# ParCoreLab/aCG

Hardware: AMD Instinct MI355X
Metric: CG iter/s (whole node), Queen_4147-shaped fp64 (higher is better)
Workload: dtype fp64; 1 GPU; model=queen4147-like-27pt-dof3-G111, rows=4102893, solver=cg-pipelined, parallelism=slab1-rccl

## Files before the change

acg_amd/gen/device_slab.py:

```python

from __future__ import annotations

import numpy as np
import torch

from ..part.subdomain import HaloPattern
from .stencil import _blocks, _slab_bounds


class DeviceSlabSystem:

    def __init__(self, **kw):
        self.__dict__.update(kw)

    @property
    def nlocal(self):
        return self.nowned + self.nghost

    @property
    def nnzA(self):
        return self._nnzA

    @property
    def nnzO(self):
        return self._nnzO


def estimate_slab_gib(gx: int, gy: int, gz: int, spec: dict, rank: int,
                      nranks: int, matfree: bool = False) -> float:
    dof = spec["dof"]
    pts = len(spec["offsets"]) + 1
    z0, z1 = _slab_bounds(gz, rank, nranks)
    nghost_planes = (1 if rank > 0 else 0) + (1 if rank < nranks - 1 else 0)
    nlocal = (z1 - z0 + nghost_planes) * gx * gy * dof
    bytes_per_row = 81.0 if matfree else 12.0 * pts * dof + 73.0
    return nlocal * bytes_per_row / 2**30


def preflight_slab(gx: int, gy: int, gz: int, spec: dict, rank: int,
                   nranks: int, matfree: bool, total_bytes: int,
                   headroom: float = 0.94) -> float:
    est = estimate_slab_gib(gx, gy, gz, spec, rank, nranks, matfree)
    budget = headroom * total_bytes / 2**30
    if est > budget:
        raise MemoryError(
            f"rank {rank}/{nranks} of {gx}x{gy}x{gz} needs ~{est:.0f} GiB "
            f"({'matfree' if matfree else 'assembled'}) but this GPU has "
            f"{total_bytes / 2**30:.0f} GiB ({budget:.0f} usable); use more "
            f"ranks, --matfree, or a smaller --grid")
    return est


def device_stencil_slab(gx: int, gy: int, gz: int, spec: dict,
                        rank: int, nranks: int, device,
                        operator: bool = True) -> DeviceSlabSystem:
    from ..ops import gpu_ops

    K = gpu_ops.K
    device = torch.device(device)
    dof = spec["dof"]
    M, D = _blocks(spec)
    z0, z1 = _slab_bounds(gz, rank, nranks)
    nz_own = z1 - z0
    if nz_own <= 0:
        raise ValueError(f"rank {rank} owns no z-planes")
    plane_nodes = gx * gy
    has_lo, has_hi = rank > 0, rank < nranks - 1
    border_planes = sorted(set(([z0] if has_lo else []) +
                               ([z1 - 1] if has_hi else [])))
    interior_planes = [z for z in range(z0, z1) if z not in border_planes]
    ghost_planes = ([z0 - 1] if has_lo else []) + ([z1] if has_hi else [])
    plane_seq = interior_planes + border_planes + ghost_planes

    nown_nodes = nz_own * plane_nodes
    ninterior_nodes = len(interior_planes) * plane_nodes
    nborder_nodes = len(border_planes) * plane_nodes
    nghost_nodes = len(ghost_planes) * plane_nodes
    nowned = nown_nodes * dof
    nghost = nghost_nodes * dof
    assert (nowned + nghost) * 1 < 2**31, "device generator needs int32 local cols"

    pb = torch.full((gz + 2,), -1, dtype=torch.int64)
    for k, z in enumerate(plane_seq):
        pb[z + 1] = k * plane_nodes
    zs_own = torch.tensor([z for z in interior_planes + border_planes],
                          dtype=torch.int32)
    pb = pb.to(device)
    zs_own = zs_own.to(device)
    offs_np = np.asarray([[dx, dy, dz, w] for (dx, dy, dz, w) in spec["offsets"]],
                         dtype=np.float64)
    offs = torch.from_numpy(offs_np).reshape(-1).to(device)
    ksten = len(spec["offsets"])
    blocks = torch.from_numpy(
        np.concatenate([M.reshape(-1), D.reshape(-1)])).to(device)
    stream = torch.cuda.current_stream(device).cuda_stream

    def build(filter_ghost: int, nodes: int, row0_node: int):
        if nodes == 0:
            empty = torch.zeros(1, dtype=torch.int64, device=device)
            return (torch.zeros(1, dtype=torch.int64, device=device),
                    torch.zeros(0, dtype=torch.int32, device=device),
                    torch.zeros(0, dtype=torch.float64, device=device), 0)
        rowlen_nodes = torch.empty(nodes, dtype=torch.int64, device=device)
        K.stencil_rowlen(nodes, row0_node, gx, gy, gz, dof, nown_nodes,
                         zs_own.data_ptr(), pb.data_ptr(), offs.data_ptr(),
                         ksten, filter_ghost, rowlen_nodes.data_ptr(), stream)
        rowlen = rowlen_nodes if dof == 1 else rowlen_nodes.repeat_interleave(dof)
        nnz = int(rowlen.sum())
        if not operator:
            return None, None, None, nnz
        nrows = nodes * dof
        nslices = (nrows + 63) // 64
        padded = torch.zeros(nslices * 64, dtype=torch.int64, device=device)
        padded[:nrows] = rowlen
        slice_len = padded.view(nslices, 64).max(dim=1).values
        sellptr = torch.zeros(nslices + 1, dtype=torch.int64, device=device)
        torch.cumsum(slice_len * 64, dim=0, out=sellptr[1:])
        total = int(sellptr[-1])
        cols = torch.zeros(total, dtype=torch.int32, device=device)
        vals = torch.zeros(total, dtype=torch.float64, device=device)
        K.stencil_fill(nodes, row0_node, gx, gy, gz, dof, nown_nodes,
                       zs_own.data_ptr(), pb.data_ptr(), offs.data_ptr(),
                       ksten, blocks.data_ptr(), filter_ghost,
                       sellptr.data_ptr(), cols.data_ptr(), vals.data_ptr(),
                       stream)
        return sellptr, cols, vals, nnz

    A_sellptr, A_cols, A_vals, nnzA = build(0, nown_nodes, 0)
    O_sellptr, O_cols, O_vals, nnzO = build(1, nborder_nodes, ninterior_nodes)

    mf_tables = None
    if dof == 1:
        w7 = None
        if ksten == 6:
            wmap = {(int(dx), int(dy), int(dz)): float(w)
                    for (dx, dy, dz, w) in spec["offsets"]}
            keys = [(-1, 0, 0), (1, 0, 0), (0, -1, 0),
                    (0, 1, 0), (0, 0, -1), (0, 0, 1)]
            if set(wmap) == set(keys):
                w7 = tuple(wmap[k] for k in keys)
        mf_tables = dict(zs=zs_own, pb=pb, offs=offs, ksten=ksten,
                         diag=float(D[0, 0]), gx=gx, gy=gy, gz=gz,
                         nown_nodes=nown_nodes, z0=z0, z1=z1, w7=w7)

    A_bsell = None
    if operator and 2 <= dof <= 4 and nown_nodes > 0:
        blocklen = torch.empty(nown_nodes, dtype=torch.int64, device=device)
        K.stencil_blocklen(nown_nodes, gx, gy, gz, nown_nodes,
                           zs_own.data_ptr(), pb.data_ptr(), offs.data_ptr(),
                           ksten, blocklen.data_ptr(), stream)
        nbslices = (nown_nodes + 63) // 64
        bp = torch.zeros(nbslices * 64, dtype=torch.int64, device=device)
        bp[:nown_nodes] = blocklen
        blk_slice = bp.view(nbslices, 64).max(dim=1).values
        bptr = torch.zeros(nbslices + 1, dtype=torch.int64, device=device)
        torch.cumsum(blk_slice * 64, dim=0, out=bptr[1:])
        btotal = int(bptr[-1])
        bcol = torch.zeros(btotal, dtype=torch.int32, device=device)
        bvals = torch.zeros(btotal * dof * dof, dtype=torch.float64, device=device)
        K.stencil_bfill(nown_nodes, gx, gy, gz, dof, nown_nodes,
                        zs_own.data_ptr(), pb.data_ptr(), offs.data_ptr(),
                        ksten, blocks.data_ptr(), bptr.data_ptr(),
                        bcol.data_ptr(), bvals.data_ptr(), stream)
        A_bsell = (bptr, bcol, bvals, dof)

    senders, recvcounts, rdispls = [], [], []
    recipients, sendidx_parts = [], []
    off = 0
    if has_lo:
        senders.append(rank - 1)
        recvcounts.append(plane_nodes * dof)
        rdispls.append(off)
        off += plane_nodes * dof
    if has_hi:
        senders.append(rank + 1)
        recvcounts.append(plane_nodes * dof)
        rdispls.append(off)
        off += plane_nodes * dof

    plane_local = {z: k for k, z in enumerate(plane_seq)}

    def plane_rows(z):
        b = plane_local[z] * plane_nodes
        node_loc = b + np.arange(plane_nodes, dtype=np.int64)
        return (node_loc[:, None] * dof + np.arange(dof)[None, :]).ravel()

    if has_lo:
        recipients.append(rank - 1)
        sendidx_parts.append(plane_rows(z0))
    if has_hi:
        recipients.append(rank + 1)
        sendidx_parts.append(plane_rows(z1 - 1))
    sendcounts = [len(s) for s in sendidx_parts]
    sdispls = list(np.concatenate([[0], np.cumsum(sendcounts)[:-1]])) if sendcounts else []
    sendidx = (np.concatenate(sendidx_parts) if sendidx_parts
               else np.zeros(0, np.int64))
    halo = HaloPattern(
        senders=np.asarray(senders, dtype=np.int32),
        recvcounts=np.asarray(recvcounts, dtype=np.int64),
        rdispls=np.asarray(rdispls, dtype=np.int64),
        recipients=np.asarray(recipients, dtype=np.int32),
        sendcounts=np.asarray(sendcounts, dtype=np.int64),
        sdispls=np.asarray(sdispls, dtype=np.int64),
        sendidx=sendidx.astype(np.int32),
    )
    return DeviceSlabSystem(
        rank=rank, nparts=nranks, n_global=gx * gy * gz * dof,
        nowned=nowned, ninterior=ninterior_nodes * dof,
        nborder=nborder_nodes * dof, nghost=nghost,
        A_sell=(A_sellptr, A_cols, A_vals) if operator else None,
        A_bsell=A_bsell,
        O_sell=(O_sellptr, O_cols, O_vals) if operator else None,
        mf_tables=mf_tables,
        _nnzA=nnzA, _nnzO=nnzO, halo=halo, device=device,
    )
```

acg_amd/ops/gpu_ops.py:

```python

from __future__ import annotations

import torch

try:
    from . import _acg_kernels as K
except ImportError as e:
    raise ImportError(
        "acg_amd HIP kernel extension (_acg_kernels) is not built. "
        "Run `python -m acg_amd.ops.build` (hipcc --offload-arch=gfx950). "
        f"Original error: {e}"
    ) from e

S_RR = K.S_RR
S_PT = K.S_PT
S_RR_PREV = K.S_RR_PREV
S_BNRM2 = K.S_BNRM2
S_GAMMA = K.S_GAMMA
S_DELTA = K.S_DELTA
S_GAMMA_PREV = K.S_GAMMA_PREV
S_ALPHA_PREV = K.S_ALPHA_PREV
S_NSLOTS = K.S_NSLOTS
MAXG = K.MAXG


def _stream() -> int:
    return torch.cuda.current_stream().cuda_stream


def alloc_scalars(device) -> torch.Tensor:
    return torch.zeros(S_NSLOTS, dtype=torch.float64, device=device)


def alloc_partials(device) -> torch.Tensor:
    return torch.zeros(2 * MAXG, dtype=torch.float64, device=device)


def pick_lanes(mean_nnz_per_row: float) -> int:
    if mean_nnz_per_row <= 4.0:
        return 4
    if mean_nnz_per_row <= 8.0:
        return 8
    if mean_nnz_per_row <= 16.0:
        return 16
    if mean_nnz_per_row <= 96.0:
        return 32
    return 64


def spmv(rowptr: torch.Tensor, colidx: torch.Tensor, vals: torch.Tensor,
         x: torch.Tensor, y: torch.Tensor, *, rowbase: int = 0,
         lanes: int = 16, accum: bool = False,
         partials: torch.Tensor | None = None,
         scal: torch.Tensor | None = None, dotslot: int = -1,
         dot_accum: bool = True) -> None:
    nrows = rowptr.numel() - 1
    if nrows <= 0:
        return
    fuse = scal is not None and dotslot >= 0
    K.spmv(nrows, rowbase, rowptr.data_ptr(), colidx.data_ptr(),
           1 if colidx.dtype == torch.int64 else 0,
           vals.data_ptr(), x.data_ptr(), y.data_ptr(), lanes, accum,
           partials.data_ptr() if fuse else 0,
           scal.data_ptr() if fuse else 0, dotslot, dot_accum, _stream())


def build_row_bins(rowptr, max_lanes: int = 64):
    import numpy as np

    rowptr = np.asarray(rowptr)
    lens = np.diff(rowptr)
    order = np.argsort(-lens, kind="stable").astype(np.int32)
    slens = lens[order.astype(np.int64)]
    bins = []
    lo = 0
    for lanes, thresh in ((64, 96), (32, 16), (16, 8), (8, 4), (4, None)):
        if lanes > max_lanes:
            continue
        if thresh is None:
            hi = len(slens)
        else:
            hi = int(np.searchsorted(-slens, -thresh - 1, side="right"))
        if hi > lo:
            bins.append((lo, hi - lo, lanes))
            lo = hi
    return order, bins


def build_sellcsr_hybrid(rowptr, colidx, vals, cut: int = 192,
                         window: int = 0, bucket: int = 8):
    import numpy as np

    from .torch_ref import sellcsr_split

    sellptr, cols, svals, perm, long_rows, nshort = sellcsr_split(
        rowptr, colidx, vals, cut=cut, window=window, bucket=bucket)
    lens = np.diff(np.asarray(rowptr))
    longlens = lens[long_rows.astype(np.int64)]
    bins = []
    lo = 0
    for lanes, thresh in ((64, 96), (32, 16), (16, 8), (8, 4), (4, None)):
        if thresh is None:
            hi = len(longlens)
        else:
            hi = int(np.searchsorted(-longlens, -thresh - 1, side="right"))
        if hi > lo:
            bins.append((lo, hi - lo, lanes))
            lo = hi
        if lo >= len(longlens):
            break
    if nshort == 0:
        sellptr = None
    return sellptr, cols, svals, perm, long_rows, bins


def spmv_binned(rowptr: torch.Tensor, colidx: torch.Tensor, vals: torch.Tensor,
                rowlist: torch.Tensor, bins, x: torch.Tensor, y: torch.Tensor,
                *, rowbase: int = 0, accum: bool = False,
                partials: torch.Tensor | None = None,
                scal: torch.Tensor | None = None, dotslot: int = -1,
                dot_accum: bool = True) -> None:
    if rowlist.numel() == 0:
        return
    assert rowlist.dtype == torch.int32
    fuse = scal is not None and dotslot >= 0
    K.spmv_binned(rowbase, rowptr.data_ptr(), colidx.data_ptr(),
                  1 if colidx.dtype == torch.int64 else 0,
                  vals.data_ptr(), x.data_ptr(), y.data_ptr(),
                  rowlist.data_ptr(), [list(b) for b in bins], accum,
                  partials.data_ptr() if fuse else 0,
                  scal.data_ptr() if fuse else 0, dotslot, dot_accum,
                  _stream())


SELL_NT, SELL_SWZ, SELL_U8 = 1, 2, 4
DEFAULT_SELL_VARIANT = SELL_NT | SELL_U8


def spmv_sell(sellptr: torch.Tensor, cols: torch.Tensor, vals: torch.Tensor,
              nrows: int, x: torch.Tensor, y: torch.Tensor, *,
              rowbase: int = 0, accum: bool = False,
              partials: torch.Tensor | None = None,
              scal: torch.Tensor | None = None, dotslot: int = -1,
              dot_accum: bool = True, variant: int | None = None,
              perm: torch.Tensor | None = None) -> None:
    nslices = sellptr.numel() - 1
    if nslices <= 0:
        return
    if variant is None:
        variant = DEFAULT_SELL_VARIANT
    fuse = scal is not None and dotslot >= 0
    K.spmv_sell(nslices, nrows, rowbase, sellptr.data_ptr(), cols.data_ptr(),
                1 if cols.dtype == torch.int64 else 0,
                vals.data_ptr(), x.data_ptr(), y.data_ptr(), accum,
                partials.data_ptr() if fuse else 0,
                scal.data_ptr() if fuse else 0, dotslot, dot_accum,
                variant, perm.data_ptr() if perm is not None else 0, _stream())


def spmv_bsell(bptr: torch.Tensor, bcol: torch.Tensor, bvals: torch.Tensor,
               nnodes: int, dof: int, x: torch.Tensor, y: torch.Tensor, *,
               partials: torch.Tensor | None = None,
               scal: torch.Tensor | None = None, dotslot: int = -1,
               dot_accum: bool = True) -> None:
    nslices = bptr.numel() - 1
    if nslices <= 0:
        return
    fuse = scal is not None and dotslot >= 0
    K.spmv_bsell(nslices, nnodes, dof, bptr.data_ptr(), bcol.data_ptr(),
                 bvals.data_ptr(), x.data_ptr(), y.data_ptr(),
                 partials.data_ptr() if fuse else 0,
                 scal.data_ptr() if fuse else 0, dotslot, dot_accum, _stream())


def stencil_spmv(mf, nrows_nodes: int, row0_node: int, x: torch.Tensor,
                 y: torch.Tensor, *, mato: bool = False,
                 partials: torch.Tensor | None = None,
                 scal: torch.Tensor | None = None, dotslot: int = -1,
                 dot_accum: bool = True) -> None:
    if nrows_nodes <= 0:
        return
    fuse = scal is not None and dotslot >= 0
    pp = partials.data_ptr() if fuse else 0
    sp = scal.data_ptr() if fuse else 0
    if not mato and mf["w7"] is not None:
        K.stencil_spmv7(mf["gx"] * mf["gy"], mf["gx"], mf["z0"], mf["z1"],
                        mf["gz"], mf["nown_nodes"], mf["pb"].data_ptr(),
                        mf["diag"], *mf["w7"], x.data_ptr(), y.data_ptr(),
                        pp, sp, dotslot, dot_accum, _stream())
        return
    K.stencil_spmv(nrows_nodes, row0_node, mf["gx"], mf["gy"], mf["gz"],
                   mf["nown_nodes"], mf["zs"].data_ptr(),
                   mf["pb"].data_ptr(), mf["offs"].data_ptr(), mf["ksten"],
                   mf["diag"], x.data_ptr(), y.data_ptr(), mato,
                   pp, sp, dotslot, dot_accum, _stream())


def stencil_pipe(mf, nrows_nodes: int, row0_node: int, border_base: int,
                 w_old, qpart, z, t, p, x, r, w_new, scal, first: bool,
                 partials, partials_off: int, mato: bool) -> int:
    if nrows_nodes <= 0:
        return 0
    qp = qpart.data_ptr() if qpart is not None else 0
    if not mato and mf["w7"] is not None:
        return K.stencil_pipe7(mf["gx"] * mf["gy"], mf["gx"], mf["z0"],
                               mf["z1"], mf["gz"], border_base,
                               mf["nown_nodes"], mf["pb"].data_ptr(),
                               mf["diag"], *mf["w7"], w_old.data_ptr(), qp,
                               z.data_ptr(), t.data_ptr(), p.data_ptr(),
                               x.data_ptr(), r.data_ptr(), w_new.data_ptr(),
                               scal.data_ptr(), 1 if first else 0,
                               partials.data_ptr(), partials_off, _stream())
    return K.stencil_pipe(nrows_nodes, row0_node, border_base, mf["gx"],
                          mf["gy"], mf["gz"], mf["nown_nodes"],
                          mf["zs"].data_ptr(), mf["pb"].data_ptr(),
                          mf["offs"].data_ptr(), mf["ksten"], mf["diag"],
                          w_old.data_ptr(), qp,
                          z.data_ptr(), t.data_ptr(), p.data_ptr(),
                          x.data_ptr(), r.data_ptr(), w_new.data_ptr(),
                          scal.data_ptr(), 1 if first else 0,
                          partials.data_ptr(), partials_off, mato, _stream())


def spmv_bsell_daypx(bptr, bcol, bvals, nnodes: int, dof: int,
                     pold: torch.Tensor, rvec: torch.Tensor,
                     pnew: torch.Tensor, y: torch.Tensor,
                     scal: torch.Tensor, partials: torch.Tensor,
                     dotslot: int) -> None:
    nslices = bptr.numel() - 1
    if nslices <= 0:
        return
    K.spmv_bsell_daypx(nslices, nnodes, dof, bptr.data_ptr(), bcol.data_ptr(),
                       bvals.data_ptr(), pold.data_ptr(), rvec.data_ptr(),
                       pnew.data_ptr(), y.data_ptr(), scal.data_ptr(),
                       partials.data_ptr(), dotslot, _stream())


def zero_scalars(scal: torch.Tensor, i0: int = 0, count: int | None = None) -> None:
    K.zero_scalars(scal.data_ptr(), i0, count if count is not None else scal.numel() - i0,
                   _stream())


def cg_prep_pt(scal: torch.Tensor) -> None:
    K.cg_prep_pt(scal.data_ptr(), _stream())


def cg_prep_rr(scal: torch.Tensor) -> None:
    K.cg_prep_rr(scal.data_ptr(), _stream())


def dot(x: torch.Tensor, y: torch.Tensor, partials: torch.Tensor,
        scal: torch.Tensor, slot: int, n: int | None = None,
        accumulate: bool = False) -> None:
    n = x.numel() if n is None else n
    K.dot(x.data_ptr(), y.data_ptr(), n, partials.data_ptr(), scal.data_ptr(),
          slot, accumulate, _stream())


def dot2(r: torch.Tensor, w: torch.Tensor, partials: torch.Tensor,
         scal: torch.Tensor, n: int, accumulate: bool = False) -> None:
    K.dot2(r.data_ptr(), w.data_ptr(), n, partials.data_ptr(), scal.data_ptr(),
           accumulate, _stream())


def axpy_ratio(y: torch.Tensor, x: torch.Tensor, scal: torch.Tensor,
               num: int, den: int, sign: float = 1.0, n: int | None = None) -> None:
    K.axpy_ratio(y.data_ptr(), x.data_ptr(), y.numel() if n is None else n,
                 scal.data_ptr(), num, den, sign, _stream())


def daypx_ratio(y: torch.Tensor, x: torch.Tensor, scal: torch.Tensor,
                num: int, den: int, n: int | None = None) -> None:
    K.daypx_ratio(y.data_ptr(), x.data_ptr(), y.numel() if n is None else n,
                  scal.data_ptr(), num, den, _stream())


def cg_fused_update(r: torch.Tensor, x: torch.Tensor, p: torch.Tensor,
                    t: torch.Tensor, scal: torch.Tensor,
                    partials: torch.Tensor, n: int) -> None:
    K.cg_fused_update(r.data_ptr(), x.data_ptr(), p.data_ptr(), t.data_ptr(),
                      n, scal.data_ptr(), partials.data_ptr(), _stream())


def pcg_fused_update(r, x, p, t, z, dinv, scal, partials, n: int) -> None:
    K.pcg_fused_update(r.data_ptr(), x.data_ptr(), p.data_ptr(), t.data_ptr(),
                       z.data_ptr(), dinv.data_ptr(), n, scal.data_ptr(),
                       partials.data_ptr(), _stream())


def sell_pipe(sellptr, cols, vals, nrows_pass: int, rowbase: int,
              border_base: int, w_old, qpart, z, t, p, x, r, w_new,
              scal, first: bool, partials, partials_off: int,
              mato: bool) -> int:
    nslices = sellptr.numel() - 1
    assert cols.dtype == torch.int32
    return K.sell_pipe(nslices, nrows_pass, rowbase, border_base,
                       sellptr.data_ptr(), cols.data_ptr(), vals.data_ptr(),
                       w_old.data_ptr(),
                       qpart.data_ptr() if qpart is not None else 0,
                       z.data_ptr(), t.data_ptr(), p.data_ptr(), x.data_ptr(),
                       r.data_ptr(), w_new.data_ptr(), scal.data_ptr(),
                       1 if first else 0, partials.data_ptr(), partials_off,
                       mato, _stream())


def pipelined_finalize(partials, nblocks: int, scal, first: bool) -> None:
    K.pipelined_finalize(partials.data_ptr(), nblocks, scal.data_ptr(),
                         1 if first else 0, _stream())


def pipelined_fused(z, t, p, x, r, w, q, scal: torch.Tensor,
                    partials: torch.Tensor, n: int, first: bool,
                    nt_update: bool = True) -> None:
    K.pipelined_fused(z.data_ptr(), t.data_ptr(), p.data_ptr(), x.data_ptr(),
                      r.data_ptr(), w.data_ptr(), q.data_ptr(), n,
                      scal.data_ptr(), 1 if first else 0, partials.data_ptr(),
                      nt_update, _stream())


BAR_STATE_WORDS = 400


def cg_device(sellptr: torch.Tensor, cols: torch.Tensor, vals: torch.Tensor,
              nrows: int, b: torch.Tensor, x: torch.Tensor, r: torch.Tensor,
              p: torch.Tensor, t: torch.Tensor, scal: torch.Tensor,
              partials: torch.Tensor, out2: torch.Tensor,
              barrier_state: torch.Tensor, maxits: int,
              res_atol: float, res_rtol: float,
              hier: bool | None = None) -> int:
    nslices = sellptr.numel() - 1
    assert barrier_state.numel() >= BAR_STATE_WORDS
    if hier is None:
        import os

        v = os.environ.get("ACG_DEVCG_HIER", "auto")
        ih = -1 if v == "auto" else (0 if v == "0" else 1)
    else:
        ih = 1 if hier else 0
    return K.cg_device(nslices, nrows, sellptr.data_ptr(), cols.data_ptr(),
                       1 if cols.dtype == torch.int64 else 0, vals.data_ptr(),
                       b.data_ptr(), x.data_ptr(), r.data_ptr(), p.data_ptr(),
                       t.data_ptr(), scal.data_ptr(), partials.data_ptr(),
                       out2.data_ptr(), barrier_state.data_ptr(),
                       maxits, res_atol, res_rtol, _stream(), ih)


def pack_gather(sendbuf: torch.Tensor, x: torch.Tensor, idx: torch.Tensor) -> None:
    K.pack_gather(sendbuf.data_ptr(), x.data_ptr(), idx.data_ptr(),
                  1 if idx.dtype == torch.int64 else 0,
                  sendbuf.numel(), _stream())
```

acg_amd/ops/kernels.hip:

```cpp
#define S_RR 0
#define S_PT 1
#define S_RR_PREV 2
#define S_BNRM2 3
#define S_GAMMA 4
#define S_DELTA 5
#define S_GAMMA_PREV 6
#define S_ALPHA_PREV 7
#define S_NSLOTS 8

#define MAXG 16384

#include <hip/hip_runtime.h>
#include <pybind11/pybind11.h>
#include <pybind11/stl.h>
#include <array>
#include <cstdint>
#include <vector>
#include <stdexcept>
#include <string>

namespace py = pybind11;

#define WAVE 64
#define BLOCK 256

static inline void check_hip(const char* what) {
    hipError_t e = hipGetLastError();
    if (e != hipSuccess)
        throw std::runtime_error(std::string("HIP error in ") + what + ": " + hipGetErrorString(e));
}

static inline long elem_grid(long n, long per_thread = 4) {
    long blocks = (n + (long)BLOCK * per_thread - 1) / ((long)BLOCK * per_thread);
    if (blocks > 4096) blocks = 4096;
    if (blocks < 1) blocks = 1;
    return blocks;
}

__device__ __forceinline__ double block_reduce(double v) {
    #pragma unroll
    for (int off = WAVE / 2; off > 0; off >>= 1)
        v += __shfl_down(v, off, WAVE);
    __shared__ double w[BLOCK / WAVE];
    const int lane = threadIdx.x & (WAVE - 1);
    const int wid = threadIdx.x >> 6;
    if (lane == 0) w[wid] = v;
    __syncthreads();
    if (wid == 0) {
        v = (lane < BLOCK / WAVE) ? w[lane] : 0.0;
        #pragma unroll
        for (int off = (BLOCK / WAVE) / 2; off > 0; off >>= 1)
            v += __shfl_down(v, off, WAVE);
    }
    return v;
}

__device__ __forceinline__ double safe_div(double a, double b) {
    return b != 0.0 ? a / b : 0.0;
}

__global__ void __launch_bounds__(BLOCK)
k_reduce_partials(const double* __restrict__ partials, int nblocks,
                  double* scal, int slot, int accumulate) {
    double v = 0.0;
    for (int i = threadIdx.x; i < nblocks; i += BLOCK) v += partials[i];
    v = block_reduce(v);
    if (threadIdx.x == 0) scal[slot] = accumulate ? scal[slot] + v : v;
}

template <typename ColT, int LANES, bool ACCUM, bool FUSE_DOT, bool ROWLIST = false>
__global__ void __launch_bounds__(BLOCK)
spmv_csr_vector(long nrows, long rowbase,
                const long* __restrict__ rowptr,
                const ColT* __restrict__ colidx,
                const double* __restrict__ vals,
                const double* __restrict__ x,
                double* __restrict__ y,
                double* __restrict__ partials,
                const int* __restrict__ rowlist = nullptr) {
    const int lane = threadIdx.x & (LANES - 1);
    const long group = ((long)blockIdx.x * BLOCK + threadIdx.x) / LANES;
    const long ngroups = (long)gridDim.x * BLOCK / LANES;
    double dacc = 0.0;
    for (long i = group; i < nrows; i += ngroups) {
        const long r = ROWLIST ? (long)rowlist[i] : i;
        const long k0 = rowptr[r], k1 = rowptr[r + 1];
        double sum = 0.0;
        for (long k = k0 + lane; k < k1; k += LANES)
            sum += vals[k] * x[colidx[k]];
        #pragma unroll
        for (int off = LANES / 2; off > 0; off >>= 1)
            sum += __shfl_down(sum, off, LANES);
        if (lane == 0) {
            const long row = rowbase + r;
            if (ACCUM) y[row] += sum; else y[row] = sum;
            if (FUSE_DOT) dacc += x[row] * sum;
        }
    }
    if (FUSE_DOT) {
        dacc = block_reduce(dacc);
        if (threadIdx.x == 0) partials[blockIdx.x] = dacc;
    }
}

#define SELL_NT 1
#define SELL_SWZ 2
#define SELL_U8 4

template <typename T>
__device__ __forceinline__ T ld_nt(const T* p) { return __builtin_nontemporal_load(p); }

template <typename ColT, bool ACCUM, bool FUSE_DOT, bool NT, bool SWZ, int UNROLL,
          bool PERM = false>
__global__ void __launch_bounds__(BLOCK)
k_spmv_sell(long nslices, long nrows, long rowbase,
          const long* __restrict__ sellptr,
          const ColT* __restrict__ cols,
          const double* __restrict__ vals,
          const double* __restrict__ x,
          double* __restrict__ y,
          double* __restrict__ partials,
          const int* __restrict__ perm = nullptr) {
    const int lane = threadIdx.x & (WAVE - 1);
    long blk = blockIdx.x;
    if (SWZ) {
        const long nb = gridDim.x, q = nb / 8, rr = nb % 8, xcd = blk % 8;
        blk = (xcd < rr ? xcd * (q + 1) : rr * (q + 1) + (xcd - rr) * q) + blk / 8;
    }
    const long wslice = (blk * BLOCK + threadIdx.x) >> 6;
    const long nw = ((long)gridDim.x * BLOCK) >> 6;
    double dacc = 0.0;
    for (long s = wslice; s < nslices; s += nw) {
        const long base = sellptr[s];
        const long len = (sellptr[s + 1] - base) >> 6;
        const double* __restrict__ v = vals + base + lane;
        const ColT* __restrict__ c = cols + base + lane;
        double sum = 0.0;
        long j = 0;
        for (; j + UNROLL <= len; j += UNROLL) {
            double a[UNROLL], xx[UNROLL];
            #pragma unroll
            for (int u = 0; u < UNROLL; ++u) {
                a[u] = NT ? ld_nt(v + (j + u) * WAVE) : v[(j + u) * WAVE];
                const ColT ci = NT ? ld_nt(c + (j + u) * WAVE) : c[(j + u) * WAVE];
                xx[u] = x[ci];
            }
            #pragma unroll
            for (int u = 0; u < UNROLL; ++u) sum += a[u] * xx[u];
        }
        for (; j < len; ++j) {
            const double a = NT ? ld_nt(v + j * WAVE) : v[j * WAVE];
            const ColT ci = NT ? ld_nt(c + j * WAVE) : c[j * WAVE];
            sum += a * x[ci];
        }
        const long row = PERM ? (long)perm[s * WAVE + lane] : s * WAVE + lane;
        if (row < nrows) {
            if (ACCUM) y[rowbase + row] += sum; else y[rowbase + row] = sum;
            if (FUSE_DOT) dacc += x[rowbase + row] * sum;
        }
    }
    if (FUSE_DOT) {
        dacc = block_reduce(dacc);
        if (threadIdx.x == 0) partials[blockIdx.x] = dacc;
    }
}

__device__ __forceinline__ long stencil_col_node(
    int xi, int yi, int zi, int dx, int dy, int dz, int gx, int gy, int gz,
    const long* __restrict__ pb);

template <int D2>
__device__ __forceinline__ long bval_off(int k, int lane) {
    constexpr int EVEN = D2 & ~1;
    return (k < EVEN) ? (long)(k >> 1) * (2 * WAVE) + lane * 2 + (k & 1)
                      : (long)EVEN * WAVE + lane;
}

template <int DOF, bool FUSE_DOT>
__global__ void __launch_bounds__(BLOCK)
k_spmv_bsell(long nslices, long nnodes,
             const long* __restrict__ bptr,
             const int* __restrict__ bcol,
             const double* __restrict__ bvals,
             const double* __restrict__ x,
             double* __restrict__ y,
             double* __restrict__ partials) {
    const int lane = threadIdx.x & (WAVE - 1);
    const long wslice = ((long)blockIdx.x * BLOCK + threadIdx.x) >> 6;
    const long nw = ((long)gridDim.x * BLOCK) >> 6;
    double dacc = 0.0;
    for (long s = wslice; s < nslices; s += nw) {
        const long b0 = bptr[s];
        const long blen = (bptr[s + 1] - b0) >> 6;
        const int* __restrict__ c = bcol + b0 + lane;
        const double* __restrict__ v = bvals + b0 * (DOF * DOF);
        double acc[DOF];
        #pragma unroll
        for (int r = 0; r < DOF; ++r) acc[r] = 0.0;
        for (long j = 0; j < blen; ++j) {
            const int cb = ld_nt(c + j * WAVE);
            double xv[DOF];
            #pragma unroll
            for (int cc = 0; cc < DOF; ++cc) xv[cc] = x[(long)cb * DOF + cc];
            const double* __restrict__ vj = v + j * (DOF * DOF) * WAVE;
            #pragma unroll
            for (int k = 0; k < DOF * DOF; ++k) {
                const double a = ld_nt(vj + bval_off<DOF * DOF>(k, lane));
                acc[k / DOF] += a * xv[k % DOF];
            }
        }
        const long node = s * WAVE + lane;
        if (node < nnodes) {
            #pragma unroll
            for (int r = 0; r < DOF; ++r) {
                y[node * DOF + r] = acc[r];
                if (FUSE_DOT) dacc += x[node * DOF + r] * acc[r];
            }
        }
    }
    if (FUSE_DOT) {
        dacc = block_reduce(dacc);
        if (threadIdx.x == 0) partials[blockIdx.x] = dacc;
    }
}

template <int DOF>
__global__ void __launch_bounds__(BLOCK)
k_spmv_bsell_daypx(long nslices, long nnodes,
                   const long* __restrict__ bptr,
                   const int* __restrict__ bcol,
                   const double* __restrict__ bvals,
                   const double* __restrict__ pold,
                   const double* __restrict__ rvec,
                   double* __restrict__ pnew,
                   double* __restrict__ y,
                   const double* __restrict__ scal,
                   double* __restrict__ partials) {
    const int lane = threadIdx.x & (WAVE - 1);
    const long wslice = ((long)blockIdx.x * BLOCK + threadIdx.x) >> 6;
    const long nw = ((long)gridDim.x * BLOCK) >> 6;
    const double beta = safe_div(scal[S_RR], scal[S_RR_PREV]);
    double dacc = 0.0;
    for (long s = wslice; s < nslices; s += nw) {
        const long b0 = bptr[s];
        const long blen = (bptr[s + 1] - b0) >> 6;
        const int* __restrict__ c = bcol + b0 + lane;
        const double* __restrict__ v = bvals + b0 * (DOF * DOF);
        double acc[DOF];
        #pragma unroll
        for (int r = 0; r < DOF; ++r) acc[r] = 0.0;
        for (long j = 0; j < blen; ++j) {
            const int cb = ld_nt(c + j * WAVE);
            double xv[DOF];
            #pragma unroll
            for (int cc = 0; cc < DOF; ++cc)
                xv[cc] = beta * pold[(long)cb * DOF + cc]
                         + rvec[(long)cb * DOF + cc];
            const double* __restrict__ vj = v + j * (DOF * DOF) * WAVE;
            #pragma unroll
            for (int k = 0; k < DOF * DOF; ++k) {
                const double a = ld_nt(vj + bval_off<DOF * DOF>(k, lane));
                acc[k / DOF] += a * xv[k % DOF];
            }
        }
        const long node = s * WAVE + lane;
        if (node < nnodes) {
            #pragma unroll
            for (int r = 0; r < DOF; ++r) {
                const double pn = beta * pold[node * DOF + r]
                                  + rvec[node * DOF + r];
                pnew[node * DOF + r] = pn;
                y[node * DOF + r] = acc[r];
                dacc += pn * acc[r];
            }
        }
    }
    dacc = block_reduce(dacc);
    if (threadIdx.x == 0) partials[blockIdx.x] = dacc;
}

__global__ void __launch_bounds__(BLOCK)
k_stencil_blocklen(long nnodes, int gx, int gy, int gz, long nown_nodes,
                   const int* __restrict__ zs_of_plane,
                   const long* __restrict__ pb,
                   const double* __restrict__ offs, int ksten,
                   long* __restrict__ blocklen) {
    const long stride = (long)gridDim.x * BLOCK;
    const long plane_nodes = (long)gx * gy;
    for (long i = (long)blockIdx.x * BLOCK + threadIdx.x; i < nnodes; i += stride) {
        const int pl = (int)(i / plane_nodes);
        const long rem = i - (long)pl * plane_nodes;
        const int xi = (int)(rem % gx), yi = (int)(rem / gx);
        const int zi = zs_of_plane[pl];
        long cnt = 1;
        for (int o = 0; o < ksten; ++o) {
            const long cn = stencil_col_node(xi, yi, zi, (int)offs[o * 4],
                                             (int)offs[o * 4 + 1],
                                             (int)offs[o * 4 + 2], gx, gy, gz, pb);
            if (cn >= 0 && cn < nown_nodes) ++cnt;
        }
        blocklen[i] = cnt;
    }
}

template <int DOF>
__global__ void __launch_bounds__(BLOCK)
k_stencil_bfill(long nnodes, int gx, int gy, int gz, long nown_nodes,
                const int* __restrict__ zs_of_plane,
                const long* __restrict__ pb,
                const double* __restrict__ offs, int ksten,
                const double* __restrict__ blocks,
                const long* __restrict__ bptr,
                int* __restrict__ bcol, double* __restrict__ bvals) {
    const long stride = (long)gridDim.x * BLOCK;
    const long plane_nodes = (long)gx * gy;
    const double* M = blocks;
    const double* D = blocks + DOF * DOF;
    for (long i = (long)blockIdx.x * BLOCK + threadIdx.x; i < nnodes; i += stride) {
        const int pl = (int)(i / plane_nodes);
        const long rem = i - (long)pl * plane_nodes;
        const int xi = (int)(rem % gx), yi = (int)(rem / gx);
        const int zi = zs_of_plane[pl];
        const long s = i >> 6;
        const int lane = (int)(i & 63);
        const long b0 = bptr[s];
        const long blen = (bptr[s + 1] - b0) >> 6;
        long j = 0;
        double* __restrict__ bv = bvals + b0 * DOF * DOF;
        bcol[b0 + j * WAVE + lane] = (int)i;
        for (int k = 0; k < DOF * DOF; ++k)
            bv[j * DOF * DOF * WAVE + bval_off<DOF * DOF>(k, lane)] = D[k];
        ++j;
        for (int o = 0; o < ksten; ++o) {
            const long cn = stencil_col_node(xi, yi, zi, (int)offs[o * 4],
                                             (int)offs[o * 4 + 1],
                                             (int)offs[o * 4 + 2], gx, gy, gz, pb);
            if (cn < 0 || cn >= nown_nodes) continue;
            const double w = offs[o * 4 + 3];
            bcol[b0 + j * WAVE + lane] = (int)cn;
            for (int k = 0; k < DOF * DOF; ++k)
                bv[j * DOF * DOF * WAVE + bval_off<DOF * DOF>(k, lane)] = w * M[k];
            ++j;
        }
        for (; j < blen; ++j) {
            bcol[b0 + j * WAVE + lane] = (int)i;
            for (int k = 0; k < DOF * DOF; ++k)
                bv[j * DOF * DOF * WAVE + bval_off<DOF * DOF>(k, lane)] = 0.0;
        }
    }
}


__global__ void __launch_bounds__(BLOCK)
k_zero_scalars(double* scal, int i0, int count) {
    for (int i = threadIdx.x; i < count; i += BLOCK) scal[i0 + i] = 0.0;
}

__global__ void k_cg_prep_pt(double* scal) { if (threadIdx.x == 0) scal[S_PT] = 0.0; }

__global__ void k_cg_prep_rr(double* scal) {
    if (threadIdx.x == 0) scal[S_RR_PREV] = scal[S_RR];
}

__global__ void __launch_bounds__(BLOCK)
k_cg_finalize(const double* __restrict__ partials, int nblocks, double* scal) {
    double v = 0.0;
    for (int i = threadIdx.x; i < nblocks; i += BLOCK) v += partials[i];
    v = block_reduce(v);
    if (threadIdx.x == 0) {
        scal[S_RR_PREV] = scal[S_RR];
        scal[S_RR] = v;
    }
}

__global__ void __launch_bounds__(BLOCK)
k_pcg_fused_update(double* __restrict__ r, double* __restrict__ x,
                   const double* __restrict__ p, const double* __restrict__ t,
                   double* __restrict__ z, const double* __restrict__ dinv,
                   long n, const double* __restrict__ scal,
                   double* __restrict__ partials) {
    const double alpha = safe_div(scal[S_RR], scal[S_PT]);
    double arz = 0.0, arr = 0.0;
    const long stride = (long)gridDim.x * BLOCK;
    for (long i = (long)blockIdx.x * BLOCK + threadIdx.x; i < n; i += stride) {
        const double rn = r[i] - alpha * ld_nt(t + i);
        r[i] = rn;
        __builtin_nontemporal_store(ld_nt(x + i) + alpha * p[i], x + i);
        const double zi = dinv[i] * rn;
        z[i] = zi;
        arz += rn * zi;
        arr += rn * rn;
    }
    arz = block_reduce(arz);
    __syncthreads();
    arr = block_reduce(arr);
    if (threadIdx.x == 0) {
        partials[blockIdx.x] = arz;
        partials[MAXG + blockIdx.x] = arr;
    }
}

__global__ void __launch_bounds__(BLOCK)
k_pcg_finalize(const double* __restrict__ partials, int nblocks,
               double* scal) {
    double vz = 0.0, vr = 0.0;
    for (int i = threadIdx.x; i < nblocks; i += BLOCK) {
        vz += partials[i];
        vr += partials[MAXG + i];
    }
    vz = block_reduce(vz);
    __syncthreads();
    vr = block_reduce(vr);
    if (threadIdx.x == 0) {
        scal[S_RR_PREV] = scal[S_RR];
        scal[S_RR] = vz;
        scal[S_GAMMA] = vr;
    }
}

__global__ void __launch_bounds__(BLOCK)
k_dot(const double* __restrict__ x, const double* __restrict__ y, long n,
      double* __restrict__ partials) {
    double acc = 0.0;
    const long stride = (long)gridDim.x * BLOCK;
    for (long i = (long)blockIdx.x * BLOCK + threadIdx.x; i < n; i += stride)
        acc += x[i] * y[i];
    acc = block_reduce(acc);
    if (threadIdx.x == 0) partials[blockIdx.x] = acc;
}

__global__ void __launch_bounds__(BLOCK)
k_dot2(const double* __restrict__ r, const double* __restrict__ w, long n,
       double* __restrict__ partials) {
    double g = 0.0, d = 0.0;
    const long stride = (long)gridDim.x * BLOCK;
    for (long i = (long)blockIdx.x * BLOCK + threadIdx.x; i < n; i += stride) {
        const double ri = r[i];
        g += ri * ri;
        d += w[i] * ri;
    }
    g = block_reduce(g);
    __syncthreads();
    d = block_reduce(d);
    if (threadIdx.x == 0) {
        partials[blockIdx.x] = g;
        partials[MAXG + blockIdx.x] = d;
    }
}

__global__ void __launch_bounds__(BLOCK)
k_reduce_partials2(const double* __restrict__ partials, int nblocks,
                   double* scal, int accumulate) {
    double g = 0.0, d = 0.0;
    for (int i = threadIdx.x; i < nblocks; i += BLOCK) {
        g += partials[i];
        d += partials[MAXG + i];
    }
    g = block_reduce(g);
    __syncthreads();
    d = block_reduce(d);
    if (threadIdx.x == 0) {
        scal[S_GAMMA] = accumulate ? scal[S_GAMMA] + g : g;
        scal[S_DELTA] = accumulate ? scal[S_DELTA] + d : d;
    }
}

__global__ void __launch_bounds__(BLOCK)
k_axpy_ratio(double* __restrict__ y, const double* __restrict__ x, long n,
             const double* __restrict__ scal, int num, int den, double sign) {
    const double a = sign * safe_div(scal[num], scal[den]);
    const long stride = (long)gridDim.x * BLOCK;
    for (long i = (long)blockIdx.x * BLOCK + threadIdx.x; i < n; i += stride)
        y[i] += a * x[i];
}

__global__ void __launch_bounds__(BLOCK)
k_daypx_ratio(double* __restrict__ y, const double* __restrict__ x, long n,
              const double* __restrict__ scal, int num, int den) {
    const double b = safe_div(scal[num], scal[den]);
    const long stride = (long)gridDim.x * BLOCK;
    for (long i = (long)blockIdx.x * BLOCK + threadIdx.x; i < n; i += stride)
        y[i] = b * y[i] + x[i];
}

__global__ void __launch_bounds__(BLOCK)
k_cg_fused_update(double* __restrict__ r, double* __restrict__ x,
                  const double* __restrict__ p, const double* __restrict__ t,
                  long n, const double* __restrict__ scal,
                  double* __restrict__ partials) {
    const double alpha = safe_div(scal[S_RR], scal[S_PT]);
    double acc = 0.0;
    const long stride = (long)gridDim.x * BLOCK;
    for (long i = (long)blockIdx.x * BLOCK + threadIdx.x; i < n; i += stride) {
        const double rn = r[i] - alpha * ld_nt(t + i);
        r[i] = rn;
        __builtin_nontemporal_store(ld_nt(x + i) + alpha * p[i], x + i);
        acc += rn * rn;
    }
    acc = block_reduce(acc);
    if (threadIdx.x == 0) partials[blockIdx.x] = acc;
}

__device__ __forceinline__ void pipelined_coeffs(const double* scal, int first,
                                                 double* beta, double* alpha) {
    const double gamma = scal[S_GAMMA], delta = scal[S_DELTA];
    if (first) { *beta = 0.0; *alpha = safe_div(gamma, delta); }
    else {
        const double b = safe_div(gamma, scal[S_GAMMA_PREV]);
        *beta = b;
        *alpha = safe_div(gamma,
                          delta - b * safe_div(gamma, scal[S_ALPHA_PREV]));
    }
}

template <bool NTU>
__global__ void __launch_bounds__(BLOCK)
k_pipelined_fused(double* __restrict__ z, double* __restrict__ t,
                  double* __restrict__ p, double* __restrict__ x,
                  double* __restrict__ r, double* __restrict__ w,
                  const double* __restrict__ q, long n,
                  const double* __restrict__ scal, int first,
                  double* __restrict__ partials) {
    double beta, alpha;
    pipelined_coeffs(scal, first, &beta, &alpha);
    double g = 0.0, d = 0.0;
    const long stride = (long)gridDim.x * BLOCK;
    for (long i = (long)blockIdx.x * BLOCK + threadIdx.x; i < n; i += stride) {
        const double zi = (NTU ? ld_nt(q + i) : q[i]) + beta * (NTU ? ld_nt(z + i) : z[i]);
        const double ti = w[i] + beta * (NTU ? ld_nt(t + i) : t[i]);
        const double pi = r[i] + beta * (NTU ? ld_nt(p + i) : p[i]);
        const double xn = (NTU ? ld_nt(x + i) : x[i]) + alpha * pi;
        if (NTU) {
            __builtin_nontemporal_store(zi, z + i);
            __builtin_nontemporal_store(ti, t + i);
            __builtin_nontemporal_store(pi, p + i);
            __builtin_nontemporal_store(xn, x + i);
        } else {
            z[i] = zi; t[i] = ti; p[i] = pi; x[i] = xn;
        }
        const double rn = r[i] - alpha * ti;
        const double wn = w[i] - alpha * zi;
        r[i] = rn; w[i] = wn;
        g += rn * rn;
        d += wn * rn;
    }
    g = block_reduce(g);
    __syncthreads();
    d = block_reduce(d);
    if (threadIdx.x == 0) {
        partials[blockIdx.x] = g;
        partials[MAXG + blockIdx.x] = d;
    }
}

template <typename ColT, bool NT, int UNROLL, bool MATO>
__global__ void __launch_bounds__(BLOCK)
k_sell_pipe(long nslices, long nrows_pass, long rowbase, long border_base,
            const long* __restrict__ sellptr, const ColT* __restrict__ cols,
            const double* __restrict__ vals,
            const double* __restrict__ w_old,
            double* __restrict__ qpart,
            double* __restrict__ z, double* __restrict__ t,
            double* __restrict__ p, double* __restrict__ x,
            double* __restrict__ r, double* __restrict__ w_new,
            const double* __restrict__ scal, int first,
            double* __restrict__ partials, long partials_off) {
    const int lane = threadIdx.x & (WAVE - 1);
    const long wslice = ((long)blockIdx.x * BLOCK + threadIdx.x) >> 6;
    const long nw = ((long)gridDim.x * BLOCK) >> 6;
    double beta, alpha;
    pipelined_coeffs(scal, first, &beta, &alpha);
    double g = 0.0, d = 0.0;
    for (long s = wslice; s < nslices; s += nw) {
        const long base = sellptr[s];
        const long len = (sellptr[s + 1] - base) >> 6;
        const double* __restrict__ v = vals + base + lane;
        const ColT* __restrict__ c = cols + base + lane;
        double sum = 0.0;
        long j = 0;
        for (; j + UNROLL <= len; j += UNROLL) {
            double a[UNROLL], xx[UNROLL];
            #pragma unroll
            for (int u = 0; u < UNROLL; ++u) {
                a[u] = NT ? ld_nt(v + (j + u) * WAVE) : v[(j + u) * WAVE];
                xx[u] = w_old[c[(j + u) * WAVE]];
            }
            #pragma unroll
            for (int u = 0; u < UNROLL; ++u) sum += a[u] * xx[u];
        }
        for (; j < len; ++j)
            sum += (NT ? ld_nt(v + j * WAVE) : v[j * WAVE]) * w_old[c[j * WAVE]];
        const long rr = s * WAVE + lane;
        if (rr < nrows_pass) {
            const long row = rowbase + rr;
            if (!MATO && row >= border_base) {
                qpart[row - border_base] = sum;
            } else {
                const double q = MATO ? sum + qpart[row - border_base] : sum;
                const double zi = q + beta * ld_nt(z + row);
                const double ti = w_old[row] + beta * ld_nt(t + row);
                const double pi = r[row] + beta * ld_nt(p + row);
                __builtin_nontemporal_store(zi, z + row);
                __builtin_nontemporal_store(ti, t + row);
                __builtin_nontemporal_store(pi, p + row);
                __builtin_nontemporal_store(ld_nt(x + row) + alpha * pi, x + row);
                const double rn = r[row] - alpha * ti;
                const double wn = w_old[row] - alpha * zi;
                r[row] = rn; w_new[row] = wn;
                g += rn * rn;
                d += wn * rn;
            }
        }
    }
    g = block_reduce(g);
    __syncthreads();
    d = block_reduce(d);
    if (threadIdx.x == 0) {
        partials[partials_off + blockIdx.x] = g;
        partials[MAXG + partials_off + blockIdx.x] = d;
    }
}

__global__ void __launch_bounds__(BLOCK)
k_pipelined_finalize(const double* __restrict__ partials, int nblocks,
                     double* scal, int first) {
    double g = 0.0, d = 0.0;
    for (int i = threadIdx.x; i < nblocks; i += BLOCK) {
        g += partials[i];
        d += partials[MAXG + i];
    }
    g = block_reduce(g);
    __syncthreads();
    d = block_reduce(d);
    if (threadIdx.x == 0) {
        double beta, alpha;
        pipelined_coeffs(scal, first, &beta, &alpha);
        scal[S_GAMMA_PREV] = scal[S_GAMMA];
        scal[S_ALPHA_PREV] = alpha;
        scal[S_GAMMA] = g;
        scal[S_DELTA] = d;
    }
}


__device__ __forceinline__ long stencil_col_node(
    int xi, int yi, int zi, int dx, int dy, int dz, int gx, int gy, int gz,
    const long* __restrict__ pb) {
    const int nx = xi + dx, ny = yi + dy, nz = zi + dz;
    if (nx < 0 || nx >= gx || ny < 0 || ny >= gy || nz < 0 || nz >= gz)
        return -1;
    const long base = pb[nz + 1];
    if (base < 0) return -1;
    return base + nx + (long)gx * ny;
}

__global__ void __launch_bounds__(BLOCK)
k_stencil_rowlen(long nrows_nodes, long row0_node, int gx, int gy, int gz,
                 int dof, long nown_nodes,
                 const int* __restrict__ zs_of_plane,
                 const long* __restrict__ pb,
                 const double* __restrict__ offs, int ksten,
                 int filter_ghost, long* __restrict__ rowlen) {
    const long stride = (long)gridDim.x * BLOCK;
    const long plane_nodes = (long)gx * gy;
    for (long i = (long)blockIdx.x * BLOCK + threadIdx.x; i < nrows_nodes;
         i += stride) {
        const long node = row0_node + i;
        const int pl = (int)(node / plane_nodes);
        const long rem = node - (long)pl * plane_nodes;
        const int xi = (int)(rem % gx), yi = (int)(rem / gx);
        const int zi = zs_of_plane[pl];
        long cnt = filter_ghost ? 0 : 1;
        for (int o = 0; o < ksten; ++o) {
            const int dx = (int)offs[o * 4 + 0], dy = (int)offs[o * 4 + 1],
                      dz = (int)offs[o * 4 + 2];
            const long cn = stencil_col_node(xi, yi, zi, dx, dy, dz, gx, gy, gz, pb);
            if (cn < 0) continue;
            const bool ghost = cn >= nown_nodes;
            if (ghost == (bool)filter_ghost) ++cnt;
        }
        rowlen[i] = cnt * dof;
    }
}

__global__ void __launch_bounds__(BLOCK)
k_stencil_fill(long nrows_nodes, long row0_node, int gx, int gy, int gz,
               int dof, long nown_nodes,
               const int* __restrict__ zs_of_plane,
               const long* __restrict__ pb,
               const double* __restrict__ offs, int ksten,
               const double* __restrict__ blocks,
               int filter_ghost,
               const long* __restrict__ sellptr,
               int* __restrict__ cols, double* __restrict__ vals) {
    const long stride = (long)gridDim.x * BLOCK;
    const long plane_nodes = (long)gx * gy;
    const double* M = blocks;
    const double* D = blocks + dof * dof;
    const long nrows = nrows_nodes * dof;
    for (long row = (long)blockIdx.x * BLOCK + threadIdx.x; row < nrows;
         row += stride) {
        const long nodei = row / dof;
        const int a = (int)(row - nodei * dof);
        const long node = row0_node + nodei;
        const int pl = (int)(node / plane_nodes);
        const long rem = node - (long)pl * plane_nodes;
        const int xi = (int)(rem % gx), yi = (int)(rem / gx);
        const int zi = zs_of_plane[pl];
        const long s = row >> 6;
        const int lane = (int)(row & 63);
        const long base = sellptr[s];
        const long len = (sellptr[s + 1] - base) >> 6;
        long j = 0;
        if (!filter_ghost) {
            for (int bb = 0; bb < dof; ++bb, ++j) {
                cols[base + j * WAVE + lane] = (int)(node * dof + bb);
                vals[base + j * WAVE + lane] = D[a * dof + bb];
            }
        }
        for (int o = 0; o < ksten; ++o) {
            const int dx = (int)offs[o * 4 + 0], dy = (int)offs[o * 4 + 1],
                      dz = (int)offs[o * 4 + 2];
            const double w = offs[o * 4 + 3];
            const long cn = stencil_col_node(xi, yi, zi, dx, dy, dz, gx, gy, gz, pb);
            if (cn < 0) continue;
            const bool ghost = cn >= nown_nodes;
            if (ghost != (bool)filter_ghost) continue;
            for (int bb = 0; bb < dof; ++bb, ++j) {
                cols[base + j * WAVE + lane] = (int)(cn * dof + bb);
                vals[base + j * WAVE + lane] = w * M[a * dof + bb];
            }
        }
        const int selfcol = (int)(filter_ghost ? 0 : node * dof + a);
        for (; j < len; ++j) {
            cols[base + j * WAVE + lane] = selfcol;
            vals[base + j * WAVE + lane] = 0.0;
        }
    }
}

void spmv_bsell(long nslices, long nnodes, int dof, uintptr_t bptr,
                uintptr_t bcol, uintptr_t bvals, uintptr_t x, uintptr_t y,
                uintptr_t partials, uintptr_t scal, int dotslot,
                bool dot_accum, uintptr_t stream) {
    if (nnodes == 0) return;
    long blocks = (nslices * WAVE + BLOCK - 1) / BLOCK;
    if (blocks > MAXG) blocks = MAXG;
    const bool fuse = partials != 0 && dotslot >= 0;
    dim3 g((unsigned)blocks), b(BLOCK);
    #define LBS(D, FD) \
        hipLaunchKernelGGL((k_spmv_bsell<D, FD>), g, b, 0, (hipStream_t)stream, \
            nslices, nnodes, (const long*)bptr, (const int*)bcol, \
            (const double*)bvals, (const double*)x, (double*)y, (double*)partials)
    switch (dof) {
        case 2: if (fuse) { LBS(2, true); } else { LBS(2, false); } break;
        case 3: if (fuse) { LBS(3, true); } else { LBS(3, false); } break;
        case 4: if (fuse) { LBS(4, true); } else { LBS(4, false); } break;
        default: throw std::runtime_error("spmv_bsell: dof must be 2/3/4");
    }
    #undef LBS
    check_hip("spmv_bsell");
    if (fuse) {
        hipLaunchKernelGGL(k_reduce_partials, dim3(1), dim3(BLOCK), 0,
                           (hipStream_t)stream, (const double*)partials,
                           (int)blocks, (double*)scal, dotslot, dot_accum ? 1 : 0);
        check_hip("spmv_bsell_reduce");
    }
}

void spmv_bsell_daypx(long nslices, long nnodes, int dof, uintptr_t bptr,
                      uintptr_t bcol, uintptr_t bvals, uintptr_t pold,
                      uintptr_t rvec, uintptr_t pnew, uintptr_t y,
                      uintptr_t scal, uintptr_t partials, int dotslot,
                      uintptr_t stream) {
    if (nnodes == 0) return;
    long blocks = (nslices * WAVE + BLOCK - 1) / BLOCK;
    if (blocks > MAXG) blocks = MAXG;
    dim3 g((unsigned)blocks), b(BLOCK);
    #define LBD(D) \
        hipLaunchKernelGGL((k_spmv_bsell_daypx<D>), g, b, 0, (hipStream_t)stream, \
            nslices, nnodes, (const long*)bptr, (const int*)bcol, \
            (const double*)bvals, (const double*)pold, (const double*)rvec, \
            (double*)pnew, (double*)y, (const double*)scal, (double*)partials)
    switch (dof) {
        case 2: LBD(2); break;
        case 3: LBD(3); break;
        case 4: LBD(4); break;
        default: throw std::runtime_error("spmv_bsell_daypx: dof must be 2/3/4");
    }
    #undef LBD
    check_hip("spmv_bsell_daypx");
    hipLaunchKernelGGL(k_reduce_partials, dim3(1), dim3(BLOCK), 0,
                       (hipStream_t)stream, (const double*)partials,
                       (int)blocks, (double*)scal, dotslot, 0);
    check_hip("spmv_bsell_daypx_reduce");
}

void stencil_blocklen(long nnodes, int gx, int gy, int gz, long nown_nodes,
                      uintptr_t zs_of_plane, uintptr_t pb, uintptr_t offs,
                      int ksten, uintptr_t blocklen, uintptr_t stream) {
    hipLaunchKernelGGL(k_stencil_blocklen, dim3((unsigned)elem_grid(nnodes)),
                       dim3(BLOCK), 0, (hipStream_t)stream,
                       nnodes, gx, gy, gz, nown_nodes, (const int*)zs_of_plane,
                       (const long*)pb, (const double*)offs, ksten,
                       (long*)blocklen);
    check_hip("stencil_blocklen");
}

void stencil_bfill(long nnodes, int gx, int gy, int gz, int dof,
                   long nown_nodes, uintptr_t zs_of_plane, uintptr_t pb,
                   uintptr_t offs, int ksten, uintptr_t blocks_md,
                   uintptr_t bptr, uintptr_t bcol, uintptr_t bvals,
                   uintptr_t stream) {
    dim3 g((unsigned)elem_grid(nnodes)), b(BLOCK);
    #define LBF(D) \
        hipLaunchKernelGGL((k_stencil_bfill<D>), g, b, 0, (hipStream_t)stream, \
            nnodes, gx, gy, gz, nown_nodes, (const int*)zs_of_plane, \
            (const long*)pb, (const double*)offs, ksten, \
            (const double*)blocks_md, (const long*)bptr, (int*)bcol, \
            (double*)bvals)
    switch (dof) {
        case 2: LBF(2); break;
        case 3: LBF(3); break;
        case 4: LBF(4); break;
        default: throw std::runtime_error("stencil_bfill: dof must be 2/3/4");
    }
    #undef LBF
    check_hip("stencil_bfill");
}

void stencil_rowlen(long nrows_nodes, long row0_node, int gx, int gy, int gz,
                    int dof, long nown_nodes, uintptr_t zs_of_plane,
                    uintptr_t pb, uintptr_t offs, int ksten, int filter_ghost,
                    uintptr_t rowlen, uintptr_t stream) {
    hipLaunchKernelGGL(k_stencil_rowlen, dim3((unsigned)elem_grid(nrows_nodes)),
                       dim3(BLOCK), 0, (hipStream_t)stream,
                       nrows_nodes, row0_node, gx, gy, gz, dof, nown_nodes,
                       (const int*)zs_of_plane, (const long*)pb,
                       (const double*)offs, ksten, filter_ghost, (long*)rowlen);
    check_hip("stencil_rowlen");
}

void stencil_fill(long nrows_nodes, long row0_node, int gx, int gy, int gz,
                  int dof, long nown_nodes, uintptr_t zs_of_plane,
                  uintptr_t pb, uintptr_t offs, int ksten, uintptr_t blocks,
                  int filter_ghost, uintptr_t sellptr, uintptr_t cols,
                  uintptr_t vals, uintptr_t stream) {
    const long nrows = nrows_nodes * dof;
    hipLaunchKernelGGL(k_stencil_fill, dim3((unsigned)elem_grid(nrows)),
                       dim3(BLOCK), 0, (hipStream_t)stream,
                       nrows_nodes, row0_node, gx, gy, gz, dof, nown_nodes,
                       (const int*)zs_of_plane, (const long*)pb,
                       (const double*)offs, ksten, (const double*)blocks,
                       filter_ghost, (const long*)sellptr, (int*)cols,
                       (double*)vals);
    check_hip("stencil_fill");
}

template <bool MATO, bool FUSE_DOT>
__global__ void __launch_bounds__(BLOCK)
k_stencil_spmv(long nrows_nodes, long row0_node, int gx, int gy, int gz,
               long nown_nodes,
               const int* __restrict__ zs_of_plane,
               const long* __restrict__ pb,
               const double* __restrict__ offs, int ksten, double diag,
               const double* __restrict__ x, double* __restrict__ y,
               double* __restrict__ partials) {
    const long stride = (long)gridDim.x * BLOCK;
    const long plane_nodes = (long)gx * gy;
    double dacc = 0.0;
    for (long i = (long)blockIdx.x * BLOCK + threadIdx.x; i < nrows_nodes;
         i += stride) {
        const long node = row0_node + i;
        const int pl = (int)(node / plane_nodes);
        const long rem = node - (long)pl * plane_nodes;
        const int xi = (int)(rem % gx), yi = (int)(rem / gx);
        const int zi = zs_of_plane[pl];
        double sum = MATO ? 0.0 : diag * x[node];
        for (int o = 0; o < ksten; ++o) {
            const int dx = (int)offs[o * 4 + 0], dy = (int)offs[o * 4 + 1],
                      dz = (int)offs[o * 4 + 2];
            const long cn = stencil_col_node(xi, yi, zi, dx, dy, dz,
                                             gx, gy, gz, pb);
            if (cn < 0) continue;
            if ((cn >= nown_nodes) == MATO) sum += offs[o * 4 + 3] * x[cn];
        }
        if (MATO) y[node] += sum; else y[node] = sum;
        if (FUSE_DOT) dacc += x[node] * sum;
    }
    if (FUSE_DOT) {
        dacc = block_reduce(dacc);
        if (threadIdx.x == 0) partials[blockIdx.x] = dacc;
    }
}

template <bool MATO>
__global__ void __launch_bounds__(BLOCK)
k_stencil_pipe(long nrows_nodes, long row0_node, long border_base,
               int gx, int gy, int gz, long nown_nodes,
               const int* __restrict__ zs_of_plane,
               const long* __restrict__ pb,
               const double* __restrict__ offs, int ksten, double diag,
               const double* __restrict__ w_old, double* __restrict__ qpart,
               double* __restrict__ z, double* __restrict__ t,
               double* __restrict__ p, double* __restrict__ xv,
               double* __restrict__ r, double* __restrict__ w_new,
               const double* __restrict__ scal, int first,
               double* __restrict__ partials, long partials_off) {
    const long stride = (long)gridDim.x * BLOCK;
    const long plane_nodes = (long)gx * gy;
    double beta, alpha;
    pipelined_coeffs(scal, first, &beta, &alpha);
    double g = 0.0, d = 0.0;
    for (long i = (long)blockIdx.x * BLOCK + threadIdx.x; i < nrows_nodes;
         i += stride) {
        const long node = row0_node + i;
        const int pl = (int)(node / plane_nodes);
        const long rem = node - (long)pl * plane_nodes;
        const int xi = (int)(rem % gx), yi = (int)(rem / gx);
        const int zi = zs_of_plane[pl];
        double sum = MATO ? 0.0 : diag * w_old[node];
        for (int o = 0; o < ksten; ++o) {
            const int dx = (int)offs[o * 4 + 0], dy = (int)offs[o * 4 + 1],
                      dz = (int)offs[o * 4 + 2];
            const long cn = stencil_col_node(xi, yi, zi, dx, dy, dz,
                                             gx, gy, gz, pb);
            if (cn < 0) continue;
            if ((cn >= nown_nodes) == MATO) sum += offs[o * 4 + 3] * w_old[cn];
        }
        const long row = node;
        if (!MATO && row >= border_base) {
            qpart[row - border_base] = sum;
        } else {
            const double q = MATO ? sum + qpart[row - border_base] : sum;
            const double zi_ = q + beta * ld_nt(z + row);
            const double ti = w_old[row] + beta * ld_nt(t + row);
            const double pi = r[row] + beta * ld_nt(p + row);
            __builtin_nontemporal_store(zi_, z + row);
            __builtin_nontemporal_store(ti, t + row);
            __builtin_nontemporal_store(pi, p + row);
            __builtin_nontemporal_store(ld_nt(xv + row) + alpha * pi, xv + row);
            const double rn = r[row] - alpha * ti;
            const double wn = w_old[row] - alpha * zi_;
            r[row] = rn; w_new[row] = wn;
            g += rn * rn;
            d += wn * rn;
        }
    }
    g = block_reduce(g);
    __syncthreads();
    d = block_reduce(d);
    if (threadIdx.x == 0) {
        partials[partials_off + blockIdx.x] = g;
        partials[MAXG + partials_off + blockIdx.x] = d;
    }
}

template <bool FUSE_DOT>
__global__ void __launch_bounds__(BLOCK)
k_stencil_spmv7(long plane_nodes, int gx, int z0, int z1, int gz,
                long nown_nodes, const long* __restrict__ pb,
                double diag, double wxm, double wxp, double wym, double wyp,
                double wzm, double wzp,
                const double* __restrict__ x, double* __restrict__ y,
                double* __restrict__ partials) {
    const long stride = (long)gridDim.x * BLOCK;
    double dacc = 0.0;
    for (long xy = (long)blockIdx.x * BLOCK + threadIdx.x; xy < plane_nodes;
         xy += stride) {
        const int xi = (int)(xy % gx);
        const long yi = xy / gx;
        const bool hxm = xi > 0, hxp = xi < gx - 1;
        const bool hym = yi > 0, hyp = yi < plane_nodes / gx - 1;
        long base_c = pb[z0 + 1];
        double xc = x[base_c + xy];
        const long base_m = (z0 > 0) ? pb[z0] : -1;
        bool hm = base_m >= 0 && base_m < nown_nodes;
        double xm = hm ? x[base_m + xy] : 0.0;
        for (int zz = z0; zz < z1; ++zz) {
            const long node = base_c + xy;
            const long base_p = (zz + 1 < gz) ? pb[zz + 2] : -1;
            const bool hp = base_p >= 0 && base_p < nown_nodes;
            const double xp = hp ? x[base_p + xy] : 0.0;
            double sum = diag * xc;
            if (hxm) sum += wxm * x[node - 1];
            if (hxp) sum += wxp * x[node + 1];
            if (hym) sum += wym * x[node - gx];
            if (hyp) sum += wyp * x[node + gx];
            if (hm) sum += wzm * xm;
            if (hp) sum += wzp * xp;
            y[node] = sum;
            if (FUSE_DOT) dacc += xc * sum;
            xm = xc; hm = true;
            xc = xp; base_c = base_p;
        }
    }
    if (FUSE_DOT) {
        dacc = block_reduce(dacc);
        if (threadIdx.x == 0) partials[blockIdx.x] = dacc;
    }
}

__global__ void __launch_bounds__(BLOCK)
k_stencil_pipe7(long plane_nodes, int gx, int z0, int z1, int gz,
                long border_base, long nown_nodes,
                const long* __restrict__ pb,
                double diag, double wxm, double wxp, double wym, double wyp,
                double wzm, double wzp,
                const double* __restrict__ w_old, double* __restrict__ qpart,
                double* __restrict__ z, double* __restrict__ t,
                double* __restrict__ p, double* __restrict__ xv,
                double* __restrict__ r, double* __restrict__ w_new,
                const double* __restrict__ scal, int first,
                double* __restrict__ partials, long partials_off) {
    const long stride = (long)gridDim.x * BLOCK;
    double beta, alpha;
    pipelined_coeffs(scal, first, &beta, &alpha);
    double g = 0.0, d = 0.0;
    for (long xy = (long)blockIdx.x * BLOCK + threadIdx.x; xy < plane_nodes;
         xy += stride) {
        const int xi = (int)(xy % gx);
        const long yi = xy / gx;
        const bool hxm = xi > 0, hxp = xi < gx - 1;
        const bool hym = yi > 0, hyp = yi < plane_nodes / gx - 1;
        long base_c = pb[z0 + 1];
        double xc = w_old[base_c + xy];
        const long base_m = (z0 > 0) ? pb[z0] : -1;
        bool hm = base_m >= 0 && base_m < nown_nodes;
        double xm = hm ? w_old[base_m + xy] : 0.0;
        for (int zz = z0; zz < z1; ++zz) {
            const long node = base_c + xy;
            const long base_p = (zz + 1 < gz) ? pb[zz + 2] : -1;
            const bool hp = base_p >= 0 && base_p < nown_nodes;
            const double xp = hp ? w_old[base_p + xy] : 0.0;
            double sum = diag * xc;
            if (hxm) sum += wxm * w_old[node - 1];
            if (hxp) sum += wxp * w_old[node + 1];
            if (hym) sum += wym * w_old[node - gx];
            if (hyp) sum += wyp * w_old[node + gx];
            if (hm) sum += wzm * xm;
            if (hp) sum += wzp * xp;
            if (node >= border_base) {
                qpart[node - border_base] = sum;
            } else {
                const double zi_ = sum + beta * ld_nt(z + node);
                const double ti = xc + beta * ld_nt(t + node);
                const double pi = r[node] + beta * ld_nt(p + node);
                __builtin_nontemporal_store(zi_, z + node);
                __builtin_nontemporal_store(ti, t + node);
                __builtin_nontemporal_store(pi, p + node);
                __builtin_nontemporal_store(ld_nt(xv + node) + alpha * pi,
                                            xv + node);
                const double rn = r[node] - alpha * ti;
                const double wn = xc - alpha * zi_;
                r[node] = rn; w_new[node] = wn;
                g += rn * rn;
                d += wn * rn;
            }
            xm = xc; hm = true;
            xc = xp; base_c = base_p;
        }
    }
    g = block_reduce(g);
    __syncthreads();
    d = block_reduce(d);
    if (threadIdx.x == 0) {
        partials[partials_off + blockIdx.x] = g;
        partials[MAXG + partials_off + blockIdx.x] = d;
    }
}

void stencil_spmv7(long plane_nodes, int gx, int z0, int z1, int gz,
                   long nown_nodes, uintptr_t pb, double diag,
                   double wxm, double wxp, double wym, double wyp,
                   double wzm, double wzp, uintptr_t x, uintptr_t y,
                   uintptr_t partials, uintptr_t scal, int dotslot,
                   bool dot_accum, uintptr_t stream) {
    if (plane_nodes == 0 || z1 <= z0) return;
    long blocks = (plane_nodes + BLOCK - 1) / BLOCK;
    if (blocks > MAXG) blocks = MAXG;
    const bool fuse = partials != 0 && dotslot >= 0;
    dim3 g((unsigned)blocks), b(BLOCK);
    #define LS7(FD) \
        hipLaunchKernelGGL((k_stencil_spmv7<FD>), g, b, 0, (hipStream_t)stream, \
            plane_nodes, gx, z0, z1, gz, nown_nodes, (const long*)pb, diag, \
            wxm, wxp, wym, wyp, wzm, wzp, (const double*)x, (double*)y, \
            (double*)partials)
    if (fuse) { LS7(true); } else { LS7(false); }
    #undef LS7
    check_hip("stencil_spmv7");
    if (fuse) {
        hipLaunchKernelGGL(k_reduce_partials, dim3(1), dim3(BLOCK), 0,
                           (hipStream_t)stream, (const double*)partials,
                           (int)blocks, (double*)scal, dotslot, dot_accum ? 1 : 0);
        check_hip("stencil_spmv7_reduce");
    }
}

long stencil_pipe7(long plane_nodes, int gx, int z0, int z1, int gz,
                   long border_base, long nown_nodes, uintptr_t pb,
                   double diag, double wxm, double wxp, double wym,
                   double wyp, double wzm, double wzp, uintptr_t w_old,
                   uintptr_t qpart, uintptr_t z, uintptr_t t, uintptr_t p,
                   uintptr_t xv, uintptr_t r, uintptr_t w_new, uintptr_t scal,
                   int first, uintptr_t partials, long partials_off,
                   uintptr_t stream) {
    if (plane_nodes == 0 || z1 <= z0) return 0;
    long blocks = (plane_nodes + BLOCK - 1) / BLOCK;
    const long cap = (partials_off == 0) ? (MAXG - 1024) : (MAXG - partials_off);
    if (blocks > cap) blocks = cap;
    dim3 g((unsigned)blocks), b(BLOCK);
    hipLaunchKernelGGL(k_stencil_pipe7, g, b, 0, (hipStream_t)stream,
                       plane_nodes, gx, z0, z1, gz, border_base, nown_nodes,
                       (const long*)pb, diag, wxm, wxp, wym, wyp, wzm, wzp,
                       (const double*)w_old, (double*)qpart, (double*)z,
                       (double*)t, (double*)p, (double*)xv, (double*)r,
                       (double*)w_new, (const double*)scal, first,
                       (double*)partials, partials_off);
    check_hip("stencil_pipe7");
    return blocks;
}

void stencil_spmv(long nrows_nodes, long row0_node, int gx, int gy, int gz,
                  long nown_nodes, uintptr_t zs_of_plane, uintptr_t pb,
                  uintptr_t offs, int ksten, double diag, uintptr_t x,
                  uintptr_t y, bool mato, uintptr_t partials, uintptr_t scal,
                  int dotslot, bool dot_accum, uintptr_t stream) {
    if (nrows_nodes == 0) return;
    const long blocks = elem_grid(nrows_nodes);
    const bool fuse = partials != 0 && dotslot >= 0;
    dim3 g((unsigned)blocks), b(BLOCK);
    #define LMS(MATO, FD) \
        hipLaunchKernelGGL((k_stencil_spmv<MATO, FD>), g, b, 0, \
            (hipStream_t)stream, nrows_nodes, row0_node, gx, gy, gz, \
            nown_nodes, (const int*)zs_of_plane, (const long*)pb, \
            (const double*)offs, ksten, diag, (const double*)x, (double*)y, \
            (double*)partials)
    if (mato) { if (fuse) { LMS(true, true); } else { LMS(true, false); } }
    else      { if (fuse) { LMS(false, true); } else { LMS(false, false); } }
    #undef LMS
    check_hip("stencil_spmv");
    if (fuse) {
        hipLaunchKernelGGL(k_reduce_partials, dim3(1), dim3(BLOCK), 0,
                           (hipStream_t)stream, (const double*)partials,
                           (int)blocks, (double*)scal, dotslot, dot_accum ? 1 : 0);
        check_hip("stencil_spmv_reduce");
    }
}

long stencil_pipe(long nrows_nodes, long row0_node, long border_base,
                  int gx, int gy, int gz, long nown_nodes,
                  uintptr_t zs_of_plane, uintptr_t pb, uintptr_t offs,
                  int ksten, double diag, uintptr_t w_old, uintptr_t qpart,
                  uintptr_t z, uintptr_t t, uintptr_t p, uintptr_t xv,
                  uintptr_t r, uintptr_t w_new, uintptr_t scal, int first,
                  uintptr_t partials, long partials_off, bool mato,
                  uintptr_t stream) {
    if (nrows_nodes == 0) return 0;
    long blocks = elem_grid(nrows_nodes);
    const long cap = (partials_off == 0) ? (MAXG - 1024) : (MAXG - partials_off);
    if (blocks > cap) blocks = cap;
    dim3 g((unsigned)blocks), b(BLOCK);
    #define LMP(MATO) \
        hipLaunchKernelGGL((k_stencil_pipe<MATO>), g, b, 0, (hipStream_t)stream, \
            nrows_nodes, row0_node, border_base, gx, gy, gz, nown_nodes, \
            (const int*)zs_of_plane, (const long*)pb, (const double*)offs, \
            ksten, diag, (const double*)w_old, (double*)qpart, (double*)z, \
            (double*)t, (double*)p, (double*)xv, (double*)r, (double*)w_new, \
            (const double*)scal, first, (double*)partials, partials_off)
    if (mato) { LMP(true); } else { LMP(false); }
    #undef LMP
    check_hip("stencil_pipe");
    return blocks;
}

#include <hip/hip_cooperative_groups.h>

#define RLX_AGENT __ATOMIC_RELAXED, __HIP_MEMORY_SCOPE_AGENT
typedef __attribute__((address_space(1))) unsigned int gu32;

#define BAR_GEN0 16
#define BAR_GENSTRIDE 16
#define BAR_XCNT0 144
#define BAR_XCNT_PAR 128
#define BAR_STATE_WORDS 400

__device__ __forceinline__ void st_sc1_f64(double* p, double v) {
    __hip_atomic_store(reinterpret_cast<unsigned long long*>(p),
                       (unsigned long long)__double_as_longlong(v), RLX_AGENT);
}

__device__ __forceinline__ bool grid_barrier_hier(unsigned* state) {
    gu32* fail = (gu32*)(state + 1);
    asm volatile("s_waitcnt vmcnt(0)" ::: "memory");
    __syncthreads();
    bool ok = true;
    if (threadIdx.x == 0) {
        const int myxcd = (int)(blockIdx.x & 7);
        const unsigned nb = gridDim.x;
        const unsigned q = nb >> 3, rmd = nb & 7u;
        const unsigned blocks_on_mine = q + ((unsigned)myxcd < rmd ? 1u : 0u);
        const unsigned nxcd = nb < 8u ? nb : 8u;
        gu32* mygen = (gu32*)(state + BAR_GEN0 + BAR_GENSTRIDE * myxcd);
        const unsigned g = __hip_atomic_load(mygen, RLX_AGENT);
        const unsigned par = g & 1u;
        gu32* xcnt = (gu32*)(state + BAR_XCNT0 + BAR_XCNT_PAR * par
                             + BAR_GENSTRIDE * myxcd);
        const unsigned ax = __hip_atomic_fetch_add(xcnt, 1u, RLX_AGENT) + 1u;
        bool releaser = false;
        if (ax == blocks_on_mine) {
            gu32* gcnt = (gu32*)(state + (par ? 8 : 0));
            const unsigned ag = __hip_atomic_fetch_add(gcnt, 1u, RLX_AGENT) + 1u;
            if (ag == nxcd) {
                __hip_atomic_store(gcnt, 0u, RLX_AGENT);
                #pragma unroll
                for (int xx = 0; xx < 8; ++xx)
                    __hip_atomic_store(
                        (gu32*)(state + BAR_XCNT0 + BAR_XCNT_PAR * par
                                + BAR_GENSTRIDE * xx), 0u, RLX_AGENT);
                #pragma unroll
                for (int xx = 0; xx < 8; ++xx)
                    __hip_atomic_store(
                        (gu32*)(state + BAR_GEN0 + BAR_GENSTRIDE * xx),
                        g + 1u, RLX_AGENT);
                releaser = true;
            }
        }
        if (!releaser) {
            unsigned spins = 0;
            while (__hip_atomic_load(mygen, RLX_AGENT) == g) {
                if (spins < 32) __builtin_amdgcn_s_sleep(2);
                else __builtin_amdgcn_s_sleep(64);
                if (++spins > 4000000u) {
                    __hip_atomic_store(fail, 1u, RLX_AGENT);
                    ok = false;
                    break;
                }
                if (__hip_atomic_load(fail, RLX_AGENT)) { ok = false; break; }
            }
        }
        __builtin_amdgcn_fence(__ATOMIC_ACQUIRE, "agent");
    }
    __syncthreads();
    return ok;
}

__device__ __forceinline__ bool grid_barrier(unsigned* state) {
    gu32* fail = (gu32*)(state + 1);
    asm volatile("s_waitcnt vmcnt(0)" ::: "memory");
    __syncthreads();
    bool ok = true;
    if (threadIdx.x == 0) {
        const int myxcd = (int)(blockIdx.x & 7);
        gu32* mygen = (gu32*)(state + BAR_GEN0 + BAR_GENSTRIDE * myxcd);
        const unsigned g = __hip_atomic_load(mygen, RLX_AGENT);
        gu32* cnt = (gu32*)(state + ((g & 1u) ? 8 : 0));
        const unsigned arrived = __hip_atomic_fetch_add(cnt, 1u, RLX_AGENT) + 1u;
        if (arrived == gridDim.x) {
            __hip_atomic_store(cnt, 0u, RLX_AGENT);
            #pragma unroll
            for (int xx = 0; xx < 8; ++xx)
                __hip_atomic_store((gu32*)(state + BAR_GEN0 + BAR_GENSTRIDE * xx),
                                   g + 1u, RLX_AGENT);
        } else {
            unsigned spins = 0;
            while (__hip_atomic_load(mygen, RLX_AGENT) == g) {
                if (spins < 32) __builtin_amdgcn_s_sleep(2);
                else __builtin_amdgcn_s_sleep(64);
                if (++spins > 4000000u) {
                    __hip_atomic_store(fail, 1u, RLX_AGENT);
                    ok = false;
                    break;
                }
                if (__hip_atomic_load(fail, RLX_AGENT)) { ok = false; break; }
            }
        }
        __builtin_amdgcn_fence(__ATOMIC_ACQUIRE, "agent");
    }
    __syncthreads();
    return ok;
}

template <typename ColT>
__global__ void __launch_bounds__(BLOCK)
k_cg_device(long nslices, long nrows,
            const long* __restrict__ sellptr, const ColT* __restrict__ cols,
            const double* __restrict__ vals,
            const double* __restrict__ b, double* __restrict__ x,
            double* __restrict__ r, double* __restrict__ p,
            double* __restrict__ t,
            double* __restrict__ scal, double* __restrict__ partials,
            int* __restrict__ out2, unsigned* __restrict__ barrier_state,
            int maxits, double res_atol, double res_rtol, int hier) {
    const long tid = (long)blockIdx.x * BLOCK + threadIdx.x;
    const long nth = (long)gridDim.x * BLOCK;
    const int lane = threadIdx.x & (WAVE - 1);
    const long wslice0 = tid >> 6;
    const long nw = nth >> 6;
    bool alive = true;
    auto gsync = [&]() {
        if (alive && !(hier ? grid_barrier_hier(barrier_state)
                            : grid_barrier(barrier_state))) alive = false;
        return alive;
    };

    auto grid_sum = [&](double v, int slot) {
        v = block_reduce(v);
        if (threadIdx.x == 0) st_sc1_f64(partials + blockIdx.x, v);
        if (!gsync()) return;
        if (blockIdx.x == 0) {
            double s = 0.0;
            for (int i = threadIdx.x; i < (int)gridDim.x; i += BLOCK)
                s += partials[i];
            s = block_reduce(s);
            if (threadIdx.x == 0) st_sc1_f64(scal + slot, s);
        }
        gsync();
    };
    auto spmv = [&](const double* __restrict__ xin, double* __restrict__ yout,
                    bool fuse) -> double {
        double dacc = 0.0;
        for (long s = wslice0; s < nslices; s += nw) {
            const long base = sellptr[s];
            const long len = (sellptr[s + 1] - base) >> 6;
            const double* __restrict__ v = vals + base + lane;
            const ColT* __restrict__ c = cols + base + lane;
            double sum = 0.0;
            long j = 0;
            for (; j + 4 <= len; j += 4) {
                double a0 = ld_nt(v + (j + 0) * WAVE), x0 = xin[c[(j + 0) * WAVE]];
                double a1 = ld_nt(v + (j + 1) * WAVE), x1 = xin[c[(j + 1) * WAVE]];
                double a2 = ld_nt(v + (j + 2) * WAVE), x2 = xin[c[(j + 2) * WAVE]];
                double a3 = ld_nt(v + (j + 3) * WAVE), x3 = xin[c[(j + 3) * WAVE]];
                sum += a0 * x0; sum += a1 * x1; sum += a2 * x2; sum += a3 * x3;
            }
            for (; j < len; ++j) sum += ld_nt(v + j * WAVE) * xin[c[j * WAVE]];
            const long row = s * WAVE + lane;
            if (row < nrows) {
                st_sc1_f64(yout + row, sum);
                if (fuse) dacc += xin[row] * sum;
            }
        }
        return dacc;
    };

    double acc = 0.0;
    for (long i = tid; i < nrows; i += nth) acc += b[i] * b[i];
    grid_sum(acc, S_BNRM2);
    spmv(x, t, false);
    gsync();
    acc = 0.0;
    for (long i = tid; i < nrows; i += nth) {
        const double ri = b[i] - t[i];
        st_sc1_f64(r + i, ri);
        st_sc1_f64(p + i, ri);
        acc += ri * ri;
    }
    grid_sum(acc, S_RR);
    const double bnrm2sqr = alive ? scal[S_BNRM2] : 1.0;
    double rr = alive ? scal[S_RR] : 0.0;
    if (tid == 0) st_sc1_f64(scal + S_RR_PREV, rr);
    const double rt = res_rtol * sqrt(bnrm2sqr) > res_atol
        ? res_rtol * sqrt(bnrm2sqr) : res_atol;
    const double rtol2 = rt * rt;
    int k = 0, converged = (rtol2 > 0.0 && rr <= rtol2) ? 1 : 0;
    while (alive && !converged && k < maxits) {
        gsync();
        const double pt_part = spmv(p, t, true);
        grid_sum(pt_part, S_PT);
        if (!alive) break;
        const double alpha = safe_div(rr, scal[S_PT]);
        acc = 0.0;
        for (long i = tid; i < nrows; i += nth) {
            const double rn = r[i] - alpha * t[i];
            st_sc1_f64(r + i, rn);
            st_sc1_f64(x + i, x[i] + alpha * p[i]);
            acc += rn * rn;
        }
        grid_sum(acc, S_RR);
        if (!alive) break;
        const double rr_new = scal[S_RR];
        const double beta = rr_new / rr;
        for (long i = tid; i < nrows; i += nth)
            st_sc1_f64(p + i, beta * p[i] + r[i]);
        rr = rr_new;
        ++k;
        if (rtol2 > 0.0 && rr <= rtol2) converged = 1;
    }
    if (tid == 0) {
        st_sc1_f64(scal + S_RR, rr);
        out2[0] = k;
        out2[1] = alive ? converged : -1;
    }
    (void)bnrm2sqr;
}

__global__ void __launch_bounds__(BLOCK)
k_atomic_probe(double* __restrict__ y, const int* __restrict__ idx,
               const double* __restrict__ v, long nnz, int mode) {
    const long stride = (long)gridDim.x * BLOCK;
    double acc = 0.0;
    for (long i = (long)blockIdx.x * BLOCK + threadIdx.x; i < nnz; i += stride) {
        if (mode == 0) unsafeAtomicAdd(&y[idx[i]], v[i]);
        else if (mode == 1) y[idx[i]] = v[i];
        else acc += y[idx[i]] * v[i];
    }
    if (mode == 2 && acc == -1.0) y[0] = acc;
}

template <typename IdxT>
__global__ void __launch_bounds__(BLOCK)
k_pack_gather(double* __restrict__ sendbuf, const double* __restrict__ x,
              const IdxT* __restrict__ idx, long n) {
    const long stride = (long)gridDim.x * BLOCK;
    for (long i = (long)blockIdx.x * BLOCK + threadIdx.x; i < n; i += stride)
        sendbuf[i] = x[idx[i]];
}


using std::uintptr_t;

static inline hipStream_t S(uintptr_t s) { return (hipStream_t)s; }

static void reduce_partials(uintptr_t partials, int nblocks, uintptr_t scal,
                            int slot, bool accumulate, uintptr_t stream) {
    hipLaunchKernelGGL(k_reduce_partials, dim3(1), dim3(BLOCK), 0, S(stream),
                       (const double*)partials, nblocks, (double*)scal, slot,
                       accumulate ? 1 : 0);
    check_hip("reduce_partials");
}

void spmv(long nrows, long rowbase, uintptr_t rowptr, uintptr_t colidx,
          int col64, uintptr_t vals, uintptr_t x, uintptr_t y,
          int lanes, bool accum, uintptr_t partials, uintptr_t scal,
          int dotslot, bool dot_accum, uintptr_t stream) {
    if (nrows == 0) return;
    const int rows_per_block = BLOCK / lanes;
    long blocks = (nrows + rows_per_block - 1) / rows_per_block;
    if (blocks > MAXG) blocks = MAXG;
    const bool fuse = partials != 0 && dotslot >= 0;
    dim3 g((unsigned)blocks), b(BLOCK);
    #define LAUNCH_SPMV(CT, L, AC, FD) \
        hipLaunchKernelGGL((spmv_csr_vector<CT, L, AC, FD>), g, b, 0, S(stream), \
            nrows, rowbase, (const long*)rowptr, (const CT*)colidx, \
            (const double*)vals, (const double*)x, (double*)y, (double*)partials)
    #define DISPATCH_L(CT, AC, FD) \
        switch (lanes) { \
            case 4:  LAUNCH_SPMV(CT, 4,  AC, FD); break; \
            case 8:  LAUNCH_SPMV(CT, 8,  AC, FD); break; \
            case 16: LAUNCH_SPMV(CT, 16, AC, FD); break; \
            case 32: LAUNCH_SPMV(CT, 32, AC, FD); break; \
            case 64: LAUNCH_SPMV(CT, 64, AC, FD); break; \
            default: throw std::runtime_error("spmv: lanes must be 4/8/16/32/64"); }
    #define DISPATCH_AC(CT) \
        if (accum) { if (fuse) { DISPATCH_L(CT, true, true) } else { DISPATCH_L(CT, true, false) } } \
        else       { if (fuse) { DISPATCH_L(CT, false, true) } else { DISPATCH_L(CT, false, false) } }
    if (col64) { DISPATCH_AC(long) } else { DISPATCH_AC(int) }
    #undef DISPATCH_AC
    #undef DISPATCH_L
    #undef LAUNCH_SPMV
    check_hip("spmv");
    if (fuse)
        reduce_partials(partials, (int)blocks, scal, dotslot, dot_accum, stream);
}

void spmv_binned(long rowbase, uintptr_t rowptr, uintptr_t colidx, int col64,
                 uintptr_t vals, uintptr_t x, uintptr_t y, uintptr_t rowlist,
                 const std::vector<std::array<long, 3>>& bins,
                 bool accum, uintptr_t partials, uintptr_t scal,
                 int dotslot, bool dot_accum, uintptr_t stream) {
    const bool fuse = partials != 0 && dotslot >= 0;
    long poff = 0;
    for (const auto& bin : bins) {
        const long start = bin[0], count = bin[1];
        const int lanes = (int)bin[2];
        if (count == 0) continue;
        const int rows_per_block = BLOCK / lanes;
        long blocks = (count + rows_per_block - 1) / rows_per_block;
        if (blocks > 3072) blocks = 3072;
        if (poff + blocks > MAXG)
            throw std::runtime_error("spmv_binned: partials overflow");
        dim3 g((unsigned)blocks), b(BLOCK);
        const int* rl = (const int*)rowlist + start;
        double* pp = (double*)partials + poff;
        #define LAUNCH_BIN(CT, L, AC, FD) \
            hipLaunchKernelGGL((spmv_csr_vector<CT, L, AC, FD, true>), g, b, 0, \
                S(stream), count, rowbase, (const long*)rowptr, \
                (const CT*)colidx, (const double*)vals, (const double*)x, \
                (double*)y, pp, rl)
        #define DISPATCH_BL(CT, AC, FD) \
            switch (lanes) { \
                case 4:  LAUNCH_BIN(CT, 4,  AC, FD); break; \
                case 8:  LAUNCH_BIN(CT, 8,  AC, FD); break; \
                case 16: LAUNCH_BIN(CT, 16, AC, FD); break; \
                case 32: LAUNCH_BIN(CT, 32, AC, FD); break; \
                case 64: LAUNCH_BIN(CT, 64, AC, FD); break; \
                default: throw std::runtime_error("spmv_binned: lanes 4/8/16/32/64"); }
        #define DISPATCH_BA(CT) \
            if (accum) { if (fuse) { DISPATCH_BL(CT, true, true) } else { DISPATCH_BL(CT, true, false) } } \
            else       { if (fuse) { DISPATCH_BL(CT, false, true) } else { DISPATCH_BL(CT, false, false) } }
        if (col64) { DISPATCH_BA(long) } else { DISPATCH_BA(int) }
        #undef DISPATCH_BA
        #undef DISPATCH_BL
        #undef LAUNCH_BIN
        if (fuse) poff += blocks;
    }
    check_hip("spmv_binned");
    if (fuse && poff > 0)
        reduce_partials(partials, (int)poff, scal, dotslot, dot_accum, stream);
}

void spmv_sell(long nslices, long nrows, long rowbase, uintptr_t sellptr,
               uintptr_t cols, int col64, uintptr_t vals, uintptr_t x,
               uintptr_t y, bool accum, uintptr_t partials, uintptr_t scal,
               int dotslot, bool dot_accum, int variant, uintptr_t perm,
               uintptr_t stream) {
    if (nrows == 0) return;
    long blocks = (nslices * WAVE + BLOCK - 1) / BLOCK;
    if (blocks > MAXG) blocks = MAXG;
    const bool fuse = partials != 0 && dotslot >= 0;
    dim3 g((unsigned)blocks), b(BLOCK);
    if (perm != 0) {
        #define LAUNCH_PERM_U(CT, AC, FD, U) \
            hipLaunchKernelGGL((k_spmv_sell<CT, AC, FD, true, false, U, true>), \
                g, b, 0, S(stream), nslices, nrows, rowbase, \
                (const long*)sellptr, (const CT*)cols, (const double*)vals, \
                (const double*)x, (double*)y, (double*)partials, (const int*)perm)
        #define LAUNCH_PERM(CT, AC, FD) \
            if (variant & SELL_U8) { LAUNCH_PERM_U(CT, AC, FD, 8); } \
            else { LAUNCH_PERM_U(CT, AC, FD, 4); }
        #define DISPP(CT) \
            if (accum) { if (fuse) { LAUNCH_PERM(CT, true, true); } else { LAUNCH_PERM(CT, true, false); } } \
            else       { if (fuse) { LAUNCH_PERM(CT, false, true); } else { LAUNCH_PERM(CT, false, false); } }
        if (col64) { DISPP(long) } else { DISPP(int) }
        #undef DISPP
        #undef LAUNCH_PERM
        #undef LAUNCH_PERM_U
        check_hip("spmv_sell_perm");
        if (fuse)
            reduce_partials(partials, (int)blocks, scal, dotslot, dot_accum, stream);
        return;
    }
    #define LAUNCH_SELL(CT, AC, FD, NT, SWZ, U) \
        hipLaunchKernelGGL((k_spmv_sell<CT, AC, FD, NT, SWZ, U>), g, b, 0, S(stream), \
            nslices, nrows, rowbase, (const long*)sellptr, (const CT*)cols, \
            (const double*)vals, (const double*)x, (double*)y, (double*)partials)
    #define DISP_V(CT, AC, FD) \
        switch (variant & (SELL_NT | SELL_SWZ | SELL_U8)) { \
            case 0:                               LAUNCH_SELL(CT, AC, FD, false, false, 4); break; \
            case SELL_NT:                         LAUNCH_SELL(CT, AC, FD, true,  false, 4); break; \
            case SELL_SWZ:                        LAUNCH_SELL(CT, AC, FD, false, true,  4); break; \
            case SELL_NT | SELL_SWZ:              LAUNCH_SELL(CT, AC, FD, true,  true,  4); break; \
            case SELL_U8:                         LAUNCH_SELL(CT, AC, FD, false, false, 8); break; \
            case SELL_U8 | SELL_NT:               LAUNCH_SELL(CT, AC, FD, true,  false, 8); break; \
            case SELL_U8 | SELL_SWZ:              LAUNCH_SELL(CT, AC, FD, false, true,  8); break; \
            default:                              LAUNCH_SELL(CT, AC, FD, true,  true,  8); break; }
    #define DISP2(CT) \
        if (accum) { if (fuse) { DISP_V(CT, true, true) } else { DISP_V(CT, true, false) } } \
        else       { if (fuse) { DISP_V(CT, false, true) } else { DISP_V(CT, false, false) } }
    if (col64) { DISP2(long) } else { DISP2(int) }
    #undef DISP2
    #undef DISP_V
    #undef LAUNCH_SELL
    check_hip("spmv_sell");
    if (fuse)
        reduce_partials(partials, (int)blocks, scal, dotslot, dot_accum, stream);
}

void zero_scalars(uintptr_t scal, int i0, int count, uintptr_t stream) {
    hipLaunchKernelGGL(k_zero_scalars, dim3(1), dim3(BLOCK), 0, S(stream),
                       (double*)scal, i0, count);
    check_hip("zero_scalars");
}

void cg_prep_pt(uintptr_t scal, uintptr_t stream) {
    hipLaunchKernelGGL(k_cg_prep_pt, dim3(1), dim3(64), 0, S(stream), (double*)scal);
    check_hip("cg_prep_pt");
}

void cg_prep_rr(uintptr_t scal, uintptr_t stream) {
    hipLaunchKernelGGL(k_cg_prep_rr, dim3(1), dim3(64), 0, S(stream), (double*)scal);
    check_hip("cg_prep_rr");
}

void dot(uintptr_t x, uintptr_t y, long n, uintptr_t partials, uintptr_t scal,
         int slot, bool accumulate, uintptr_t stream) {
    long blocks = elem_grid(n);
    hipLaunchKernelGGL(k_dot, dim3((unsigned)blocks), dim3(BLOCK), 0, S(stream),
                       (const double*)x, (const double*)y, n, (double*)partials);
    check_hip("dot");
    reduce_partials(partials, (int)blocks, scal, slot, accumulate, stream);
}

void dot2(uintptr_t r, uintptr_t w, long n, uintptr_t partials, uintptr_t scal,
          bool accumulate, uintptr_t stream) {
    long blocks = elem_grid(n);
    hipLaunchKernelGGL(k_dot2, dim3((unsigned)blocks), dim3(BLOCK), 0, S(stream),
                       (const double*)r, (const double*)w, n, (double*)partials);
    check_hip("dot2");
    hipLaunchKernelGGL(k_reduce_partials2, dim3(1), dim3(BLOCK), 0, S(stream),
                       (const double*)partials, (int)blocks, (double*)scal,
                       accumulate ? 1 : 0);
    check_hip("dot2_reduce");
}

void axpy_ratio(uintptr_t y, uintptr_t x, long n, uintptr_t scal, int num, int den,
                double sign, uintptr_t stream) {
    hipLaunchKernelGGL(k_axpy_ratio, dim3((unsigned)elem_grid(n)), dim3(BLOCK), 0, S(stream),
                       (double*)y, (const double*)x, n, (const double*)scal, num, den, sign);
    check_hip("axpy_ratio");
}

void daypx_ratio(uintptr_t y, uintptr_t x, long n, uintptr_t scal, int num, int den,
                 uintptr_t stream) {
    hipLaunchKernelGGL(k_daypx_ratio, dim3((unsigned)elem_grid(n)), dim3(BLOCK), 0, S(stream),
                       (double*)y, (const double*)x, n, (const double*)scal, num, den);
    check_hip("daypx_ratio");
}

void pcg_fused_update(uintptr_t r, uintptr_t x, uintptr_t p, uintptr_t t,
                      uintptr_t z, uintptr_t dinv, long n, uintptr_t scal,
                      uintptr_t partials, uintptr_t stream) {
    long blocks = elem_grid(n);
    hipLaunchKernelGGL(k_pcg_fused_update, dim3((unsigned)blocks), dim3(BLOCK),
                       0, S(stream), (double*)r, (double*)x, (const double*)p,
                       (const double*)t, (double*)z, (const double*)dinv,
                       n, (const double*)scal, (double*)partials);
    check_hip("pcg_fused_update");
    hipLaunchKernelGGL(k_pcg_finalize, dim3(1), dim3(BLOCK), 0, S(stream),
                       (const double*)partials, (int)blocks, (double*)scal);
    check_hip("pcg_finalize");
}

void cg_fused_update(uintptr_t r, uintptr_t x, uintptr_t p, uintptr_t t, long n,
                     uintptr_t scal, uintptr_t partials, uintptr_t stream) {
    long blocks = elem_grid(n);
    hipLaunchKernelGGL(k_cg_fused_update, dim3((unsigned)blocks), dim3(BLOCK), 0, S(stream),
                       (double*)r, (double*)x, (const double*)p, (const double*)t,
                       n, (const double*)scal, (double*)partials);
    check_hip("cg_fused_update");
    hipLaunchKernelGGL(k_cg_finalize, dim3(1), dim3(BLOCK), 0, S(stream),
                       (const double*)partials, (int)blocks, (double*)scal);
    check_hip("cg_finalize");
}

long sell_pipe(long nslices, long nrows_pass, long rowbase, long border_base,
               uintptr_t sellptr, uintptr_t cols, uintptr_t vals,
               uintptr_t w_old, uintptr_t qpart, uintptr_t z, uintptr_t t,
               uintptr_t p, uintptr_t x, uintptr_t r, uintptr_t w_new,
               uintptr_t scal, int first, uintptr_t partials,
               long partials_off, bool mato, uintptr_t stream) {
    if (nrows_pass == 0) return 0;
    long blocks = (nslices * WAVE + BLOCK - 1) / BLOCK;
    const long cap = (partials_off == 0) ? (MAXG - 1024) : (MAXG - partials_off);
    if (blocks > cap) blocks = cap;
    dim3 g((unsigned)blocks), b(BLOCK);
    #define LP(MATO) \
        hipLaunchKernelGGL((k_sell_pipe<int, true, 8, MATO>), g, b, 0, S(stream), \
            nslices, nrows_pass, rowbase, border_base, (const long*)sellptr, \
            (const int*)cols, (const double*)vals, (const double*)w_old, \
            (double*)qpart, (double*)z, (double*)t, (double*)p, (double*)x, \
            (double*)r, (double*)w_new, (const double*)scal, first, \
            (double*)partials, partials_off)
    if (mato) { LP(true); } else { LP(false); }
    #undef LP
    check_hip("sell_pipe");
    return blocks;
}

void pipelined_finalize(uintptr_t partials, int nblocks, uintptr_t scal, int first,
                        uintptr_t stream) {
    hipLaunchKernelGGL(k_pipelined_finalize, dim3(1), dim3(BLOCK), 0, S(stream),
                       (const double*)partials, nblocks, (double*)scal, first);
    check_hip("pipelined_finalize");
}

void pipelined_fused(uintptr_t z, uintptr_t t, uintptr_t p, uintptr_t x, uintptr_t r,
                     uintptr_t w, uintptr_t q, long n, uintptr_t scal, int first,
                     uintptr_t partials, bool nt_update, uintptr_t stream) {
    long blocks = elem_grid(n);
    if (nt_update)
        hipLaunchKernelGGL(k_pipelined_fused<true>, dim3((unsigned)blocks), dim3(BLOCK), 0, S(stream),
                           (double*)z, (double*)t, (double*)p, (double*)x, (double*)r,
                           (double*)w, (const double*)q, n, (const double*)scal, first,
                           (double*)partials);
    else
        hipLaunchKernelGGL(k_pipelined_fused<false>, dim3((unsigned)blocks), dim3(BLOCK), 0, S(stream),
                           (double*)z, (double*)t, (double*)p, (double*)x, (double*)r,
                           (double*)w, (const double*)q, n, (const double*)scal, first,
                           (double*)partials);
    check_hip("pipelined_fused");
    hipLaunchKernelGGL(k_pipelined_finalize, dim3(1), dim3(BLOCK), 0, S(stream),
                       (const double*)partials, (int)blocks, (double*)scal, first);
    check_hip("pipelined_finalize");
}

int cg_device(long nslices, long nrows, uintptr_t sellptr, uintptr_t cols,
              int col64, uintptr_t vals, uintptr_t b, uintptr_t x, uintptr_t r,
              uintptr_t p, uintptr_t t, uintptr_t scal, uintptr_t partials,
              uintptr_t out2, uintptr_t barrier_state,
              int maxits, double res_atol, double res_rtol,
              uintptr_t stream, int hier) {
    int dev = 0;
    hipGetDevice(&dev);
    hipDeviceProp_t props;
    hipGetDeviceProperties(&props, dev);
    const void* kern = col64 ? (const void*)&k_cg_device<long>
                             : (const void*)&k_cg_device<int>;
    int blocks_per_cu = 0;
    hipError_t oe = hipOccupancyMaxActiveBlocksPerMultiprocessor(
        &blocks_per_cu, kern, BLOCK, 0);
    if (oe != hipSuccess || blocks_per_cu < 1) blocks_per_cu = 1;
    if (blocks_per_cu > 4) blocks_per_cu = 4;
    long grid = (long)props.multiProcessorCount * blocks_per_cu;
    long need = (nslices * WAVE + BLOCK - 1) / BLOCK;
    if (grid > need) grid = need;
    if (grid > MAXG) grid = MAXG;
    if (hier < 0) hier = grid >= 64 ? 1 : 0;
    for (;;) {
        void* args[] = {&nslices, &nrows, (void*)&sellptr, (void*)&cols,
                        (void*)&vals, (void*)&b, (void*)&x, (void*)&r,
                        (void*)&p, (void*)&t, (void*)&scal, (void*)&partials,
                        (void*)&out2, (void*)&barrier_state,
                        &maxits, &res_atol, &res_rtol, &hier};
        hipError_t e = hipLaunchCooperativeKernel(
            kern, dim3((unsigned)grid), dim3(BLOCK), args, 0, S(stream));
        if (e == hipSuccess) break;
        if (e == hipErrorCooperativeLaunchTooLarge && grid > props.multiProcessorCount) {
            (void)hipGetLastError();
            grid -= props.multiProcessorCount;
            continue;
        }
        throw std::runtime_error(std::string("cg_device launch: ") + hipGetErrorString(e));
    }
    check_hip("cg_device");
    return (int)grid;
}

void atomic_probe(uintptr_t y, uintptr_t idx, uintptr_t v, long nnz,
                  int mode, uintptr_t stream) {
    const long blocks = elem_grid(nnz, 8);
    hipLaunchKernelGGL(k_atomic_probe, dim3((unsigned)blocks), dim3(BLOCK), 0,
                       S(stream), (double*)y, (const int*)idx,
                       (const double*)v, nnz, mode);
    check_hip("atomic_probe");
}

void pack_gather(uintptr_t sendbuf, uintptr_t x, uintptr_t idx, int idx64, long n,
                 uintptr_t stream) {
    if (n == 0) return;
    dim3 g((unsigned)elem_grid(n, 1)), b(BLOCK);
    if (idx64)
        hipLaunchKernelGGL(k_pack_gather<long>, g, b, 0, S(stream),
                           (double*)sendbuf, (const double*)x, (const long*)idx, n);
    else
        hipLaunchKernelGGL(k_pack_gather<int>, g, b, 0, S(stream),
                           (double*)sendbuf, (const double*)x, (const int*)idx, n);
    check_hip("pack_gather");
}

PYBIND11_MODULE(_acg_kernels, m) {
    m.doc() = "acg_amd gfx950 HIP kernels";
    m.def("spmv", &spmv);
    m.def("spmv_binned", &spmv_binned);
    m.def("spmv_sell", &spmv_sell);
    m.def("zero_scalars", &zero_scalars);
    m.def("cg_prep_pt", &cg_prep_pt);
    m.def("cg_prep_rr", &cg_prep_rr);
    m.def("dot", &dot);
    m.def("dot2", &dot2);
    m.def("axpy_ratio", &axpy_ratio);
    m.def("daypx_ratio", &daypx_ratio);
    m.def("cg_fused_update", &cg_fused_update);
    m.def("pcg_fused_update", &pcg_fused_update);
    m.def("pipelined_fused", &pipelined_fused);
    m.def("sell_pipe", &sell_pipe);
    m.def("pipelined_finalize", &pipelined_finalize);
    m.def("pack_gather", &pack_gather);
    m.def("atomic_probe", &atomic_probe);
    m.def("cg_device", &cg_device);
    m.def("stencil_rowlen", &stencil_rowlen);
    m.def("stencil_fill", &stencil_fill);
    m.def("spmv_bsell", &spmv_bsell);
    m.def("spmv_bsell_daypx", &spmv_bsell_daypx);
    m.def("stencil_blocklen", &stencil_blocklen);
    m.def("stencil_bfill", &stencil_bfill);
    m.def("stencil_spmv", &stencil_spmv);
    m.def("stencil_pipe", &stencil_pipe);
    m.def("stencil_spmv7", &stencil_spmv7);
    m.def("stencil_pipe7", &stencil_pipe7);
    m.attr("S_RR") = S_RR;
    m.attr("S_PT") = S_PT;
    m.attr("S_RR_PREV") = S_RR_PREV;
    m.attr("S_BNRM2") = S_BNRM2;
    m.attr("S_GAMMA") = S_GAMMA;
    m.attr("S_DELTA") = S_DELTA;
    m.attr("S_GAMMA_PREV") = S_GAMMA_PREV;
    m.attr("S_ALPHA_PREV") = S_ALPHA_PREV;
    m.attr("S_NSLOTS") = S_NSLOTS;
    m.attr("MAXG") = MAXG;
}
```

acg_amd/ops/torch_ref.py:

```python

from __future__ import annotations

import torch

S_RR, S_PT, S_RR_PREV, S_BNRM2 = 0, 1, 2, 3
S_GAMMA, S_DELTA, S_GAMMA_PREV, S_ALPHA_PREV = 4, 5, 6, 7
S_NSLOTS = 8
MAXG = 16384


def alloc_scalars(device="cpu") -> torch.Tensor:
    return torch.zeros(S_NSLOTS, dtype=torch.float64, device=device)


def alloc_partials(device="cpu") -> torch.Tensor:
    return torch.zeros(1, dtype=torch.float64, device=device)


def spmv(rowptr, colidx, vals, x, y, *, rowbase: int = 0, accum: bool = False,
         partials=None, scal=None, dotslot: int = -1, dot_accum: bool = True) -> None:
    nrows = rowptr.numel() - 1
    if nrows <= 0:
        return
    counts = rowptr[1:] - rowptr[:-1]
    rows = torch.repeat_interleave(torch.arange(nrows, dtype=torch.int64,
                                                device=rowptr.device), counts)
    prod = vals * x[colidx.long()]
    contrib = torch.zeros(nrows, dtype=torch.float64, device=x.device)
    contrib.index_add_(0, rows, prod)
    sl = slice(rowbase, rowbase + nrows)
    if accum:
        y[sl] += contrib
    else:
        y[sl] = contrib
    if scal is not None and dotslot >= 0:
        d = torch.dot(x[sl], contrib)
        scal[dotslot] = scal[dotslot] + d if dot_accum else d


def spmv_binned(rowptr, colidx, vals, rowlist, bins, x, y, *, rowbase: int = 0,
                accum: bool = False, partials=None, scal=None,
                dotslot: int = -1, dot_accum: bool = True) -> None:
    if rowlist.numel() == 0:
        return
    spmv(rowptr, colidx, vals, x, y, rowbase=rowbase, accum=accum,
         partials=partials, scal=scal, dotslot=dotslot, dot_accum=dot_accum)


def zero_scalars(scal, i0: int = 0, count=None) -> None:
    scal[i0:i0 + (count if count is not None else scal.numel() - i0)] = 0.0


def sell_from_csr(rowptr, colidx, vals, C: int = 64, sigma: int = 1):
    import numpy as np

    rowptr = np.asarray(rowptr)
    colidx = np.asarray(colidx)
    vals = np.asarray(vals)
    nrows = len(rowptr) - 1
    nslices = (nrows + C - 1) // C
    counts = np.diff(rowptr)
    perm = None
    rowof = np.arange(nslices * C, dtype=np.int64)
    if sigma > 1 and nrows:
        win = sigma * C
        order = np.empty(nrows, dtype=np.int64)
        for w0 in range(0, nrows, win):
            w1 = min(w0 + win, nrows)
            sub = np.argsort(-counts[w0:w1], kind="stable")
            order[w0:w1] = w0 + sub
        rowof = np.full(nslices * C, nrows, dtype=np.int64)
        rowof[:nrows] = order
        perm = rowof.astype(np.int32)
    cpad = np.zeros(nslices * C, dtype=np.int64)
    valid = rowof < nrows
    cpad[valid] = counts[rowof[valid]]
    slice_len = cpad.reshape(nslices, C).max(axis=1)
    sellptr = np.zeros(nslices + 1, dtype=np.int64)
    np.cumsum(slice_len * C, out=sellptr[1:])
    total = int(sellptr[-1])
    slice_of_p = np.repeat(np.arange(nslices, dtype=np.int64), slice_len * C)
    lane = (np.arange(total, dtype=np.int64) - sellptr[slice_of_p]) % C
    defrow = np.minimum(rowof[np.minimum(slice_of_p * C + lane,
                                         nslices * C - 1)], nrows - 1)
    cols = defrow.astype(colidx.dtype)
    svals = np.zeros(total, dtype=np.float64)
    nnz = len(colidx)
    if perm is not None:
        invperm = np.empty(nslices * C, dtype=np.int64)
        invperm[rowof] = np.arange(nslices * C, dtype=np.int64)
        sellrow = invperm[:nrows]
    else:
        sellrow = np.arange(nrows, dtype=np.int64)
    rows = np.repeat(sellrow, counts)
    within = np.arange(nnz, dtype=np.int64) - rowptr[np.repeat(
        np.arange(nrows, dtype=np.int64), counts)]
    dst = sellptr[rows // C] + within * C + rows % C
    cols[dst] = colidx
    svals[dst] = vals
    if perm is not None:
        return sellptr, cols, svals, perm
    return sellptr, cols, svals


def sellcsr_split(rowptr, colidx, vals, cut: int = 192, C: int = 64,
                  window: int = 0, bucket: int = 8):
    import numpy as np

    rowptr = np.asarray(rowptr)
    colidx = np.asarray(colidx)
    vals = np.asarray(vals)
    n = len(rowptr) - 1
    lens = np.diff(rowptr)
    order = np.argsort(-lens, kind="stable")
    slens = lens[order]
    nlong = int(np.searchsorted(-slens, -int(cut) - 1, side="right"))
    long_rows = order[:nlong].astype(np.int32)
    short_rows = order[nlong:].astype(np.int64)
    if bucket and nlong and cut >= 96:
        ll = lens[long_rows.astype(np.int64)]
        fc = colidx[rowptr[long_rows.astype(np.int64)]]
        bw = max(bucket * 8, 64)
        long_rows = long_rows[np.lexsort((fc, -((ll + bw - 1) // bw)))]
    if window and len(short_rows):
        sr = np.sort(short_rows)
        out = np.empty_like(sr)
        for w0 in range(0, len(sr), window):
            w1 = min(w0 + window, len(sr))
            sub = np.argsort(-lens[sr[w0:w1]], kind="stable")
            out[w0:w1] = sr[w0:w1][sub]
        short_rows = out
    elif bucket and len(short_rows):
        sl = lens[short_rows]
        firstcol = np.where(sl > 0, colidx[rowptr[short_rows]], 0)
        bkt = (sl + bucket - 1) // bucket
        order2 = np.lexsort((firstcol, -bkt))
        short_rows = short_rows[order2]
    nshort = len(short_rows)
    nslices = (nshort + C - 1) // C
    padlens = np.zeros(nslices * C, dtype=np.int64)
    padlens[:nshort] = lens[short_rows]
    slice_len = padlens.reshape(nslices, C).max(axis=1) if nslices else \
        np.zeros(0, np.int64)
    sellptr = np.zeros(nslices + 1, dtype=np.int64)
    np.cumsum(slice_len * C, out=sellptr[1:])
    total = int(sellptr[-1])
    perm = np.full(nslices * C, n, dtype=np.int32)
    perm[:nshort] = short_rows
    slice_of_p = np.repeat(np.arange(nslices, dtype=np.int64), slice_len * C)
    lane = (np.arange(total, dtype=np.int64) - sellptr[slice_of_p]) % C
    defrow = np.minimum(perm[np.minimum(slice_of_p * C + lane,
                                        max(nslices * C - 1, 0))], n - 1)
    cols = defrow.astype(colidx.dtype)
    svals = np.zeros(total, dtype=np.float64)
    counts = lens[short_rows]
    rows_rep = np.repeat(np.arange(nshort, dtype=np.int64), counts)
    excl = np.zeros(nshort, dtype=np.int64)
    if nshort:
        np.cumsum(counts[:-1], out=excl[1:])
    within = np.arange(int(counts.sum()), dtype=np.int64) - excl[rows_rep]
    src = np.repeat(rowptr[short_rows], counts) + within
    dst = sellptr[rows_rep // C] + within * C + rows_rep % C
    cols[dst] = colidx[src]
    svals[dst] = vals[src]
    return sellptr, cols, svals, perm, long_rows, nshort


def bsell_from_csr(rowptr, colidx, vals, dof: int, C: int = 64):
    import numpy as np

    rowptr = np.asarray(rowptr)
    colidx = np.asarray(colidx, dtype=np.int64)
    vals = np.asarray(vals)
    nrows = len(rowptr) - 1
    if dof < 2 or nrows % dof:
        return None
    nnodes = nrows // dof
    nnz = len(colidx)
    rows = np.repeat(np.arange(nrows, dtype=np.int64), np.diff(rowptr))
    try:
        from ..host import _acg_host as H

        blocks_per_node, bcols, inv = (np.asarray(a) for a in
                                       H.bsell_blocks(rowptr, colidx, dof))
        nblocks = len(bcols)
        bnode = np.repeat(np.arange(nnodes, dtype=np.int64), blocks_per_node)
    except ImportError:
        node = rows // dof
        bcol_of_entry = colidx // dof
        key = node * (np.int64(1) << 32) | bcol_of_entry.astype(np.int64)
        uk, inv = np.unique(key, return_inverse=True)
        nblocks = len(uk)
        bnode = (uk >> 32).astype(np.int64)
        bcols = (uk & 0xFFFFFFFF).astype(np.int64)
        blocks_per_node = np.bincount(bnode, minlength=nnodes)
    density = nnz / (nblocks * dof * dof)
    nslices = (nnodes + C - 1) // C
    padlen = np.zeros(nslices * C, dtype=np.int64)
    padlen[:nnodes] = blocks_per_node
    slice_len = padlen.reshape(nslices, C).max(axis=1)
    bptr = np.zeros(nslices + 1, dtype=np.int64)
    np.cumsum(slice_len * C, out=bptr[1:])
    btotal = int(bptr[-1])
    slice_of_p = np.repeat(np.arange(nslices, dtype=np.int64), slice_len * C)
    lane = (np.arange(btotal, dtype=np.int64) - bptr[slice_of_p]) % C
    bcol = np.minimum(slice_of_p * C + lane, nnodes - 1).astype(np.int32)
    bvals = np.zeros(btotal * dof * dof, dtype=np.float64)
    starts = np.zeros(nnodes + 1, dtype=np.int64)
    np.cumsum(blocks_per_node, out=starts[1:])
    within = np.arange(nblocks, dtype=np.int64) - starts[bnode]
    bdst = bptr[bnode // C] + within * C + bnode % C
    bcol[bdst] = bcols.astype(np.int32)
    entry_block_dst = bdst[inv]
    k = (rows % dof) * dof + colidx % dof
    lane_p = entry_block_dst % C
    base_p = entry_block_dst - lane_p
    D2 = dof * dof
    even = D2 & ~1
    off = np.where(k < even, (k >> 1) * (2 * C) + lane_p * 2 + (k & 1),
                   even * C + lane_p)
    vdst = base_p * D2 + off
    bvals[vdst] = vals
    return bptr, bcol, bvals, density


def spmv_sell(sellptr, cols, vals, nrows, x, y, *, rowbase: int = 0,
              accum: bool = False, partials=None, scal=None,
              dotslot: int = -1, dot_accum: bool = True, C: int = 64,
              variant=None, perm=None) -> None:
    nslices = sellptr.numel() - 1
    assert (nrows + C - 1) // C == nslices, \
        f"SELL structure was built with a different chunk size than C={C}"
    contrib = torch.zeros(nrows, dtype=torch.float64, device=x.device)
    for s in range(nslices):
        base = int(sellptr[s])
        L = (int(sellptr[s + 1]) - base) // C
        block = (vals[base:base + L * C].view(L, C)
                 * x[cols[base:base + L * C].long()].view(L, C)).sum(dim=0)
        if perm is not None:
            rowof = perm[s * C:(s + 1) * C].long()
            ok = rowof < nrows
            contrib[rowof[ok]] = block[ok]
            continue
        hi = min(C, nrows - s * C)
        contrib[s * C:s * C + hi] = block[:hi]
    sl = slice(rowbase, rowbase + nrows)
    if accum:
        y[sl] += contrib
    else:
        y[sl] = contrib
    if scal is not None and dotslot >= 0:
        d = torch.dot(x[sl], contrib)
        scal[dotslot] = scal[dotslot] + d if dot_accum else d


def _bsell_contrib(bptr, bcol, bvals, nnodes: int, dof: int, xg, C: int = 64):
    D2 = dof * dof
    even = D2 & ~1
    nslices = bptr.numel() - 1
    assert (nnodes + C - 1) // C == nslices, \
        f"BSELL structure was built with a different chunk size than C={C}"
    contrib = torch.zeros(nnodes * dof, dtype=torch.float64, device=xg.device)
    for s in range(nslices):
        b0 = int(bptr[s])
        L = (int(bptr[s + 1]) - b0) // C
        acc = torch.zeros(C, dof, dtype=torch.float64, device=xg.device)
        if L:
            cb = bcol[b0:b0 + L * C].view(L, C).long()
            v = bvals[b0 * D2:(b0 + L * C) * D2].view(L, D2 * C)
            for k in range(D2):
                if k < even:
                    lo = (k >> 1) * 2 * C + (k & 1)
                    a = v[:, lo:(k >> 1) * 2 * C + 2 * C:2]
                else:
                    a = v[:, even * C:even * C + C]
                acc[:, k // dof] += (a * xg[cb * dof + k % dof]).sum(dim=0)
        hi = min(C, nnodes - s * C)
        contrib[s * C * dof:(s * C + hi) * dof] = acc[:hi].reshape(-1)
    return contrib


def spmv_bsell(bptr, bcol, bvals, nnodes: int, dof: int, x, y, *,
               partials=None, scal=None, dotslot: int = -1,
               dot_accum: bool = True) -> None:
    if bptr.numel() - 1 <= 0:
        return
    n = nnodes * dof
    contrib = _bsell_contrib(bptr, bcol, bvals, nnodes, dof, x)
    y[:n] = contrib
    if scal is not None and dotslot >= 0:
        d = torch.dot(x[:n], contrib)
        scal[dotslot] = scal[dotslot] + d if dot_accum else d


def spmv_bsell_daypx(bptr, bcol, bvals, nnodes: int, dof: int, pold, rvec,
                     pnew, y, scal, partials, dotslot: int) -> None:
    if bptr.numel() - 1 <= 0:
        return
    n = nnodes * dof
    beta = _sdiv(float(scal[S_RR]), float(scal[S_RR_PREV]))
    pn = beta * pold[:n] + rvec[:n]
    contrib = _bsell_contrib(bptr, bcol, bvals, nnodes, dof, pn)
    pnew[:n] = pn
    y[:n] = contrib
    scal[dotslot] = torch.dot(pn, contrib)


def cg_prep_pt(scal) -> None:
    scal[S_PT] = 0.0


def cg_prep_rr(scal) -> None:
    scal[S_RR_PREV] = scal[S_RR].clone()


def dot(x, y, partials, scal, slot, n=None, accumulate=False) -> None:
    n = x.numel() if n is None else n
    d = torch.dot(x[:n], y[:n])
    scal[slot] = scal[slot] + d if accumulate else d


def dot2(r, w, partials, scal, n, accumulate=False) -> None:
    g = torch.dot(r[:n], r[:n])
    d = torch.dot(w[:n], r[:n])
    if accumulate:
        scal[S_GAMMA] += g
        scal[S_DELTA] += d
    else:
        scal[S_GAMMA] = g
        scal[S_DELTA] = d


def _sdiv(a, b):
    return a / b if float(b) != 0.0 else torch.zeros_like(a) if torch.is_tensor(a) else 0.0


def axpy_ratio(y, x, scal, num, den, sign=1.0, n=None) -> None:
    n = y.numel() if n is None else n
    a = sign * _sdiv(float(scal[num]), float(scal[den]))
    y[:n] += a * x[:n]


def daypx_ratio(y, x, scal, num, den, n=None) -> None:
    n = y.numel() if n is None else n
    b = _sdiv(float(scal[num]), float(scal[den]))
    y[:n] = b * y[:n] + x[:n]


def cg_fused_update(r, x, p, t, scal, partials, n) -> None:
    alpha = _sdiv(float(scal[S_RR]), float(scal[S_PT]))
    r[:n] -= alpha * t[:n]
    x[:n] += alpha * p[:n]
    scal[S_RR_PREV] = scal[S_RR].clone()
    scal[S_RR] = torch.dot(r[:n], r[:n])


def pcg_fused_update(r, x, p, t, z, dinv, scal, partials, n) -> None:
    alpha = _sdiv(float(scal[S_RR]), float(scal[S_PT]))
    r[:n] -= alpha * t[:n]
    x[:n] += alpha * p[:n]
    z[:n] = dinv[:n] * r[:n]
    scal[S_RR_PREV] = scal[S_RR].clone()
    scal[S_RR] = torch.dot(r[:n], z[:n])
    scal[S_GAMMA] = torch.dot(r[:n], r[:n])


def _pipelined_coeffs(scal, first: bool):
    gamma = float(scal[S_GAMMA])
    delta = float(scal[S_DELTA])
    if first:
        return 0.0, _sdiv(gamma, delta)
    beta = _sdiv(gamma, float(scal[S_GAMMA_PREV]))
    alpha = _sdiv(gamma, delta - beta * _sdiv(gamma, float(scal[S_ALPHA_PREV])))
    return beta, alpha


def pipelined_fused(z, t, p, x, r, w, q, scal, partials, n, first: bool,
                    nt_update: bool = True) -> None:
    beta, alpha = _pipelined_coeffs(scal, first)
    z[:n] = q[:n] + beta * z[:n]
    t[:n] = w[:n] + beta * t[:n]
    p[:n] = r[:n] + beta * p[:n]
    x[:n] += alpha * p[:n]
    r[:n] -= alpha * t[:n]
    w[:n] -= alpha * z[:n]
    scal[S_GAMMA_PREV] = scal[S_GAMMA].clone()
    scal[S_ALPHA_PREV] = alpha
    scal[S_GAMMA] = torch.dot(r[:n], r[:n])
    scal[S_DELTA] = torch.dot(w[:n], r[:n])


def sell_pipe(sellptr, cols, vals, nrows_pass: int, rowbase: int,
              border_base: int, w_old, qpart, z, t, p, x, r, w_new, scal,
              first: bool, partials, partials_off: int, mato: bool,
              C: int = 64) -> int:
    if nrows_pass == 0:
        return 0
    q = torch.zeros(rowbase + nrows_pass, dtype=torch.float64,
                    device=w_old.device)
    spmv_sell(sellptr, cols, vals, nrows_pass, w_old, q, rowbase=rowbase, C=C)
    beta, alpha = _pipelined_coeffs(scal, first)
    rows = torch.arange(rowbase, rowbase + nrows_pass, device=w_old.device)
    if mato:
        upd = rows
        qu = q[upd] + qpart[upd - border_base]
    else:
        defer = rows[rows >= border_base]
        qpart[defer - border_base] = q[defer]
        upd = rows[rows < border_base]
        qu = q[upd]
    zi = qu + beta * z[upd]
    ti = w_old[upd] + beta * t[upd]
    pi = r[upd] + beta * p[upd]
    z[upd] = zi
    t[upd] = ti
    p[upd] = pi
    x[upd] += alpha * pi
    rn = r[upd] - alpha * ti
    wn = w_old[upd] - alpha * zi
    r[upd] = rn
    w_new[upd] = wn
    partials[partials_off] = torch.dot(rn, rn)
    partials[MAXG + partials_off] = torch.dot(wn, rn)
    return 1


def pipelined_finalize(partials, nblocks: int, scal, first: bool) -> None:
    _, alpha = _pipelined_coeffs(scal, first)
    g = partials[:nblocks].sum()
    d = partials[MAXG:MAXG + nblocks].sum()
    scal[S_GAMMA_PREV] = scal[S_GAMMA].clone()
    scal[S_ALPHA_PREV] = alpha
    scal[S_GAMMA] = g
    scal[S_DELTA] = d


def pack_gather(sendbuf, x, idx) -> None:
    torch.index_select(x, 0, idx.long(), out=sendbuf)
```

acg_amd/solvers/hip.py:

```python

from __future__ import annotations

import math
import os
import time

import numpy as np
import torch

from ..dist.halo import HaloExchange
from ..ops import gpu_ops as ops
from ..part.subdomain import LocalSystem
from .base import SolveResult, cg_flops_per_iter


class CGSolverHIP:

    def __init__(self, local: LocalSystem, comm=None, device=None,
                 lanes: int | None = None, use_sell: bool = True,
                 profile: bool = False, matfree: bool = False,
                 force_format: str | None = None):
        self.local = local
        self.comm = comm
        if device is None:
            device = comm.device if comm is not None and comm.device is not None \
                else torch.device("cuda", 0)
        self.device = torch.device(device)
        L = local

        def up(a, dtype=None):
            t = torch.from_numpy(np.ascontiguousarray(a))
            return t.to(self.device, non_blocking=True)

        self.n = L.nowned
        self.nlocal = L.nowned + L.nghost
        self.sell = None
        self.sellO = None
        self.sell_perm = None
        self.A_rowptr = self.A_colidx = self.A_vals = None
        self.O_rowptr = self.O_colidx = self.O_vals = None
        self.lanesA = self.lanesO = lanes or 16
        self.bsell = None
        self.hybrid = None
        self.matfree = None
        if matfree:
            mf = getattr(L, "mf_tables", None)
            if mf is None:
                raise ValueError(
                    "matfree=True needs a device-generated dof=1 stencil "
                    "system (gen.device_slab with spec dof==1)")
            self.matfree = mf
        if hasattr(L, "A_sell"):
            self.sell = L.A_sell
            self.sellO = L.O_sell
            self.bsell = getattr(L, "A_bsell", None)
            if self.sell is None and self.matfree is None:
                raise ValueError("system generated with operator=False "
                                 "requires matfree=True")
        else:
            self.A_rowptr = up(L.A_rowptr)
            self.A_colidx = up(L.A_colidx)
            self.A_vals = up(L.A_vals)
            self.O_rowptr = up(L.O_rowptr)
            self.O_colidx = up(L.O_colidx)
            self.O_vals = up(L.O_vals)
            mean_nnz = L.nnzA / max(L.nowned, 1)
            self.lanesA = lanes or ops.pick_lanes(mean_nnz)
            mean_nnzO = L.nnzO / max(L.nborder, 1)
            self.lanesO = lanes or ops.pick_lanes(mean_nnzO)
            self._pick_format(L, up, use_sell, force_format)
        self.can_megafuse = (
            self.matfree is not None
            or (self.sell is not None and self.sell_perm is None
                and self.sell[1].dtype == torch.int32
                and (L.nnzO == 0 or (self.sellO is not None
                                     and self.sellO[1].dtype == torch.int32))))
        self.megafuse_auto = (self.can_megafuse
                              and (self.matfree is not None
                                   or L.nnzA / max(L.nowned, 1) <= 16.0))
        self.halo = HaloExchange(L.halo, L.nowned, self.device, comm)
        self.scal = ops.alloc_scalars(self.device)
        self.partials = ops.alloc_partials(self.device)
        from .profiling import EventProfiler

        self.prof = EventProfiler(profile)
        self.comm_stream = torch.cuda.Stream(self.device)
        self.allred_stream = torch.cuda.Stream(self.device)
        self.copy_stream = torch.cuda.Stream(self.device)
        self._rr_host = torch.zeros(1, dtype=torch.float64, pin_memory=True)
        self._ev_p = torch.cuda.Event()
        self._ev_recv = torch.cuda.Event()
        self._ev_rr = torch.cuda.Event()
        self.niterations_total = 0
        self._ws: dict = {}
        self._graphs: dict = {}
        self._nstag = 0

    def _pick_format(self, L, up, use_sell: bool, force: str | None) -> None:
        from ..ops.torch_ref import bsell_from_csr, sell_from_csr

        if L.nowned == 0:
            return

        def mk_hybrid(cut: int | None = None):
            if cut is None:
                cut = int(os.environ.get("ACG_HYBRID_CUT", "192"))
            window = int(os.environ.get("ACG_HYBRID_WINDOW", "0"))
            bucket = int(os.environ.get("ACG_HYBRID_BUCKET", "8"))
            sp_, cols, svals, perm, rowlist, bins = ops.build_sellcsr_hybrid(
                L.A_rowptr, L.A_colidx, L.A_vals, cut=cut, window=window,
                bucket=bucket)
            self.hybrid = {
                "sellptr": up(sp_) if sp_ is not None else None,
                "cols": up(cols) if sp_ is not None else None,
                "svals": up(svals) if sp_ is not None else None,
                "perm": up(perm) if sp_ is not None else None,
                "rowlist": up(rowlist) if len(rowlist) else None,
                "bins": bins,
            }
            if L.nnzO > 0:
                rlO, binsO = ops.build_row_bins(L.O_rowptr)
                self.hybrid["rowlistO"] = up(rlO)
                self.hybrid["binsO"] = binsO

        def mk_binned():
            rowlist, bins = ops.build_row_bins(L.A_rowptr)
            self.hybrid = {"sellptr": None, "cols": None, "svals": None,
                           "perm": None, "rowlist": up(rowlist),
                           "bins": bins}

        def mk_sell(sigma):
            out = sell_from_csr(L.A_rowptr, L.A_colidx, L.A_vals, sigma=sigma)
            if sigma > 1:
                sellptr, scols, svals, perm = out
                self.sell_perm = up(perm)
            else:
                sellptr, scols, svals = out
                self.sell_perm = None
            self.sell = (up(sellptr), up(scols), up(svals))
            if L.nnzO > 0:
                optr, ocols, ovals = sell_from_csr(L.O_rowptr, L.O_colidx,
                                                   L.O_vals)
                self.sellO = (up(optr), up(ocols), up(ovals))
            return (int(sellptr[-1]) - L.nnzA) / max(L.nnzA, 1)

        def mk_bsell():
            for dof_try in (4, 3, 2):
                out = bsell_from_csr(L.A_rowptr, L.A_colidx, L.A_vals, dof_try)
                if out is None:
                    continue
                bptr_h, bcol_h, bvals_h, density = out
                if density >= 0.75:
                    self.bsell = (up(bptr_h), up(bcol_h), up(bvals_h), dof_try)
                    return True
            return False

        if force == "csr":
            return
        if force == "hybrid":
            mk_hybrid()
            return
        if force == "binned":
            mk_binned()
            return
        if force == "sell":
            mk_sell(1)
        elif force == "sigma":
            mk_sell(4096)
        elif force == "bsell":
            if not mk_bsell():
                raise ValueError("force_format=bsell: no dense dof x dof "
                                 "block structure (density < 0.75)")
        elif use_sell:
            waste = mk_sell(1)
            if waste > 0.3:
                self.sell = self.sellO = self.sell_perm = None
                waste = mk_sell(16)
                if waste > 0.5:
                    self.sell = self.sellO = self.sell_perm = None
                    mk_hybrid()
            mk_bsell()
        if self.sell is not None or self.bsell is not None:
            self.A_rowptr = self.A_colidx = self.A_vals = None

    def _workspace(self, key: str, names) -> dict:
        ws = self._ws.setdefault(key, {})
        for nm, nghost in names:
            if nm not in ws:
                n = self.nlocal if nghost else self.n
                off = 520 * self._nstag
                self._nstag += 1
                buf = torch.zeros(n + off, dtype=torch.float64,
                                  device=self.device)
                ws[nm] = buf[off:] if off else buf
        return ws


    def _allreduce_slot(self, slot: int, count: int = 1):
        if self.comm is not None and self.comm.size > 1:
            self.comm.allreduce_(self.scal[slot:slot + count])

    def _spmv_overlapped(self, xfull: torch.Tensor, y: torch.Tensor,
                         fuse_dotslot: int = -1):
        L = self.local
        have_halo = self.comm is not None and self.comm.size > 1
        cur = torch.cuda.current_stream(self.device)
        halo_span = None
        if have_halo:
            self._ev_p.record(cur)
            self.comm_stream.wait_event(self._ev_p)
            halo_span = self.prof.span("halo", self.comm_stream)
            halo_span.__enter__()
            with torch.cuda.stream(self.comm_stream):
                self.halo.begin(xfull)
        fuse = dict(partials=self.partials,
                    scal=self.scal if fuse_dotslot >= 0 else None,
                    dotslot=fuse_dotslot)
        with self.prof.span("spmvA"):
            if self.matfree is not None:
                ops.stencil_spmv(self.matfree, self.n, 0, xfull, y,
                                 mato=False, dot_accum=False, **fuse)
            elif self.bsell is not None:
                bptr, bcol, bvals, dof = self.bsell
                ops.spmv_bsell(bptr, bcol, bvals, self.n // dof, dof,
                               xfull, y, dot_accum=False, **fuse)
            elif self.sell is not None:
                sellptr, scols, svals = self.sell
                ops.spmv_sell(sellptr, scols, svals, self.n, xfull, y,
                              accum=False, perm=self.sell_perm,
                              dot_accum=False, **fuse)
            elif self.hybrid is not None:
                h = self.hybrid
                have_sell = h["sellptr"] is not None
                if have_sell:
                    ops.spmv_sell(h["sellptr"], h["cols"], h["svals"],
                                  self.n, xfull, y, accum=False,
                                  perm=h["perm"], dot_accum=False, **fuse)
                if h["rowlist"] is not None:
                    ops.spmv_binned(self.A_rowptr, self.A_colidx,
                                    self.A_vals, h["rowlist"], h["bins"],
                                    xfull, y, accum=False,
                                    dot_accum=have_sell, **fuse)
            else:
                ops.spmv(self.A_rowptr, self.A_colidx, self.A_vals, xfull, y,
                         lanes=self.lanesA, accum=False, dot_accum=False,
                         **fuse)
        if have_halo:
            with torch.cuda.stream(self.comm_stream):
                self.halo.end()
                self._ev_recv.record(self.comm_stream)
            if halo_span is not None:
                halo_span.__exit__(None, None, None)
            cur.wait_event(self._ev_recv)
        if L.nborder > 0 and self.local.nnzO > 0:
            with self.prof.span("spmvO"):
                if self.matfree is not None:
                    ops.stencil_spmv(self.matfree, L.nborder, L.ninterior,
                                     xfull, y, mato=True, **fuse)
                elif self.sellO is not None:
                    optr, ocols, ovals = self.sellO
                    ops.spmv_sell(optr, ocols, ovals, L.nborder, xfull, y,
                                  rowbase=L.ninterior, accum=True, **fuse)
                elif self.hybrid is not None and "rowlistO" in self.hybrid:
                    ops.spmv_binned(self.O_rowptr, self.O_colidx, self.O_vals,
                                    self.hybrid["rowlistO"],
                                    self.hybrid["binsO"], xfull, y,
                                    rowbase=L.ninterior, accum=True, **fuse)
                else:
                    ops.spmv(self.O_rowptr, self.O_colidx, self.O_vals, xfull, y,
                             rowbase=L.ninterior, lanes=self.lanesO, accum=True,
                             **fuse)

    def _host_scalar(self, slot: int) -> float:
        cur = torch.cuda.current_stream(self.device)
        self._ev_rr.record(cur)
        self.copy_stream.wait_event(self._ev_rr)
        with torch.cuda.stream(self.copy_stream):
            self._rr_host.copy_(self.scal[slot:slot + 1], non_blocking=True)
        self.copy_stream.synchronize()
        return float(self._rr_host[0])

    def _vec(self, nghost: bool = False) -> torch.Tensor:
        return torch.zeros(self.nlocal if nghost else self.n,
                           dtype=torch.float64, device=self.device)


    def solve(self, b: torch.Tensor, x: torch.Tensor, maxits: int = 100,
              res_atol: float = 0.0, res_rtol: float = 1e-9,
              use_graph: bool | None = None,
              fold_daypx: bool | None = None,
              diff_atol: float = 0.0, diff_rtol: float = 0.0) -> SolveResult:
        res = SolveResult(solver="cg-hip", maxits=maxits, res_atol=res_atol,
                          res_rtol=res_rtol,
                          nranks=self.comm.size if self.comm else 1)
        n = self.n
        S = ops
        scal = self.scal
        ws = self._workspace("classic", [("r", False), ("t", False),
                                         ("p", True), ("xi", True)])
        r, t, p, xi = ws["r"], ws["t"], ws["p"], ws["xi"]
        xi.copy_(x)
        torch.cuda.synchronize(self.device)
        t0 = time.perf_counter()
        S.dot(b, b, self.partials, scal, S.S_BNRM2, n=n)
        self._allreduce_slot(S.S_BNRM2)
        self._spmv_overlapped(xi, t)
        torch.sub(b[:n], t, out=r)
        p[:n] = r
        S.dot(r, r, self.partials, scal, S.S_RR, n=n)
        self._allreduce_slot(S.S_RR)
        bnrm2sqr = self._host_scalar(S.S_BNRM2)
        rr = self._host_scalar(S.S_RR)
        res.bnrm2 = math.sqrt(max(bnrm2sqr, 0.0))
        res.r0nrm2 = math.sqrt(max(rr, 0.0))
        rtol2 = max(res_atol, res_rtol * res.bnrm2) ** 2
        dtol = max(diff_atol, diff_rtol * res.bnrm2)
        if rtol2 > 0 and rr <= rtol2 and dtol == 0.0:
            res.converged = True
            res.rnrm2 = math.sqrt(rr)
            res.tsolve = time.perf_counter() - t0
            return res
        converged = False
        serial = self.comm is None or self.comm.size == 1
        if dtol > 0:
            converged = self._solve_diffmode(res, r, t, p, xi, rtol2, dtol,
                                             maxits)
            return self._finish_classic(res, x, xi, converged, rtol2, t0)
        fold = (serial and self.bsell is not None and self.local.nnzO == 0
                and fold_daypx is True)
        if fold:
            p2 = self._workspace("classic", [("p2", True)])["p2"]
            scal[S.S_RR_PREV] = math.inf
        if use_graph is None:
            use_graph = not serial
        graph_ok = use_graph and serial and not self.prof.enabled and not fold
        graph = self._graphs.get("classic") if graph_ok else None
        dist_key = "classic:dist"
        dist_failed_key = "classic:capture_failed"
        dist_graph_ok = (use_graph and not serial and not self.prof.enabled
                         and not fold
                         and getattr(self.comm, "can_capture", False)
                         and os.environ.get("ACG_DIST_GRAPH", "1") != "0"
                         and not self._graphs.get(dist_failed_key, False))
        dgraph = self._graphs.get(dist_key) if dist_graph_ok else None
        LAG = 2
        hostbuf = [torch.zeros(1, dtype=torch.float64, pin_memory=True)
                   for _ in range(LAG + 1)]
        evdone = [torch.cuda.Event() for _ in range(LAG + 1)]

        def body(k: int = 0):
            if fold:
                bptr, bcol, bvals, dof = self.bsell
                pold, pnew = (p, p2) if k % 2 == 0 else (p2, p)
                with self.prof.span("spmvA"):
                    S.spmv_bsell_daypx(bptr, bcol, bvals, n // dof, dof,
                                       pold, r, pnew, t, scal,
                                       self.partials, S.S_PT)
                with self.prof.span("update_classic"):
                    S.cg_fused_update(r, xi, pnew, t, scal, self.partials, n)
                return
            self._spmv_overlapped(p, t, fuse_dotslot=S.S_PT)
            with self.prof.span("allreduce"):
                self._allreduce_slot(S.S_PT)
            with self.prof.span("update_classic"):
                S.cg_fused_update(r, xi, p, t, scal, self.partials, n)
            with self.prof.span("allreduce"):
                self._allreduce_slot(S.S_RR)
            with self.prof.span("daypx"):
                S.daypx_ratio(p, r, scal, S.S_RR, S.S_RR_PREV, n=n)

        def read_rr(j):
            evdone[j % (LAG + 1)].synchronize()
            return float(hostbuf[j % (LAG + 1)][0])

        def check(j):
            nonlocal rr, converged
            rr = read_rr(j)
            if not math.isfinite(rr):
                raise FloatingPointError(f"CG diverged: rr={rr} at it {j + 1}")
            if rtol2 > 0 and rr <= rtol2:
                converged = True
                res.niterations = j + 1
                return True
            return False

        k = 0
        cur = torch.cuda.current_stream(self.device)
        while k < maxits:
            if k >= LAG and check(k - LAG):
                break
            if graph is not None:
                graph.replay()
            elif dgraph is not None and k > 0:
                dgraph.replay()
            else:
                body(k)
                if graph_ok and k == 1:
                    graph = torch.cuda.CUDAGraph()
                    with torch.cuda.graph(graph):
                        body()
                    self._graphs["classic"] = graph
                elif dist_graph_ok and k == 2 and dgraph is None:
                    try:
                        gg = torch.cuda.CUDAGraph()
                        with torch.cuda.graph(gg):
                            body()
                        dgraph = gg
                        self._graphs[dist_key] = gg
                    except Exception as e:
                        self._graphs[dist_failed_key] = True
                        torch.cuda.synchronize(self.device)
                        if self.comm is None or self.comm.rank == 0:
                            print(f"[acg_amd] classic distributed graph "
                                  f"capture unavailable ({type(e).__name__});"
                                  f" eager iterations",
                                  file=__import__("sys").stderr)
            j = k % (LAG + 1)
            hostbuf[j].copy_(scal[S.S_RR:S.S_RR + 1], non_blocking=True)
            evdone[j].record(cur)
            k += 1
            res.niterations = k
        if not converged:
            for j in range(max(maxits - LAG, 0), maxits):
                if check(j):
                    break
        return self._finish_classic(res, x, xi, converged, rtol2, t0)

    def _solve_diffmode(self, res, r, t, p, xi, rtol2: float, dtol: float,
                        maxits: int) -> bool:
        S = ops
        n = self.n
        scal = self.scal
        converged = False
        for k in range(maxits):
            self._spmv_overlapped(p, t, fuse_dotslot=S.S_PT)
            self._allreduce_slot(S.S_PT)
            S.dot(p, p, self.partials, scal, S.S_GAMMA, n=n)
            self._allreduce_slot(S.S_GAMMA)
            S.cg_fused_update(r, xi, p, t, scal, self.partials, n)
            self._allreduce_slot(S.S_RR)
            res.niterations = k + 1
            rr_old = self._host_scalar(S.S_RR_PREV)
            pt = self._host_scalar(S.S_PT)
            pp = self._host_scalar(S.S_GAMMA)
            rr = self._host_scalar(S.S_RR)
            if not math.isfinite(rr):
                raise FloatingPointError(f"CG diverged: rr={rr} at it {k + 1}")
            alpha = rr_old / pt if pt != 0.0 else 0.0
            dx = abs(alpha) * math.sqrt(max(pp, 0.0))
            if (rtol2 > 0 and rr <= rtol2) or dx <= dtol:
                converged = True
                break
            S.daypx_ratio(p, r, scal, S.S_RR, S.S_RR_PREV, n=n)
        return converged

    def _finish_classic(self, res, x, xi, converged: bool, rtol2: float,
                        t0: float):
        S = ops
        torch.cuda.synchronize(self.device)
        res.tsolve = time.perf_counter() - t0
        x.copy_(xi)
        rr = self._host_scalar(S.S_RR)
        res.rnrm2 = math.sqrt(max(rr, 0.0))
        res.converged = converged or (rtol2 > 0 and rr <= rtol2)
        nnz_full = self.local.nnzA + self.local.nnzO
        res.nflops = res.niterations * cg_flops_per_iter(nnz_full, self.n)
        res.halo_bytes_sent = self.halo.bytes_sent
        res.halo_msgs_sent = self.halo.nmsgs_sent
        self.niterations_total += res.niterations
        if self.prof.enabled:
            from .profiling import annotate_op_stats

            idxb = None
            if self.matfree is not None:
                idxb = -8.0
            elif self.bsell is not None:
                idxb = 4.0 / (self.bsell[3] ** 2)
            annotate_op_stats(res, self.local, self.prof.collect(),
                              idx_bytes_per_nnz=idxb)
            self.prof.reset()
        return res


    def solve_device(self, b: torch.Tensor, x: torch.Tensor, maxits: int = 100,
                     res_atol: float = 0.0, res_rtol: float = 1e-9) -> SolveResult:
        if self.comm is not None and self.comm.size > 1:
            from ..utils.errors import AcgError, ErrCode

            raise AcgError(ErrCode.NOT_SUPPORTED,
                           "device-side CG is single-GPU (reference parity)")
        if self.sell is None or self.sell_perm is not None:
            from ..utils.errors import AcgError, ErrCode

            raise AcgError(ErrCode.NOT_SUPPORTED,
                           "device-side CG requires the unpermuted SELL format")
        res = SolveResult(solver="cg-hip-device", maxits=maxits,
                          res_atol=res_atol, res_rtol=res_rtol, nranks=1)
        n = self.n
        r = self._vec()
        t = self._vec()
        p = self._vec(nghost=True)
        out2 = torch.zeros(2, dtype=torch.int32, device=self.device)
        barrier_state = torch.zeros(ops.BAR_STATE_WORDS, dtype=torch.int32,
                                    device=self.device)
        sellptr, scols, svals = self.sell
        torch.cuda.synchronize(self.device)
        t0 = time.perf_counter()
        ops.cg_device(sellptr, scols, svals, n, b, x, r, p, t, self.scal,
                      self.partials, out2, barrier_state, maxits, res_atol,
                      res_rtol)
        torch.cuda.synchronize(self.device)
        res.tsolve = time.perf_counter() - t0
        S = ops
        res.bnrm2 = math.sqrt(max(float(self.scal[S.S_BNRM2]), 0.0))
        res.r0nrm2 = math.sqrt(max(float(self.scal[S.S_RR_PREV]), 0.0))
        res.rnrm2 = math.sqrt(max(float(self.scal[S.S_RR]), 0.0))
        res.niterations = int(out2[0])
        conv = int(out2[1])
        if conv < 0:
            raise RuntimeError("device CG grid barrier timed out (residency?)")
        res.converged = bool(conv)
        nnz_full = self.local.nnzA + self.local.nnzO
        res.nflops = res.niterations * cg_flops_per_iter(nnz_full, n)
        self.niterations_total += res.niterations
        return res


    def solve_jacobi(self, b: torch.Tensor, x: torch.Tensor,
                     maxits: int = 100, res_atol: float = 0.0,
                     res_rtol: float = 1e-9) -> SolveResult:
        L = self.local
        if getattr(L, "A_rowptr", None) is None or not hasattr(L, "owned_global"):
            from ..utils.errors import AcgError, ErrCode

            raise AcgError(ErrCode.NOT_SUPPORTED,
                           "jacobi PCG needs the host CSR arrays "
                           "(file/extracted systems; not device-generated "
                           "slabs)")
        res = SolveResult(solver="cg-hip-jacobi", maxits=maxits,
                          res_atol=res_atol, res_rtol=res_rtol,
                          nranks=self.comm.size if self.comm else 1)
        n = self.n
        S = ops
        scal = self.scal
        if "jacobi_dinv" not in self._ws:
            rows = np.repeat(np.arange(n, dtype=np.int64),
                             np.diff(L.A_rowptr))
            dmask = rows == L.A_colidx
            d = np.zeros(n, dtype=np.float64)
            d[rows[dmask]] = L.A_vals[dmask]
            if (d == 0).any():
                from ..utils.errors import AcgError, ErrCode

                raise AcgError(ErrCode.INVALID_VALUE,
                               "jacobi preconditioner needs a full diagonal")
            self._ws["jacobi_dinv"] = torch.from_numpy(1.0 / d).to(self.device)
        dinv = self._ws["jacobi_dinv"]
        ws = self._workspace("jacobi", [("r", False), ("t", False),
                                        ("z", False), ("p", True),
                                        ("xi", True)])
        r, t, z, p, xi = ws["r"], ws["t"], ws["z"], ws["p"], ws["xi"]
        xi.copy_(x)
        torch.cuda.synchronize(self.device)
        t0 = time.perf_counter()
        S.dot(b, b, self.partials, scal, S.S_BNRM2, n=n)
        self._allreduce_slot(S.S_BNRM2)
        self._spmv_overlapped(xi, t)
        torch.sub(b[:n], t, out=r)
        torch.mul(r, dinv, out=z)
        p[:n] = z
        S.dot(r, z, self.partials, scal, S.S_RR, n=n)
        self._allreduce_slot(S.S_RR)
        S.dot(r, r, self.partials, scal, S.S_GAMMA, n=n)
        self._allreduce_slot(S.S_GAMMA)
        res.bnrm2 = math.sqrt(max(self._host_scalar(S.S_BNRM2), 0.0))
        rr = self._host_scalar(S.S_GAMMA)
        res.r0nrm2 = math.sqrt(max(rr, 0.0))
        rtol2 = max(res_atol, res_rtol * res.bnrm2) ** 2
        converged = rtol2 > 0 and rr <= rtol2
        k = 0
        while not converged and k < maxits:
            self._spmv_overlapped(p, t, fuse_dotslot=S.S_PT)
            self._allreduce_slot(S.S_PT)
            S.pcg_fused_update(r, xi, p, t, z, dinv, scal, self.partials, n)
            self._allreduce_slot(S.S_RR)
            self._allreduce_slot(S.S_GAMMA)
            rr = self._host_scalar(S.S_GAMMA)
            k += 1
            res.niterations = k
            if not math.isfinite(rr):
                raise FloatingPointError(f"jacobi PCG diverged at it {k}")
            if rtol2 > 0 and rr <= rtol2:
                converged = True
                break
            S.daypx_ratio(p, z, scal, S.S_RR, S.S_RR_PREV, n=n)
        torch.cuda.synchronize(self.device)
        res.tsolve = time.perf_counter() - t0
        x.copy_(xi)
        res.rnrm2 = math.sqrt(max(rr, 0.0))
        res.converged = converged
        nnz_full = L.nnzA + L.nnzO
        res.nflops = res.niterations * (cg_flops_per_iter(nnz_full, n) + 3.0 * n)
        res.halo_bytes_sent = self.halo.bytes_sent
        res.halo_msgs_sent = self.halo.nmsgs_sent
        self.niterations_total += res.niterations
        return res


    def solve_pipelined(self, b: torch.Tensor, x: torch.Tensor, maxits: int = 100,
                        res_atol: float = 0.0, res_rtol: float = 1e-9,
                        use_graph: bool | None = None,
                        megafuse: bool | None = None) -> SolveResult:
        res = SolveResult(solver="cg-hip-pipelined", maxits=maxits,
                          res_atol=res_atol, res_rtol=res_rtol,
                          nranks=self.comm.size if self.comm else 1)
        n = self.n
        S = ops
        L = self.local
        scal = self.scal
        mega = self.megafuse_auto if megafuse is None else (megafuse and self.can_megafuse)
        wskey = f"pipelined{'_mega' if mega else ''}"
        names = [("r", True), ("w", True), ("z", False), ("t", False),
                 ("p", False), ("tmp", False), ("xi", True)]
        names += [("w2", True)] if mega else [("q", False)]
        ws = self._workspace(wskey, names)
        r, w, z, t, p, tmp, xi = (ws["r"], ws["w"], ws["z"], ws["t"],
                                  ws["p"], ws["tmp"], ws["xi"])
        w2 = ws.get("w2")
        q = ws.get("q")
        if mega and "qpart" not in ws:
            ws["qpart"] = torch.zeros(max(L.nborder, 1), dtype=torch.float64,
                                      device=self.device)
        qpart = ws.get("qpart")
        xi.copy_(x)
        for v in (z, t, p):
            v.zero_()
        torch.cuda.synchronize(self.device)
        t0 = time.perf_counter()
        S.dot(b, b, self.partials, scal, S.S_BNRM2, n=n)
        self._allreduce_slot(S.S_BNRM2)
        self._spmv_overlapped(xi, tmp)
        torch.sub(b[:n], tmp, out=r[:n])
        self._spmv_overlapped(r, w)
        res.bnrm2 = math.sqrt(max(self._host_scalar(S.S_BNRM2), 0.0))
        rtol2 = max(res_atol, res_rtol * res.bnrm2) ** 2
        S.dot2(r, w, self.partials, scal, n)
        converged = False
        gamma_host = None
        serial = self.comm is None or self.comm.size == 1
        if use_graph is None:
            use_graph = not serial
        graph_ok = use_graph and serial and not self.prof.enabled
        graph = self._graphs.get(wskey) if graph_ok and not mega else None
        graphs = (self._graphs.get(wskey, [None, None])
                  if graph_ok and mega else [None, None])

        def mega_body(wa, wb, first):
            have_halo = not serial
            cur = torch.cuda.current_stream(self.device)
            if have_halo:
                self._ev_p.record(cur)
                self.comm_stream.wait_event(self._ev_p)
                with torch.cuda.stream(self.comm_stream):
                    self.halo.begin(wa)
            border_base = L.ninterior if L.nnzO > 0 else n
            if self.matfree is not None:
                nbA = S.stencil_pipe(self.matfree, n, 0, border_base, wa,
                                     qpart, z, t, p, xi, r, wb, scal, first,
                                     self.partials, 0, mato=False)
            else:
                sp, sc, sv = self.sell
                nbA = S.sell_pipe(sp, sc, sv, n, 0, border_base, wa, qpart,
                                  z, t, p, xi, r, wb, scal, first,
                                  self.partials, 0, mato=False)
            nb = nbA
            if have_halo:
                with torch.cuda.stream(self.comm_stream):
                    self.halo.end()
                    self._ev_recv.record(self.comm_stream)
                cur.wait_event(self._ev_recv)
            if L.nnzO > 0:
                if self.matfree is not None:
                    nbO = S.stencil_pipe(self.matfree, L.nborder, L.ninterior,
                                         L.ninterior, wa, qpart, z, t, p, xi,
                                         r, wb, scal, first, self.partials,
                                         nbA, mato=True)
                else:
                    op_, oc, ov = self.sellO
                    nbO = S.sell_pipe(op_, oc, ov, L.nborder, L.ninterior,
                                      L.ninterior, wa, qpart, z, t, p, xi, r,
                                      wb, scal, first, self.partials, nbA,
                                      mato=True)
                nb += nbO
            S.pipelined_finalize(self.partials, nb, scal, first)
        LAG = 1
        hostbuf = [torch.zeros(1, dtype=torch.float64, pin_memory=True)
                   for _ in range(LAG + 1)]
        evdone = [torch.cuda.Event() for _ in range(LAG + 1)]

        def issue_gamma_copy(k):
            cur = torch.cuda.current_stream(self.device)
            j = k % (LAG + 1)
            hostbuf[j].copy_(scal[S.S_GAMMA:S.S_GAMMA + 1], non_blocking=True)
            evdone[j].record(cur)

        def read_gamma(j):
            evdone[j % (LAG + 1)].synchronize()
            return float(hostbuf[j % (LAG + 1)][0])

        def check(j):
            nonlocal gamma_host, converged
            gamma_host = read_gamma(j)
            if j == 0:
                res.r0nrm2 = math.sqrt(max(gamma_host, 0.0))
            if not math.isfinite(gamma_host):
                raise FloatingPointError(f"pipelined CG diverged at it {j}")
            if rtol2 > 0 and gamma_host <= rtol2:
                converged = True
                res.rnrm2 = math.sqrt(max(gamma_host, 0.0))
                res.niterations = j
                return True
            return False

        ev_gd = torch.cuda.Event()
        ev_ar = torch.cuda.Event()
        dist_key = wskey + ":dist"
        dist_failed_key = wskey + ":capture_failed"
        dist_graph_ok = (use_graph and not serial and not self.prof.enabled
                         and getattr(self.comm, "can_capture", False)
                         and os.environ.get("ACG_DIST_GRAPH", "1") != "0"
                         and not self._graphs.get(dist_failed_key, False))
        dgraph = self._graphs.get(dist_key) if dist_graph_ok and not mega else None
        dgraphs = (self._graphs.get(dist_key, [None, None])
                   if dist_graph_ok and mega else [None, None])

        if "gsnap" not in ws:
            ws["gsnap"] = torch.zeros(1, dtype=torch.float64,
                                      device=self.device)
        gsnap = ws["gsnap"]

        def body_dist(wa=None, wb=None):
            if mega:
                self._allreduce_slot(S.S_GAMMA, 2)
                gsnap.copy_(scal[S.S_GAMMA:S.S_GAMMA + 1])
                mega_body(wa, wb, False)
            else:
                cur = torch.cuda.current_stream(self.device)
                ev_gd.record(cur)
                self.allred_stream.wait_event(ev_gd)
                with torch.cuda.stream(self.allred_stream):
                    self._allreduce_slot(S.S_GAMMA, 2)
                    ev_ar.record(self.allred_stream)
                self._spmv_overlapped(w, q)
                cur.wait_event(ev_ar)
                gsnap.copy_(scal[S.S_GAMMA:S.S_GAMMA + 1])
                S.pipelined_fused(z, t, p, xi, r, w, q, scal, self.partials,
                                  n, False)

        def try_capture_dist(kk):
            nonlocal dgraph
            if self._graphs.get(dist_failed_key):
                return
            try:
                gg = torch.cuda.CUDAGraph()
                if mega:
                    wa, wb = (w, w2) if kk % 2 == 0 else (w2, w)
                    with torch.cuda.graph(gg):
                        body_dist(wa, wb)
                    dgraphs[kk % 2] = gg
                    self._graphs[dist_key] = dgraphs
                else:
                    with torch.cuda.graph(gg):
                        body_dist()
                    dgraph = gg
                    self._graphs[dist_key] = gg
            except Exception as e:
                self._graphs[dist_failed_key] = True
                torch.cuda.synchronize(self.device)
                if (self.comm is None or self.comm.rank == 0):
                    print(f"[acg_amd] distributed graph capture unavailable "
                          f"({type(e).__name__}); eager iterations",
                          file=__import__("sys").stderr)

        k = 0
        while k < maxits:
            first = (k == 0)
            if not serial and dist_graph_ok:
                g = dgraphs[k % 2] if mega else dgraph
                if g is not None and k > 0:
                    if k >= LAG and check(k - LAG):
                        break
                    g.replay()
                    cur = torch.cuda.current_stream(self.device)
                    j = k % (LAG + 1)
                    hostbuf[j].copy_(gsnap, non_blocking=True)
                    evdone[j].record(cur)
                    k += 1
                    res.niterations = k
                    continue
            overlap_ar = (not serial) and not mega
            if overlap_ar:
                cur = torch.cuda.current_stream(self.device)
                ev_gd.record(cur)
                self.allred_stream.wait_event(ev_gd)
                with torch.cuda.stream(self.allred_stream):
                    with self.prof.span("allreduce", self.allred_stream):
                        self._allreduce_slot(S.S_GAMMA, 2)
                    ev_ar.record(self.allred_stream)
            else:
                with self.prof.span("allreduce"):
                    self._allreduce_slot(S.S_GAMMA, 2)
            if k >= LAG and check(k - LAG):
                break
            if overlap_ar:
                j = k % (LAG + 1)
                self.copy_stream.wait_event(ev_ar)
                with torch.cuda.stream(self.copy_stream):
                    hostbuf[j].copy_(scal[S.S_GAMMA:S.S_GAMMA + 1],
                                     non_blocking=True)
                    evdone[j].record(self.copy_stream)
            else:
                issue_gamma_copy(k)
            if mega:
                wa, wb = (w, w2) if k % 2 == 0 else (w2, w)
                g = graphs[k % 2]
                if g is not None and k > 0:
                    g.replay()
                else:
                    mega_body(wa, wb, first)
                    if graph_ok and graphs[k % 2] is None and k in (2, 3):
                        gg = torch.cuda.CUDAGraph()
                        with torch.cuda.graph(gg):
                            mega_body(wa, wb, False)
                        graphs[k % 2] = gg
                        self._graphs[wskey] = graphs
            elif graph is not None and k > 0:
                graph.replay()
            else:
                self._spmv_overlapped(w, q)
                if overlap_ar:
                    cur2 = torch.cuda.current_stream(self.device)
                    cur2.wait_event(ev_ar)
                    cur2.wait_event(evdone[k % (LAG + 1)])
                with self.prof.span("update"):
                    S.pipelined_fused(z, t, p, xi, r, w, q, scal, self.partials,
                                      n, first)
                if graph_ok and graph is None and k == 2:
                    graph = torch.cuda.CUDAGraph()
                    with torch.cuda.graph(graph):
                        self._spmv_overlapped(w, q)
                        S.pipelined_fused(z, t, p, xi, r, w, q, scal,
                                          self.partials, n, False)
                    self._graphs[wskey] = graph
            if dist_graph_ok and not serial and (
                    (mega and k in (2, 3) and dgraphs[k % 2] is None)
                    or (not mega and k == 2 and dgraph is None)):
                try_capture_dist(k)
            k += 1
            res.niterations = k
        if not converged:
            for j in range(max(maxits - LAG, 0), maxits):
                if check(j):
                    break
        torch.cuda.synchronize(self.device)
        res.tsolve = time.perf_counter() - t0
        x.copy_(xi)
        if not converged and gamma_host is not None:
            res.rnrm2 = math.sqrt(max(gamma_host, 0.0))
        res.converged = converged
        nnz_full = self.local.nnzA + self.local.nnzO
        res.nflops = res.niterations * (cg_flops_per_iter(nnz_full, n) + 8.0 * n)
        res.halo_bytes_sent = self.halo.bytes_sent
        res.halo_msgs_sent = self.halo.nmsgs_sent
        self.niterations_total += res.niterations
        if self.prof.enabled:
            from .profiling import annotate_op_stats

            idxb = None
            if self.matfree is not None:
                idxb = -8.0
            elif self.bsell is not None:
                idxb = 4.0 / (self.bsell[3] ** 2)
            annotate_op_stats(res, self.local, self.prof.collect(),
                              idx_bytes_per_nnz=idxb)
            self.prof.reset()
        return res
```

Measured before the change: 1894 iter/s.

## Compress BSELL column indices to 16-bit with per-slice base and fuse CG tail

Stores BSELL block column indices as uint16 offsets from a per-slice int32 base, enabled by default, which cuts index traffic in the block SpMV and daypx kernels. The padded tail columns are set to a valid nearby node so the 16-bit offsets stay in range. Separately, the classic single-GPU CG path gets a fused tail: the SpMV leaves its partial dot products unreduced, one kernel reduces them and updates r while accumulating rr partials, and a second reduces those and updates x and p, saving separate reduction launches. The risk is that some slices span more than 65535 nodes (the assert checks dtype and shape, not range), and the solver here is pipelined CG, so the fused tail may not run.

```diff
diff --git a/acg_amd/gen/device_slab.py b/acg_amd/gen/device_slab.py
--- a/acg_amd/gen/device_slab.py
+++ b/acg_amd/gen/device_slab.py
@@ -162,6 +162,9 @@
                         zs_own.data_ptr(), pb.data_ptr(), offs.data_ptr(),
                         ksten, blocks.data_ptr(), bptr.data_ptr(),
                         bcol.data_ptr(), bvals.data_ptr(), stream)
+        tail = nown_nodes - (nbslices - 1) * 64
+        if tail < 64:
+            bcol[int(bptr[-2]):].view(-1, 64)[:, tail:] = nown_nodes - 1
         A_bsell = (bptr, bcol, bvals, dof)
 
     senders, recvcounts, rdispls = [], [], []
diff --git a/acg_amd/ops/gpu_ops.py b/acg_amd/ops/gpu_ops.py
--- a/acg_amd/ops/gpu_ops.py
+++ b/acg_amd/ops/gpu_ops.py
@@ -53,16 +53,17 @@
          lanes: int = 16, accum: bool = False,
          partials: torch.Tensor | None = None,
          scal: torch.Tensor | None = None, dotslot: int = -1,
-         dot_accum: bool = True) -> None:
+         dot_accum: bool = True, finalize: bool = True) -> int:
     nrows = rowptr.numel() - 1
     if nrows <= 0:
-        return
-    fuse = scal is not None and dotslot >= 0
-    K.spmv(nrows, rowbase, rowptr.data_ptr(), colidx.data_ptr(),
+        return 0
+    fuse = scal is not None and dotslot >= 0
+    return K.spmv(nrows, rowbase, rowptr.data_ptr(), colidx.data_ptr(),
            1 if colidx.dtype == torch.int64 else 0,
            vals.data_ptr(), x.data_ptr(), y.data_ptr(), lanes, accum,
            partials.data_ptr() if fuse else 0,
-           scal.data_ptr() if fuse else 0, dotslot, dot_accum, _stream())
+           scal.data_ptr() if fuse and finalize else 0, dotslot, dot_accum,
+           _stream())
 
 
 def build_row_bins(rowptr, max_lanes: int = 64):
@@ -119,18 +120,18 @@
                 *, rowbase: int = 0, accum: bool = False,
                 partials: torch.Tensor | None = None,
                 scal: torch.Tensor | None = None, dotslot: int = -1,
-                dot_accum: bool = True) -> None:
+                dot_accum: bool = True, finalize: bool = True) -> int:
     if rowlist.numel() == 0:
-        return
+        return 0
     assert rowlist.dtype == torch.int32
     fuse = scal is not None and dotslot >= 0
-    K.spmv_binned(rowbase, rowptr.data_ptr(), colidx.data_ptr(),
+    return K.spmv_binned(rowbase, rowptr.data_ptr(), colidx.data_ptr(),
                   1 if colidx.dtype == torch.int64 else 0,
                   vals.data_ptr(), x.data_ptr(), y.data_ptr(),
                   rowlist.data_ptr(), [list(b) for b in bins], accum,
                   partials.data_ptr() if fuse else 0,
-                  scal.data_ptr() if fuse else 0, dotslot, dot_accum,
-                  _stream())
+                  scal.data_ptr() if fuse and finalize else 0, dotslot,
+                  dot_accum, _stream())
 
 
 SELL_NT, SELL_SWZ, SELL_U8 = 1, 2, 4
@@ -143,57 +144,73 @@
               partials: torch.Tensor | None = None,
               scal: torch.Tensor | None = None, dotslot: int = -1,
               dot_accum: bool = True, variant: int | None = None,
-              perm: torch.Tensor | None = None) -> None:
+              perm: torch.Tensor | None = None,
+              finalize: bool = True) -> int:
     nslices = sellptr.numel() - 1
     if nslices <= 0:
-        return
+        return 0
     if variant is None:
         variant = DEFAULT_SELL_VARIANT
     fuse = scal is not None and dotslot >= 0
-    K.spmv_sell(nslices, nrows, rowbase, sellptr.data_ptr(), cols.data_ptr(),
+    return K.spmv_sell(nslices, nrows, rowbase, sellptr.data_ptr(), cols.data_ptr(),
                 1 if cols.dtype == torch.int64 else 0,
                 vals.data_ptr(), x.data_ptr(), y.data_ptr(), accum,
                 partials.data_ptr() if fuse else 0,
-                scal.data_ptr() if fuse else 0, dotslot, dot_accum,
-                variant, perm.data_ptr() if perm is not None else 0, _stream())
+                scal.data_ptr() if fuse and finalize else 0, dotslot,
+                dot_accum, variant, perm.data_ptr() if perm is not None else 0, _stream())
 
 
 def spmv_bsell(bptr: torch.Tensor, bcol: torch.Tensor, bvals: torch.Tensor,
                nnodes: int, dof: int, x: torch.Tensor, y: torch.Tensor, *,
                partials: torch.Tensor | None = None,
                scal: torch.Tensor | None = None, dotslot: int = -1,
-               dot_accum: bool = True) -> None:
+               dot_accum: bool = True, finalize: bool = True,
+               bbase: torch.Tensor | None = None) -> int:
     nslices = bptr.numel() - 1
     if nslices <= 0:
-        return
-    fuse = scal is not None and dotslot >= 0
-    K.spmv_bsell(nslices, nnodes, dof, bptr.data_ptr(), bcol.data_ptr(),
-                 bvals.data_ptr(), x.data_ptr(), y.data_ptr(),
-                 partials.data_ptr() if fuse else 0,
-                 scal.data_ptr() if fuse else 0, dotslot, dot_accum, _stream())
+        return 0
+    fuse = scal is not None and dotslot >= 0
+    pp = partials.data_ptr() if fuse else 0
+    sp = scal.data_ptr() if fuse and finalize else 0
+    if bbase is not None:
+        _check_idx16(bptr, bcol, bbase)
+        return K.spmv_bsell16(nslices, nnodes, dof, bptr.data_ptr(),
+                              bbase.data_ptr(), bcol.data_ptr(),
+                              bvals.data_ptr(), x.data_ptr(), y.data_ptr(),
+                              pp, sp, dotslot, dot_accum, _stream())
+    assert bcol.dtype == torch.int32
+    return K.spmv_bsell(nslices, nnodes, dof, bptr.data_ptr(), bcol.data_ptr(),
+                        bvals.data_ptr(), x.data_ptr(), y.data_ptr(),
+                        pp, sp, dotslot, dot_accum, _stream())
+
+
+def _check_idx16(bptr, bcol16, bbase) -> None:
+    assert bcol16.dtype == torch.uint16 and bcol16.is_contiguous()
+    assert bbase.dtype == torch.int32 and bbase.is_contiguous()
+    assert bbase.numel() == bptr.numel() - 1
 
 
 def stencil_spmv(mf, nrows_nodes: int, row0_node: int, x: torch.Tensor,
                  y: torch.Tensor, *, mato: bool = False,
                  partials: torch.Tensor | None = None,
                  scal: torch.Tensor | None = None, dotslot: int = -1,
-                 dot_accum: bool = True) -> None:
+                 dot_accum: bool = True, finalize: bool = True) -> int:
     if nrows_nodes <= 0:
-        return
+        return 0
     fuse = scal is not None and dotslot >= 0
     pp = partials.data_ptr() if fuse else 0
-    sp = scal.data_ptr() if fuse else 0
+    sp = scal.data_ptr() if fuse and finalize else 0
     if not mato and mf["w7"] is not None:
-        K.stencil_spmv7(mf["gx"] * mf["gy"], mf["gx"], mf["z0"], mf["z1"],
-                        mf["gz"], mf["nown_nodes"], mf["pb"].data_ptr(),
-                        mf["diag"], *mf["w7"], x.data_ptr(), y.data_ptr(),
-                        pp, sp, dotslot, dot_accum, _stream())
-        return
-    K.stencil_spmv(nrows_nodes, row0_node, mf["gx"], mf["gy"], mf["gz"],
-                   mf["nown_nodes"], mf["zs"].data_ptr(),
-                   mf["pb"].data_ptr(), mf["offs"].data_ptr(), mf["ksten"],
-                   mf["diag"], x.data_ptr(), y.data_ptr(), mato,
-                   pp, sp, dotslot, dot_accum, _stream())
+        return K.stencil_spmv7(mf["gx"] * mf["gy"], mf["gx"], mf["z0"],
+                               mf["z1"], mf["gz"], mf["nown_nodes"],
+                               mf["pb"].data_ptr(), mf["diag"], *mf["w7"],
+                               x.data_ptr(), y.data_ptr(),
+                               pp, sp, dotslot, dot_accum, _stream())
+    return K.stencil_spmv(nrows_nodes, row0_node, mf["gx"], mf["gy"], mf["gz"],
+                          mf["nown_nodes"], mf["zs"].data_ptr(),
+                          mf["pb"].data_ptr(), mf["offs"].data_ptr(),
+                          mf["ksten"], mf["diag"], x.data_ptr(), y.data_ptr(),
+                          mato, pp, sp, dotslot, dot_accum, _stream())
 
 
 def stencil_pipe(mf, nrows_nodes: int, row0_node: int, border_base: int,
@@ -226,9 +243,18 @@
                      pold: torch.Tensor, rvec: torch.Tensor,
                      pnew: torch.Tensor, y: torch.Tensor,
                      scal: torch.Tensor, partials: torch.Tensor,
-                     dotslot: int) -> None:
+                     dotslot: int, bbase: torch.Tensor | None = None) -> None:
     nslices = bptr.numel() - 1
     if nslices <= 0:
+        return
+    if bbase is not None:
+        _check_idx16(bptr, bcol, bbase)
+        K.spmv_bsell_daypx16(nslices, nnodes, dof, bptr.data_ptr(),
+                             bbase.data_ptr(), bcol.data_ptr(),
+                             bvals.data_ptr(), pold.data_ptr(),
+                             rvec.data_ptr(), pnew.data_ptr(), y.data_ptr(),
+                             scal.data_ptr(), partials.data_ptr(), dotslot,
+                             _stream())
         return
     K.spmv_bsell_daypx(nslices, nnodes, dof, bptr.data_ptr(), bcol.data_ptr(),
                        bvals.data_ptr(), pold.data_ptr(), rvec.data_ptr(),
@@ -280,6 +306,27 @@
                     partials: torch.Tensor, n: int) -> None:
     K.cg_fused_update(r.data_ptr(), x.data_ptr(), p.data_ptr(), t.data_ptr(),
                       n, scal.data_ptr(), partials.data_ptr(), _stream())
+
+
+def reduce_partials(partials: torch.Tensor, nb: int, scal: torch.Tensor,
+                    slot: int, accumulate: bool = False) -> None:
+    assert 0 <= nb <= MAXG
+    K.reduce_partials(partials.data_ptr(), nb, scal.data_ptr(), slot,
+                      accumulate, _stream())
+
+
+def cg_update_r(r: torch.Tensor, t: torch.Tensor, scal: torch.Tensor,
+                partials: torch.Tensor, n: int, nb: int) -> None:
+    assert partials.numel() >= 2 * MAXG and 1 <= nb <= MAXG
+    K.cg_update_r(r.data_ptr(), t.data_ptr(), n, scal.data_ptr(),
+                  partials.data_ptr(), nb, _stream())
+
+
+def cg_update_xp(x: torch.Tensor, p: torch.Tensor, r: torch.Tensor,
+                 scal: torch.Tensor, partials: torch.Tensor, n: int) -> None:
+    assert partials.numel() >= 2 * MAXG
+    K.cg_update_xp(x.data_ptr(), p.data_ptr(), r.data_ptr(), n,
+                   scal.data_ptr(), partials.data_ptr(), _stream())
 
 
 def pcg_fused_update(r, x, p, t, z, dinv, scal, partials, n: int) -> None:
diff --git a/acg_amd/ops/kernels.hip b/acg_amd/ops/kernels.hip
--- a/acg_amd/ops/kernels.hip
+++ b/acg_amd/ops/kernels.hip
@@ -176,11 +176,12 @@
                       : (long)EVEN * WAVE + lane;
 }
 
-template <int DOF, bool FUSE_DOT>
+template <int DOF, bool FUSE_DOT, typename IdxT = int>
 __global__ void __launch_bounds__(BLOCK)
 k_spmv_bsell(long nslices, long nnodes,
              const long* __restrict__ bptr,
-             const int* __restrict__ bcol,
+             const IdxT* __restrict__ bcol,
+             const int* __restrict__ bbase,
              const double* __restrict__ bvals,
              const double* __restrict__ x,
              double* __restrict__ y,
@@ -192,13 +193,15 @@
     for (long s = wslice; s < nslices; s += nw) {
         const long b0 = bptr[s];
         const long blen = (bptr[s + 1] - b0) >> 6;
-        const int* __restrict__ c = bcol + b0 + lane;
+        const IdxT* __restrict__ c = bcol + b0 + lane;
         const double* __restrict__ v = bvals + b0 * (DOF * DOF);
+        int cbase = 0;
+        if constexpr (sizeof(IdxT) == 2) cbase = bbase[s];
         double acc[DOF];
         #pragma unroll
         for (int r = 0; r < DOF; ++r) acc[r] = 0.0;
         for (long j = 0; j < blen; ++j) {
-            const int cb = ld_nt(c + j * WAVE);
+            const int cb = cbase + (int)ld_nt(c + j * WAVE);
             double xv[DOF];
             #pragma unroll
             for (int cc = 0; cc < DOF; ++cc) xv[cc] = x[(long)cb * DOF + cc];
@@ -224,11 +227,12 @@
     }
 }
 
-template <int DOF>
+template <int DOF, typename IdxT = int>
 __global__ void __launch_bounds__(BLOCK)
 k_spmv_bsell_daypx(long nslices, long nnodes,
                    const long* __restrict__ bptr,
-                   const int* __restrict__ bcol,
+                   const IdxT* __restrict__ bcol,
+                   const int* __restrict__ bbase,
                    const double* __restrict__ bvals,
                    const double* __restrict__ pold,
                    const double* __restrict__ rvec,
@@ -244,13 +248,15 @@
     for (long s = wslice; s < nslices; s += nw) {
         const long b0 = bptr[s];
         const long blen = (bptr[s + 1] - b0) >> 6;
-        const int* __restrict__ c = bcol + b0 + lane;
+        const IdxT* __restrict__ c = bcol + b0 + lane;
         const double* __restrict__ v = bvals + b0 * (DOF * DOF);
+        int cbase = 0;
+        if constexpr (sizeof(IdxT) == 2) cbase = bbase[s];
         double acc[DOF];
         #pragma unroll
         for (int r = 0; r < DOF; ++r) acc[r] = 0.0;
         for (long j = 0; j < blen; ++j) {
-            const int cb = ld_nt(c + j * WAVE);
+            const int cb = cbase + (int)ld_nt(c + j * WAVE);
             double xv[DOF];
             #pragma unroll
             for (int cc = 0; cc < DOF; ++cc)
@@ -501,6 +507,107 @@
     if (threadIdx.x == 0) partials[blockIdx.x] = acc;
 }
 
+
+__device__ __forceinline__ double block_sum_partials(const double* partials,
+                                                     int nb) {
+    double v = 0.0;
+    int i = threadIdx.x;
+    for (; i + 7 * BLOCK < nb; i += 8 * BLOCK) {
+        double a[8];
+        #pragma unroll
+        for (int u = 0; u < 8; ++u) a[u] = partials[i + u * BLOCK];
+        #pragma unroll
+        for (int u = 0; u < 8; ++u) v += a[u];
+    }
+    for (; i < nb; i += BLOCK) v += partials[i];
+    v = block_reduce(v);
+    __shared__ double bcast;
+    if (threadIdx.x == 0) bcast = v;
+    __syncthreads();
+    return bcast;
+}
+
+#define TAIL_V 4
+
+__global__ void __launch_bounds__(BLOCK)
+k_cg_update_r(double* __restrict__ r, const double* __restrict__ t, long n,
+              double* scal, double* partials, int nb, int vblocks) {
+    const double pt = block_sum_partials(partials, nb);
+    const double rr = scal[S_RR];
+    const double alpha = safe_div(rr, pt);
+    const long vstride = (long)vblocks * BLOCK;
+    long i0[TAIL_V];
+    double acc[TAIL_V];
+    #pragma unroll
+    for (int v = 0; v < TAIL_V; ++v) {
+        const long vb = (long)blockIdx.x + (long)v * gridDim.x;
+        i0[v] = vb < vblocks ? vb * BLOCK + threadIdx.x : n;
+        acc[v] = 0.0;
+    }
+    for (long k = 0; i0[0] + k < n; k += vstride) {
+        double rv[TAIL_V], tv[TAIL_V];
+        #pragma unroll
+        for (int v = 0; v < TAIL_V; ++v) {
+            const long i = i0[v] + k;
+            const bool ok = i0[v] < n && i < n;
+            rv[v] = ok ? r[i] : 0.0;
+            tv[v] = ok ? ld_nt(t + i) : 0.0;
+        }
+        #pragma unroll
+        for (int v = 0; v < TAIL_V; ++v) {
+            const long i = i0[v] + k;
+            if (i0[v] < n && i < n) {
+                const double rn = rv[v] - alpha * tv[v];
+                r[i] = rn;
+                acc[v] += rn * rn;
+            }
+        }
+    }
+    #pragma unroll
+    for (int v = 0; v < TAIL_V; ++v) {
+        const long vb = (long)blockIdx.x + (long)v * gridDim.x;
+        const double a = block_reduce(acc[v]);
+        if (threadIdx.x == 0 && vb < vblocks) partials[MAXG + vb] = a;
+        __syncthreads();
+    }
+    if (blockIdx.x == 0 && threadIdx.x == 0) {
+        scal[S_PT] = pt;
+        scal[S_RR_PREV] = rr;
+    }
+}
+
+__global__ void __launch_bounds__(BLOCK)
+k_cg_update_xp(double* __restrict__ x, double* __restrict__ p,
+               const double* __restrict__ r, long n, double* scal,
+               const double* partials, int nb2) {
+    const double rr_new = block_sum_partials(partials + MAXG, nb2);
+    const double rr_old = scal[S_RR_PREV];
+    const double alpha = safe_div(rr_old, scal[S_PT]);
+    const double beta = safe_div(rr_new, rr_old);
+    const long stride = (long)gridDim.x * BLOCK;
+    for (long i = (long)blockIdx.x * BLOCK + threadIdx.x; i < n;
+         i += stride * TAIL_V) {
+        double pv[TAIL_V], xv[TAIL_V], rv[TAIL_V];
+        #pragma unroll
+        for (int v = 0; v < TAIL_V; ++v) {
+            const long j = i + v * stride;
+            const bool ok = j < n;
+            pv[v] = ok ? p[j] : 0.0;
+            xv[v] = ok ? ld_nt(x + j) : 0.0;
+            rv[v] = ok ? r[j] : 0.0;
+        }
+        #pragma unroll
+        for (int v = 0; v < TAIL_V; ++v) {
+            const long j = i + v * stride;
+            if (j < n) {
+                __builtin_nontemporal_store(xv[v] + alpha * pv[v], x + j);
+                p[j] = beta * pv[v] + rv[v];
+            }
+        }
+    }
+    if (blockIdx.x == 0 && threadIdx.x == 0) scal[S_RR] = rr_new;
+}
+
 __device__ __forceinline__ void pipelined_coeffs(const double* scal, int first,
                                                  double* beta, double* alpha) {
     const double gamma = scal[S_GAMMA], delta = scal[S_DELTA];
@@ -739,61 +846,109 @@
     }
 }
 
-void spmv_bsell(long nslices, long nnodes, int dof, uintptr_t bptr,
-                uintptr_t bcol, uintptr_t bvals, uintptr_t x, uintptr_t y,
-                uintptr_t partials, uintptr_t scal, int dotslot,
-                bool dot_accum, uintptr_t stream) {
-    if (nnodes == 0) return;
+static long spmv_bsell_impl(long nslices, long nnodes, int dof, uintptr_t bptr,
+                            uintptr_t bcol, uintptr_t bbase, uintptr_t bvals,
+                            uintptr_t x, uintptr_t y, uintptr_t partials,
+                            uintptr_t scal, int dotslot, bool dot_accum,
+                            uintptr_t stream) {
+    if (nnodes == 0) return 0;
     long blocks = (nslices * WAVE + BLOCK - 1) / BLOCK;
     if (blocks > MAXG) blocks = MAXG;
     const bool fuse = partials != 0 && dotslot >= 0;
     dim3 g((unsigned)blocks), b(BLOCK);
-    #define LBS(D, FD) \
-        hipLaunchKernelGGL((k_spmv_bsell<D, FD>), g, b, 0, (hipStream_t)stream, \
-            nslices, nnodes, (const long*)bptr, (const int*)bcol, \
-            (const double*)bvals, (const double*)x, (double*)y, (double*)partials)
+    #define LBS(D, FD, IT) \
+        hipLaunchKernelGGL((k_spmv_bsell<D, FD, IT>), g, b, 0, (hipStream_t)stream, \
+            nslices, nnodes, (const long*)bptr, (const IT*)bcol, \
+            (const int*)bbase, (const double*)bvals, (const double*)x, \
+            (double*)y, (double*)partials)
+    #define LBS_I(D, FD) \
+        if (bbase != 0) { LBS(D, FD, unsigned short); } else { LBS(D, FD, int); }
     switch (dof) {
-        case 2: if (fuse) { LBS(2, true); } else { LBS(2, false); } break;
-        case 3: if (fuse) { LBS(3, true); } else { LBS(3, false); } break;
-        case 4: if (fuse) { LBS(4, true); } else { LBS(4, false); } break;
+        case 2: if (fuse) { LBS_I(2, true); } else { LBS_I(2, false); } break;
+        case 3: if (fuse) { LBS_I(3, true); } else { LBS_I(3, false); } break;
+        case 4: if (fuse) { LBS_I(4, true); } else { LBS_I(4, false); } break;
         default: throw std::runtime_error("spmv_bsell: dof must be 2/3/4");
     }
+    #undef LBS_I
     #undef LBS
     check_hip("spmv_bsell");
-    if (fuse) {
+    if (fuse && scal != 0) {
         hipLaunchKernelGGL(k_reduce_partials, dim3(1), dim3(BLOCK), 0,
                            (hipStream_t)stream, (const double*)partials,
                            (int)blocks, (double*)scal, dotslot, dot_accum ? 1 : 0);
         check_hip("spmv_bsell_reduce");
     }
-}
-
-void spmv_bsell_daypx(long nslices, long nnodes, int dof, uintptr_t bptr,
-                      uintptr_t bcol, uintptr_t bvals, uintptr_t pold,
-                      uintptr_t rvec, uintptr_t pnew, uintptr_t y,
-                      uintptr_t scal, uintptr_t partials, int dotslot,
-                      uintptr_t stream) {
+    return fuse ? blocks : 0;
+}
+
+long spmv_bsell(long nslices, long nnodes, int dof, uintptr_t bptr,
+                uintptr_t bcol, uintptr_t bvals, uintptr_t x, uintptr_t y,
+                uintptr_t partials, uintptr_t scal, int dotslot,
+                bool dot_accum, uintptr_t stream) {
+    return spmv_bsell_impl(nslices, nnodes, dof, bptr, bcol, 0, bvals, x, y,
+                           partials, scal, dotslot, dot_accum, stream);
+}
+
+long spmv_bsell16(long nslices, long nnodes, int dof, uintptr_t bptr,
+                  uintptr_t bbase, uintptr_t bcol16, uintptr_t bvals,
+                  uintptr_t x, uintptr_t y, uintptr_t partials, uintptr_t scal,
+                  int dotslot, bool dot_accum, uintptr_t stream) {
+    if (bbase == 0) throw std::runtime_error("spmv_bsell16: bbase is null");
+    return spmv_bsell_impl(nslices, nnodes, dof, bptr, bcol16, bbase, bvals,
+                           x, y, partials, scal, dotslot, dot_accum, stream);
+}
+
+static void spmv_bsell_daypx_impl(long nslices, long nnodes, int dof,
+                                  uintptr_t bptr, uintptr_t bcol,
+                                  uintptr_t bbase, uintptr_t bvals,
+                                  uintptr_t pold, uintptr_t rvec,
+                                  uintptr_t pnew, uintptr_t y, uintptr_t scal,
+                                  uintptr_t partials, int dotslot,
+                                  uintptr_t stream) {
     if (nnodes == 0) return;
     long blocks = (nslices * WAVE + BLOCK - 1) / BLOCK;
     if (blocks > MAXG) blocks = MAXG;
     dim3 g((unsigned)blocks), b(BLOCK);
-    #define LBD(D) \
-        hipLaunchKernelGGL((k_spmv_bsell_daypx<D>), g, b, 0, (hipStream_t)stream, \
-            nslices, nnodes, (const long*)bptr, (const int*)bcol, \
-            (const double*)bvals, (const double*)pold, (const double*)rvec, \
-            (double*)pnew, (double*)y, (const double*)scal, (double*)partials)
+    #define LBD(D, IT) \
+        hipLaunchKernelGGL((k_spmv_bsell_daypx<D, IT>), g, b, 0, (hipStream_t)stream, \
+            nslices, nnodes, (const long*)bptr, (const IT*)bcol, \
+            (const int*)bbase, (const double*)bvals, (const double*)pold, \
+            (const double*)rvec, (double*)pnew, (double*)y, \
+            (const double*)scal, (double*)partials)
+    #define LBD_I(D) \
+        if (bbase != 0) { LBD(D, unsigned short); } else { LBD(D, int); }
     switch (dof) {
-        case 2: LBD(2); break;
-        case 3: LBD(3); break;
-        case 4: LBD(4); break;
+        case 2: LBD_I(2); break;
+        case 3: LBD_I(3); break;
+        case 4: LBD_I(4); break;
         default: throw std::runtime_error("spmv_bsell_daypx: dof must be 2/3/4");
     }
+    #undef LBD_I
     #undef LBD
     check_hip("spmv_bsell_daypx");
     hipLaunchKernelGGL(k_reduce_partials, dim3(1), dim3(BLOCK), 0,
                        (hipStream_t)stream, (const double*)partials,
                        (int)blocks, (double*)scal, dotslot, 0);
     check_hip("spmv_bsell_daypx_reduce");
+}
+
+void spmv_bsell_daypx(long nslices, long nnodes, int dof, uintptr_t bptr,
+                      uintptr_t bcol, uintptr_t bvals, uintptr_t pold,
+                      uintptr_t rvec, uintptr_t pnew, uintptr_t y,
+                      uintptr_t scal, uintptr_t partials, int dotslot,
+                      uintptr_t stream) {
+    spmv_bsell_daypx_impl(nslices, nnodes, dof, bptr, bcol, 0, bvals, pold,
+                          rvec, pnew, y, scal, partials, dotslot, stream);
+}
+
+void spmv_bsell_daypx16(long nslices, long nnodes, int dof, uintptr_t bptr,
+                        uintptr_t bbase, uintptr_t bcol16, uintptr_t bvals,
+                        uintptr_t pold, uintptr_t rvec, uintptr_t pnew,
+                        uintptr_t y, uintptr_t scal, uintptr_t partials,
+                        int dotslot, uintptr_t stream) {
+    if (bbase == 0) throw std::runtime_error("spmv_bsell_daypx16: bbase is null");
+    spmv_bsell_daypx_impl(nslices, nnodes, dof, bptr, bcol16, bbase, bvals,
+                          pold, rvec, pnew, y, scal, partials, dotslot, stream);
 }
 
 void stencil_blocklen(long nnodes, int gx, int gy, int gz, long nown_nodes,
@@ -1070,13 +1225,13 @@
     }
 }
 
-void stencil_spmv7(long plane_nodes, int gx, int z0, int z1, int gz,
+long stencil_spmv7(long plane_nodes, int gx, int z0, int z1, int gz,
                    long nown_nodes, uintptr_t pb, double diag,
                    double wxm, double wxp, double wym, double wyp,
                    double wzm, double wzp, uintptr_t x, uintptr_t y,
                    uintptr_t partials, uintptr_t scal, int dotslot,
                    bool dot_accum, uintptr_t stream) {
-    if (plane_nodes == 0 || z1 <= z0) return;
+    if (plane_nodes == 0 || z1 <= z0) return 0;
     long blocks = (plane_nodes + BLOCK - 1) / BLOCK;
     if (blocks > MAXG) blocks = MAXG;
     const bool fuse = partials != 0 && dotslot >= 0;
@@ -1089,12 +1244,13 @@
     if (fuse) { LS7(true); } else { LS7(false); }
     #undef LS7
     check_hip("stencil_spmv7");
-    if (fuse) {
+    if (fuse && scal != 0) {
         hipLaunchKernelGGL(k_reduce_partials, dim3(1), dim3(BLOCK), 0,
                            (hipStream_t)stream, (const double*)partials,
                            (int)blocks, (double*)scal, dotslot, dot_accum ? 1 : 0);
         check_hip("stencil_spmv7_reduce");
     }
+    return fuse ? blocks : 0;
 }
 
 long stencil_pipe7(long plane_nodes, int gx, int z0, int z1, int gz,
@@ -1121,12 +1277,12 @@
     return blocks;
 }
 
-void stencil_spmv(long nrows_nodes, long row0_node, int gx, int gy, int gz,
+long stencil_spmv(long nrows_nodes, long row0_node, int gx, int gy, int gz,
                   long nown_nodes, uintptr_t zs_of_plane, uintptr_t pb,
                   uintptr_t offs, int ksten, double diag, uintptr_t x,
                   uintptr_t y, bool mato, uintptr_t partials, uintptr_t scal,
                   int dotslot, bool dot_accum, uintptr_t stream) {
-    if (nrows_nodes == 0) return;
+    if (nrows_nodes == 0) return 0;
     const long blocks = elem_grid(nrows_nodes);
     const bool fuse = partials != 0 && dotslot >= 0;
     dim3 g((unsigned)blocks), b(BLOCK);
@@ -1140,12 +1296,13 @@
     else      { if (fuse) { LMS(false, true); } else { LMS(false, false); } }
     #undef LMS
     check_hip("stencil_spmv");
-    if (fuse) {
+    if (fuse && scal != 0) {
         hipLaunchKernelGGL(k_reduce_partials, dim3(1), dim3(BLOCK), 0,
                            (hipStream_t)stream, (const double*)partials,
                            (int)blocks, (double*)scal, dotslot, dot_accum ? 1 : 0);
         check_hip("stencil_spmv_reduce");
     }
+    return fuse ? blocks : 0;
 }
 
 long stencil_pipe(long nrows_nodes, long row0_node, long border_base,
@@ -1430,11 +1587,11 @@
     check_hip("reduce_partials");
 }
 
-void spmv(long nrows, long rowbase, uintptr_t rowptr, uintptr_t colidx,
+long spmv(long nrows, long rowbase, uintptr_t rowptr, uintptr_t colidx,
           int col64, uintptr_t vals, uintptr_t x, uintptr_t y,
           int lanes, bool accum, uintptr_t partials, uintptr_t scal,
           int dotslot, bool dot_accum, uintptr_t stream) {
-    if (nrows == 0) return;
+    if (nrows == 0) return 0;
     const int rows_per_block = BLOCK / lanes;
     long blocks = (nrows + rows_per_block - 1) / rows_per_block;
     if (blocks > MAXG) blocks = MAXG;
@@ -1460,11 +1617,12 @@
     #undef DISPATCH_L
     #undef LAUNCH_SPMV
     check_hip("spmv");
-    if (fuse)
+    if (fuse && scal != 0)
         reduce_partials(partials, (int)blocks, scal, dotslot, dot_accum, stream);
-}
-
-void spmv_binned(long rowbase, uintptr_t rowptr, uintptr_t colidx, int col64,
+    return fuse ? blocks : 0;
+}
+
+long spmv_binned(long rowbase, uintptr_t rowptr, uintptr_t colidx, int col64,
                  uintptr_t vals, uintptr_t x, uintptr_t y, uintptr_t rowlist,
                  const std::vector<std::array<long, 3>>& bins,
                  bool accum, uintptr_t partials, uintptr_t scal,
@@ -1506,16 +1664,17 @@
         if (fuse) poff += blocks;
     }
     check_hip("spmv_binned");
-    if (fuse && poff > 0)
+    if (fuse && poff > 0 && scal != 0)
         reduce_partials(partials, (int)poff, scal, dotslot, dot_accum, stream);
-}
-
-void spmv_sell(long nslices, long nrows, long rowbase, uintptr_t sellptr,
+    return poff;
+}
+
+long spmv_sell(long nslices, long nrows, long rowbase, uintptr_t sellptr,
                uintptr_t cols, int col64, uintptr_t vals, uintptr_t x,
                uintptr_t y, bool accum, uintptr_t partials, uintptr_t scal,
                int dotslot, bool dot_accum, int variant, uintptr_t perm,
                uintptr_t stream) {
-    if (nrows == 0) return;
+    if (nrows == 0) return 0;
     long blocks = (nslices * WAVE + BLOCK - 1) / BLOCK;
     if (blocks > MAXG) blocks = MAXG;
     const bool fuse = partials != 0 && dotslot >= 0;
@@ -1537,9 +1696,9 @@
         #undef LAUNCH_PERM
         #undef LAUNCH_PERM_U
         check_hip("spmv_sell_perm");
-        if (fuse)
+        if (fuse && scal != 0)
             reduce_partials(partials, (int)blocks, scal, dotslot, dot_accum, stream);
-        return;
+        return fuse ? blocks : 0;
     }
     #define LAUNCH_SELL(CT, AC, FD, NT, SWZ, U) \
         hipLaunchKernelGGL((k_spmv_sell<CT, AC, FD, NT, SWZ, U>), g, b, 0, S(stream), \
@@ -1563,8 +1722,9 @@
     #undef DISP_V
     #undef LAUNCH_SELL
     check_hip("spmv_sell");
-    if (fuse)
+    if (fuse && scal != 0)
         reduce_partials(partials, (int)blocks, scal, dotslot, dot_accum, stream);
+    return fuse ? blocks : 0;
 }
 
 void zero_scalars(uintptr_t scal, int i0, int count, uintptr_t stream) {
@@ -1642,6 +1802,28 @@
     hipLaunchKernelGGL(k_cg_finalize, dim3(1), dim3(BLOCK), 0, S(stream),
                        (const double*)partials, (int)blocks, (double*)scal);
     check_hip("cg_finalize");
+}
+
+void cg_update_r(uintptr_t r, uintptr_t t, long n, uintptr_t scal,
+                 uintptr_t partials, int nb, uintptr_t stream) {
+    if (nb < 1 || nb > MAXG)
+        throw std::runtime_error("cg_update_r: nb must be in [1, MAXG]");
+    const long vblocks = elem_grid(n);
+    const long blocks = (vblocks + TAIL_V - 1) / TAIL_V;
+    hipLaunchKernelGGL(k_cg_update_r, dim3((unsigned)blocks), dim3(BLOCK), 0, S(stream),
+                       (double*)r, (const double*)t, n, (double*)scal,
+                       (double*)partials, nb, (int)vblocks);
+    check_hip("cg_update_r");
+}
+
+void cg_update_xp(uintptr_t x, uintptr_t p, uintptr_t r, long n, uintptr_t scal,
+                  uintptr_t partials, uintptr_t stream) {
+    const long vblocks = elem_grid(n);
+    const long blocks = (vblocks + TAIL_V - 1) / TAIL_V;
+    hipLaunchKernelGGL(k_cg_update_xp, dim3((unsigned)blocks), dim3(BLOCK), 0, S(stream),
+                       (double*)x, (double*)p, (const double*)r, n, (double*)scal,
+                       (const double*)partials, (int)vblocks);
+    check_hip("cg_update_xp");
 }
 
 long sell_pipe(long nslices, long nrows_pass, long rowbase, long border_base,
@@ -1772,6 +1954,11 @@
     m.def("axpy_ratio", &axpy_ratio);
     m.def("daypx_ratio", &daypx_ratio);
     m.def("cg_fused_update", &cg_fused_update);
+    m.def("reduce_partials", &reduce_partials);
+    m.def("cg_update_r", &cg_update_r);
+    m.def("cg_update_xp", &cg_update_xp);
+    m.def("spmv_bsell16", &spmv_bsell16);
+    m.def("spmv_bsell_daypx16", &spmv_bsell_daypx16);
     m.def("pcg_fused_update", &pcg_fused_update);
     m.def("pipelined_fused", &pipelined_fused);
     m.def("sell_pipe", &sell_pipe);
diff --git a/acg_amd/ops/torch_ref.py b/acg_amd/ops/torch_ref.py
--- a/acg_amd/ops/torch_ref.py
+++ b/acg_amd/ops/torch_ref.py
@@ -14,14 +14,23 @@
 
 
 def alloc_partials(device="cpu") -> torch.Tensor:
-    return torch.zeros(1, dtype=torch.float64, device=device)
+    return torch.zeros(2 * MAXG, dtype=torch.float64, device=device)
+
+
+def _publish_dot(d, partials, scal, dotslot, dot_accum, finalize) -> int:
+    if finalize:
+        scal[dotslot] = scal[dotslot] + d if dot_accum else d
+        return 0
+    partials[0] = d
+    return 1
 
 
 def spmv(rowptr, colidx, vals, x, y, *, rowbase: int = 0, accum: bool = False,
-         partials=None, scal=None, dotslot: int = -1, dot_accum: bool = True) -> None:
+         partials=None, scal=None, dotslot: int = -1, dot_accum: bool = True,
+         finalize: bool = True) -> int:
     nrows = rowptr.numel() - 1
     if nrows <= 0:
-        return
+        return 0
     counts = rowptr[1:] - rowptr[:-1]
     rows = torch.repeat_interleave(torch.arange(nrows, dtype=torch.int64,
                                                 device=rowptr.device), counts)
@@ -34,17 +43,20 @@
     else:
         y[sl] = contrib
     if scal is not None and dotslot >= 0:
-        d = torch.dot(x[sl], contrib)
-        scal[dotslot] = scal[dotslot] + d if dot_accum else d
+        return _publish_dot(torch.dot(x[sl], contrib), partials, scal,
+                            dotslot, dot_accum, finalize)
+    return 0
 
 
 def spmv_binned(rowptr, colidx, vals, rowlist, bins, x, y, *, rowbase: int = 0,
                 accum: bool = False, partials=None, scal=None,
-                dotslot: int = -1, dot_accum: bool = True) -> None:
+                dotslot: int = -1, dot_accum: bool = True,
+                finalize: bool = True) -> int:
     if rowlist.numel() == 0:
-        return
-    spmv(rowptr, colidx, vals, x, y, rowbase=rowbase, accum=accum,
-         partials=partials, scal=scal, dotslot=dotslot, dot_accum=dot_accum)
+        return 0
+    return spmv(rowptr, colidx, vals, x, y, rowbase=rowbase, accum=accum,
+                partials=partials, scal=scal, dotslot=dotslot,
+                dot_accum=dot_accum, finalize=finalize)
 
 
 def zero_scalars(scal, i0: int = 0, count=None) -> None:
@@ -227,7 +239,7 @@
 def spmv_sell(sellptr, cols, vals, nrows, x, y, *, rowbase: int = 0,
               accum: bool = False, partials=None, scal=None,
               dotslot: int = -1, dot_accum: bool = True, C: int = 64,
-              variant=None, perm=None) -> None:
+              variant=None, perm=None, finalize: bool = True) -> int:
     nslices = sellptr.numel() - 1
     assert (nrows + C - 1) // C == nslices, \
         f"SELL structure was built with a different chunk size than C={C}"
@@ -250,8 +262,9 @@
     else:
         y[sl] = contrib
     if scal is not None and dotslot >= 0:
-        d = torch.dot(x[sl], contrib)
-        scal[dotslot] = scal[dotslot] + d if dot_accum else d
+        return _publish_dot(torch.dot(x[sl], contrib), partials, scal,
+                            dotslot, dot_accum, finalize)
+    return 0
 
 
 def _bsell_contrib(bptr, bcol, bvals, nnodes: int, dof: int, xg, C: int = 64):
@@ -280,23 +293,63 @@
     return contrib
 
 
+def bsell_compress_idx16(bptr, bcol, C: int = 64):
+    import numpy as np
+
+    nslices = bptr.numel() - 1
+    if nslices <= 0 or bcol.numel() == 0:
+        return None
+    rows = bcol.view(-1, C)
+    rmin = rows.min(dim=1).values.cpu().numpy().astype(np.int64)
+    rmax = rows.max(dim=1).values.cpu().numpy().astype(np.int64)
+    rptr = bptr.cpu().numpy().astype(np.int64) // C
+    blen = np.diff(rptr)
+    ne = blen > 0
+    smin = np.zeros(nslices, dtype=np.int64)
+    smax = np.zeros(nslices, dtype=np.int64)
+    smin[ne] = np.minimum.reduceat(rmin, rptr[:-1][ne])
+    smax[ne] = np.maximum.reduceat(rmax, rptr[:-1][ne])
+    if int((smax - smin).max()) > 65535 or int(smin.min()) < 0:
+        return None
+    bbase = torch.from_numpy(smin.astype(np.int32)).to(bcol.device)
+    row_base = torch.repeat_interleave(
+        bbase, torch.from_numpy(blen).to(bcol.device))
+    off = rows - row_base[:, None]
+    off16 = torch.where(off >= 32768, off - 65536, off).to(torch.int16)
+    return bbase, off16.reshape(-1).view(torch.uint16)
+
+
+def bsell_expand_idx16(bptr, bbase, bcol16, C: int = 64):
+    blen = (bptr[1:] - bptr[:-1]) // C
+    row_base = torch.repeat_interleave(bbase, blen.to(bbase.device))
+    off = bcol16.view(torch.int16).to(torch.int32) & 0xFFFF
+    return (off.view(-1, C) + row_base[:, None]).reshape(-1).to(torch.int32)
+
+
 def spmv_bsell(bptr, bcol, bvals, nnodes: int, dof: int, x, y, *,
                partials=None, scal=None, dotslot: int = -1,
-               dot_accum: bool = True) -> None:
+               dot_accum: bool = True, finalize: bool = True,
+               bbase=None) -> int:
     if bptr.numel() - 1 <= 0:
-        return
+        return 0
+    if bbase is not None:
+        bcol = bsell_expand_idx16(bptr, bbase, bcol)
     n = nnodes * dof
     contrib = _bsell_contrib(bptr, bcol, bvals, nnodes, dof, x)
     y[:n] = contrib
     if scal is not None and dotslot >= 0:
-        d = torch.dot(x[:n], contrib)
-        scal[dotslot] = scal[dotslot] + d if dot_accum else d
+        return _publish_dot(torch.dot(x[:n], contrib), partials, scal,
+                            dotslot, dot_accum, finalize)
+    return 0
 
 
 def spmv_bsell_daypx(bptr, bcol, bvals, nnodes: int, dof: int, pold, rvec,
-                     pnew, y, scal, partials, dotslot: int) -> None:
+                     pnew, y, scal, partials, dotslot: int,
+                     bbase=None) -> None:
     if bptr.numel() - 1 <= 0:
         return
+    if bbase is not None:
+        bcol = bsell_expand_idx16(bptr, bbase, bcol)
     n = nnodes * dof
     beta = _sdiv(float(scal[S_RR]), float(scal[S_RR_PREV]))
     pn = beta * pold[:n] + rvec[:n]
@@ -353,6 +406,30 @@
     x[:n] += alpha * p[:n]
     scal[S_RR_PREV] = scal[S_RR].clone()
     scal[S_RR] = torch.dot(r[:n], r[:n])
+
+
+def reduce_partials(partials, nb, scal, slot, accumulate=False) -> None:
+    d = partials[:nb].sum()
+    scal[slot] = scal[slot] + d if accumulate else d
+
+
+def cg_update_r(r, t, scal, partials, n, nb) -> None:
+    pt = partials[:nb].sum()
+    alpha = _sdiv(float(scal[S_RR]), float(pt))
+    r[:n] -= alpha * t[:n]
+    partials[MAXG] = torch.dot(r[:n], r[:n])
+    scal[S_PT] = pt
+    scal[S_RR_PREV] = scal[S_RR].clone()
+
+
+def cg_update_xp(x, p, r, scal, partials, n) -> None:
+    rr_new = partials[MAXG].clone()
+    rr_old = float(scal[S_RR_PREV])
+    alpha = _sdiv(rr_old, float(scal[S_PT]))
+    beta = _sdiv(float(rr_new), rr_old)
+    x[:n] += alpha * p[:n]
+    p[:n] = beta * p[:n] + r[:n]
+    scal[S_RR] = rr_new
 
 
 def pcg_fused_update(r, x, p, t, z, dinv, scal, partials, n) -> None:
diff --git a/acg_amd/solvers/hip.py b/acg_amd/solvers/hip.py
--- a/acg_amd/solvers/hip.py
+++ b/acg_amd/solvers/hip.py
@@ -19,7 +19,8 @@
     def __init__(self, local: LocalSystem, comm=None, device=None,
                  lanes: int | None = None, use_sell: bool = True,
                  profile: bool = False, matfree: bool = False,
-                 force_format: str | None = None):
+                 force_format: str | None = None,
+                 idx16: bool | None = None):
         self.local = local
         self.comm = comm
         if device is None:
@@ -69,6 +70,13 @@
             mean_nnzO = L.nnzO / max(L.nborder, 1)
             self.lanesO = lanes or ops.pick_lanes(mean_nnzO)
             self._pick_format(L, up, use_sell, force_format)
+        self.bsell16 = None
+        if idx16 is None:
+            idx16 = os.environ.get("ACG_BSELL_IDX16", "1") != "0"
+        if idx16 and self.bsell is not None:
+            from ..ops.torch_ref import bsell_compress_idx16
+
+            self.bsell16 = bsell_compress_idx16(self.bsell[0], self.bsell[1])
         self.can_megafuse = (
             self.matfree is not None
             or (self.sell is not None and self.sell_perm is None
@@ -183,6 +191,13 @@
         if self.sell is not None or self.bsell is not None:
             self.A_rowptr = self.A_colidx = self.A_vals = None
 
+    def _bsell_idx_bytes_per_nnz(self) -> float:
+        d2 = float(self.bsell[3] ** 2)
+        if self.bsell16 is None:
+            return 4.0 / d2
+        nblocks = max(self.bsell[1].numel(), 1)
+        return (2.0 + 4.0 * self.bsell16[0].numel() / nblocks) / d2
+
     def _workspace(self, key: str, names) -> dict:
         ws = self._ws.setdefault(key, {})
         for nm, nghost in names:
@@ -201,8 +216,9 @@
             self.comm.allreduce_(self.scal[slot:slot + count])
 
     def _spmv_overlapped(self, xfull: torch.Tensor, y: torch.Tensor,
-                         fuse_dotslot: int = -1):
+                         fuse_dotslot: int = -1, finalize: bool = True):
         L = self.local
+        nb = 0
         have_halo = self.comm is not None and self.comm.size > 1
         cur = torch.cuda.current_stream(self.device)
         halo_span = None
@@ -215,20 +231,24 @@
                 self.halo.begin(xfull)
         fuse = dict(partials=self.partials,
                     scal=self.scal if fuse_dotslot >= 0 else None,
-                    dotslot=fuse_dotslot)
+                    dotslot=fuse_dotslot, finalize=finalize)
         with self.prof.span("spmvA"):
             if self.matfree is not None:
-                ops.stencil_spmv(self.matfree, self.n, 0, xfull, y,
-                                 mato=False, dot_accum=False, **fuse)
+                nb = ops.stencil_spmv(self.matfree, self.n, 0, xfull, y,
+                                      mato=False, dot_accum=False, **fuse)
             elif self.bsell is not None:
                 bptr, bcol, bvals, dof = self.bsell
-                ops.spmv_bsell(bptr, bcol, bvals, self.n // dof, dof,
-                               xfull, y, dot_accum=False, **fuse)
+                bbase = None
+                if self.bsell16 is not None:
+                    bbase, bcol = self.bsell16
+                nb = ops.spmv_bsell(bptr, bcol, bvals, self.n // dof, dof,
+                                    xfull, y, dot_accum=False, bbase=bbase,
+                                    **fuse)
             elif self.sell is not None:
                 sellptr, scols, svals = self.sell
-                ops.spmv_sell(sellptr, scols, svals, self.n, xfull, y,
-                              accum=False, perm=self.sell_perm,
-                              dot_accum=False, **fuse)
+                nb = ops.spmv_sell(sellptr, scols, svals, self.n, xfull, y,
+                                   accum=False, perm=self.sell_perm,
+                                   dot_accum=False, **fuse)
             elif self.hybrid is not None:
                 h = self.hybrid
                 have_sell = h["sellptr"] is not None
@@ -242,9 +262,9 @@
                                     xfull, y, accum=False,
                                     dot_accum=have_sell, **fuse)
             else:
-                ops.spmv(self.A_rowptr, self.A_colidx, self.A_vals, xfull, y,
-                         lanes=self.lanesA, accum=False, dot_accum=False,
-                         **fuse)
+                nb = ops.spmv(self.A_rowptr, self.A_colidx, self.A_vals,
+                              xfull, y, lanes=self.lanesA, accum=False,
+                              dot_accum=False, **fuse)
         if have_halo:
             with torch.cuda.stream(self.comm_stream):
                 self.halo.end()
@@ -270,6 +290,7 @@
                     ops.spmv(self.O_rowptr, self.O_colidx, self.O_vals, xfull, y,
                              rowbase=L.ninterior, lanes=self.lanesO, accum=True,
                              **fuse)
+        return nb
 
     def _host_scalar(self, slot: int) -> float:
         cur = torch.cuda.current_stream(self.device)
@@ -289,7 +310,8 @@
               res_atol: float = 0.0, res_rtol: float = 1e-9,
               use_graph: bool | None = None,
               fold_daypx: bool | None = None,
-              diff_atol: float = 0.0, diff_rtol: float = 0.0) -> SolveResult:
+              diff_atol: float = 0.0, diff_rtol: float = 0.0,
+              fused_tail: bool | None = None) -> SolveResult:
         res = SolveResult(solver="cg-hip", maxits=maxits, res_atol=res_atol,
                           res_rtol=res_rtol,
                           nranks=self.comm.size if self.comm else 1)
@@ -331,10 +353,16 @@
         if fold:
             p2 = self._workspace("classic", [("p2", True)])["p2"]
             scal[S.S_RR_PREV] = math.inf
+        if fused_tail is None:
+            fused_tail = os.environ.get("ACG_FUSED_TAIL", "1") != "0"
+        tail3 = (bool(fused_tail) and serial and not fold
+                 and not self.prof.enabled and self.local.nnzO == 0
+                 and self.hybrid is None and n > 0)
         if use_graph is None:
             use_graph = not serial
         graph_ok = use_graph and serial and not self.prof.enabled and not fold
-        graph = self._graphs.get("classic") if graph_ok else None
+        gkey = "classic:tail3" if tail3 else "classic"
+        graph = self._graphs.get(gkey) if graph_ok else None
         dist_key = "classic:dist"
         dist_failed_key = "classic:capture_failed"
         dist_graph_ok = (use_graph and not serial and not self.prof.enabled
@@ -351,13 +379,22 @@
         def body(k: int = 0):
             if fold:
                 bptr, bcol, bvals, dof = self.bsell
+                bbase = None
+                if self.bsell16 is not None:
+                    bbase, bcol = self.bsell16
                 pold, pnew = (p, p2) if k % 2 == 0 else (p2, p)
                 with self.prof.span("spmvA"):
                     S.spmv_bsell_daypx(bptr, bcol, bvals, n // dof, dof,
                                        pold, r, pnew, t, scal,
-                                       self.partials, S.S_PT)
+                                       self.partials, S.S_PT, bbase=bbase)
                 with self.prof.span("update_classic"):
                     S.cg_fused_update(r, xi, pnew, t, scal, self.partials, n)
+                return
+            if tail3:
+                nb = self._spmv_overlapped(p, t, fuse_dotslot=S.S_PT,
+                                           finalize=False)
+                S.cg_update_r(r, t, scal, self.partials, n, nb)
+                S.cg_update_xp(xi, p, r, scal, self.partials, n)
                 return
             self._spmv_overlapped(p, t, fuse_dotslot=S.S_PT)
             with self.prof.span("allreduce"):
@@ -399,7 +436,7 @@
                     graph = torch.cuda.CUDAGraph()
                     with torch.cuda.graph(graph):
                         body()
-                    self._graphs["classic"] = graph
+                    self._graphs[gkey] = graph
                 elif dist_graph_ok and k == 2 and dgraph is None:
                     try:
                         gg = torch.cuda.CUDAGraph()
@@ -475,7 +512,7 @@
             if self.matfree is not None:
                 idxb = -8.0
             elif self.bsell is not None:
-                idxb = 4.0 / (self.bsell[3] ** 2)
+                idxb = self._bsell_idx_bytes_per_nnz()
             annotate_op_stats(res, self.local, self.prof.collect(),
                               idx_bytes_per_nnz=idxb)
             self.prof.reset()
@@ -880,7 +917,7 @@
             if self.matfree is not None:
                 idxb = -8.0
             elif self.bsell is not None:
-                idxb = 4.0 / (self.bsell[3] ** 2)
+                idxb = self._bsell_idx_bytes_per_nnz()
             annotate_op_stats(res, self.local, self.prof.collect(),
                               idx_bytes_per_nnz=idxb)
             self.prof.reset()
```

After: 1868 iter/s. 1.4% lower.
